# pgvector/pgvector

Measured on AMD Instinct MI355X. Metric: QPS @ recall@10 (IVFFlat, 1M x 1536d), higher is better.
Workload: dtype f32

## Files before the change

include/pgv_hip.h:

```cpp
#ifndef PGV_HIP_H
#define PGV_HIP_H

#include <stddef.h>
#include <stdint.h>

#ifdef __cplusplus
extern "C" {
#endif

#define PGV_ABI_VERSION 1

#define PGV_OK 0
#define PGV_ERR_ARG 1
#define PGV_ERR_DIMS 2
#define PGV_ERR_DEVICE 3
#define PGV_ERR_NOMEM 4
#define PGV_ERR_STATE 5
#define PGV_ERR_DATA 6

typedef enum pgv_dtype
{
	PGV_F32 = 0,
	PGV_F16 = 1
}			pgv_dtype;

typedef enum pgv_metric
{
	PGV_L2SQ = 0,
	PGV_NEG_IP = 1,
	PGV_L1 = 2
}			pgv_metric;

typedef enum pgv_ops
{
	PGV_OPS_L2 = 0,
	PGV_OPS_IP = 1,
	PGV_OPS_COSINE = 2
}			pgv_ops;

typedef struct pgv_ctx pgv_ctx;
typedef struct pgv_index pgv_index;
typedef struct pgv_hnsw pgv_hnsw;

typedef struct pgv_rng
{
	double		(*next_double) (void *state);
	uint32_t	(*next_u32) (void *state);
	void	   *state;
	uint64_t	seed;
}			pgv_rng;


const char *pgv_last_error(void);
int			pgv_abi_version(void);

int			pgv_device_count(void);
int			pgv_scan_chain_length(int dim, pgv_dtype dtype, int path);
int			pgv_device_memory(int device, uint64_t *free_bytes, uint64_t *total_bytes);
int			pgv_pinned_alloc(size_t bytes, void **out);
void		pgv_pinned_free(void *p);
int			pgv_pinned_register(void *p, size_t bytes);
void		pgv_pinned_unregister(void *p);

#define PGV_DEFAULT_STREAM ((void *) (intptr_t) -1)
int			pgv_ctx_create(int device, void *stream, pgv_ctx * *out);
void		pgv_ctx_destroy(pgv_ctx * ctx);
int			pgv_ctx_sync(pgv_ctx * ctx);
void	   *pgv_ctx_stream(pgv_ctx * ctx);
int			pgv_timer_start(pgv_ctx * ctx);
int			pgv_timer_stop(pgv_ctx * ctx, float *out_ms);

typedef struct pgv_stats
{
	double		scan_ms;
	int64_t		scan_launches;
	double		scan_pairs;
	double		scan_rows;
	double		aux_ms;
	int64_t		aux_launches;
	double		aux_pairs;
	double		assign_redo_rows;
	double		assign_rows;
	double		assign_recheck_rows;
	double		scan_unique_rows;
	double		scan_redo_queries;
	double		scan_widened_queries;
	double		scan_shadow_queries;
}			pgv_stats;
int			pgv_ctx_set_profiling(pgv_ctx * ctx, int on);
int			pgv_ctx_set_exact_scan(pgv_ctx * ctx, int on);
#define PGV_BOUND_STATISTICAL 0
#define PGV_BOUND_WORST_CASE 1
int			pgv_ctx_set_bound(pgv_ctx * ctx, int mode);
int			pgv_ctx_reset_stats(pgv_ctx * ctx);
int			pgv_ctx_get_stats(pgv_ctx * ctx, pgv_stats * out);


int			pgv_index_upload(pgv_ctx * ctx, pgv_metric metric, pgv_dtype dtype, int dim, int nlists,
							 const void *centers, const int64_t *list_offsets,
							 const void *vectors, const uint64_t *tids, pgv_index * *out);
void		pgv_index_free(pgv_index * index);
int			pgv_index_share(pgv_index * index, pgv_ctx * ctx, pgv_index * *out);
int			pgv_index_set_overlap(pgv_index * index, int lanes);
#define PGV_INDEX_HANDLE_BYTES 256
typedef struct pgv_index_handle
{
	unsigned char bytes[PGV_INDEX_HANDLE_BYTES];
}			pgv_index_handle;
int			pgv_index_export(pgv_index * index, pgv_index_handle * out);
int			pgv_index_import(pgv_ctx * ctx, const pgv_index_handle * handle, pgv_index * *out);
int			pgv_index_tids(pgv_index * index, const int64_t *slots, int64_t n, uint64_t *out);
int64_t		pgv_index_rows(const pgv_index * index);
int			pgv_index_lists(const pgv_index * index);

int			pgv_rank_lists(pgv_index * index, const void *queries, int nq, int maxprobes,
						   int32_t *out_lists, float *out_dist);

int			pgv_scan_lists(pgv_index * index, const void *query, const int32_t *lists, int nlists,
						   float *out_dist, int64_t *out_slot, int64_t capacity, int64_t *out_count);

int			pgv_search_batch(pgv_index * index, const void *queries, int nq, int probes, int k,
							 float *out_dist, int64_t *out_slot, uint64_t *out_tid);

int			pgv_scan_batch(pgv_index * index, const void *queries, int nq, const int32_t *probe_lists,
						   int probes, int k, float *out_dist, int64_t *out_slot, uint64_t *out_tid);

typedef struct pgv_query pgv_query;
int			pgv_query_begin(pgv_index * index, pgv_query * *out);
void		pgv_query_end(pgv_query * q);
int			pgv_query_rank(pgv_query * q, const void *query, int max_probes);
int			pgv_query_scan(pgv_query * q, int first, int nprobes, int head, float *out_dist, int64_t *out_slot,
						   uint64_t *out_tid, int *out_count, int64_t *out_total);
int			pgv_query_more(pgv_query * q, int skip, int count, float *out_dist, int64_t *out_slot,
						   uint64_t *out_tid, int *out_count);
int			pgv_query_lists(pgv_query * q, int32_t *out_lists, int n);


int			pgv_assign(pgv_ctx * ctx, pgv_metric metric, pgv_dtype dtype, int dim,
					   const void *centers, int k, const void *rows, int64_t n,
					   int32_t *out_list, float *out_dist);

int			pgv_kmeans(pgv_ctx * ctx, pgv_ops ops, pgv_dtype dtype, int dim,
					   const void *samples, int n, int k, int max_iterations, const pgv_rng * rng,
					   void *out_centers, int32_t *out_closest, int *out_iters);

int			pgv_lloyd_partial(pgv_ctx * ctx, pgv_ops ops, pgv_dtype dtype, int dim,
							  const void *samples, int n, const void *centers, int k,
							  int32_t *io_closest, float *out_sums, int32_t *out_counts,
							  int64_t *out_changes);
int			pgv_lloyd_finish(pgv_ctx * ctx, pgv_ops ops, pgv_dtype dtype, int dim, int k,
							 const float *sums, const int32_t *counts, const pgv_rng * rng,
							 void *out_centers);

int			pgv_kmeanspp_init(pgv_ctx * ctx, pgv_ops ops, pgv_dtype dtype, int dim,
							  const void *samples, int n, int k, const pgv_rng * rng,
							  void *out_centers);


typedef struct pgv_comm pgv_comm;

#define PGV_COMM_ID_BYTES 128
int			pgv_comm_unique_id(void *out_id);
int			pgv_comm_create(pgv_ctx * ctx, int nranks, int rank, const void *unique_id, pgv_comm * *out);

typedef struct pgv_collectives
{
	int			(*all_reduce_sum_f32) (void *state, float *buf, size_t count, void *stream);
	int			(*all_gather) (void *state, const void *send, void *recv, size_t bytes_per_rank, void *stream);
	void	   *state;
}			pgv_collectives;
int			pgv_comm_create_custom(pgv_ctx * ctx, int nranks, int rank, const pgv_collectives * coll, pgv_comm * *out);
void		pgv_comm_destroy(pgv_comm * comm);
int			pgv_comm_size(const pgv_comm * comm);
int			pgv_comm_rank(const pgv_comm * comm);

int			pgv_kmeans_sharded(pgv_comm * comm, pgv_ops ops, pgv_dtype dtype, int dim,
							   const void *samples_local, int n_local, int k, int max_iterations,
							   const pgv_rng * rng, void *out_centers, int32_t *out_closest_local, int *out_iters);

int			pgv_search_batch_sharded(pgv_comm * comm, pgv_index * local_index, const void *queries, int nq,
									 int probes, int k, float *out_dist, uint64_t *out_tid);

typedef struct pgv_builder pgv_builder;
int			pgv_builder_begin(pgv_ctx * ctx, pgv_metric metric, pgv_dtype dtype, int dim, int nlists, const void *centers,
							  int64_t expected_rows, pgv_builder * *out);
int			pgv_builder_add(pgv_builder * b, const void *rows, const uint64_t *tids, int64_t n);
int			pgv_builder_set_centers(pgv_builder * b, const void *centers);
int64_t		pgv_builder_rows(const pgv_builder * b);
int			pgv_builder_finish(pgv_builder * b, pgv_index * *out_index, int64_t *out_offsets, int32_t *out_lists);
void		pgv_builder_free(pgv_builder * b);
typedef int (*pgv_rows_sink) (void *arg, int64_t first_slot, int64_t count, const void *vectors, const uint64_t *tids);
int			pgv_index_drain(pgv_index * index, int64_t chunk_rows, pgv_rows_sink sink, void *arg);


int			pgv_distance_batch(pgv_ctx * ctx, pgv_metric metric, pgv_dtype dtype, int dim,
							   const void *query, const void *rows, int64_t n, float *out);

int			pgv_exact_topk(pgv_ctx * ctx, pgv_metric metric, pgv_dtype dtype, int dim, const void *queries, int nq,
						   const void *rows, int64_t n, int k, float *out_dist, int64_t *out_idx);

int			pgv_cosine_distance_batch(pgv_ctx * ctx, pgv_dtype dtype, int dim,
									  const void *query, const void *rows, int64_t n, double *out);

typedef enum pgv_bit_metric
{
	PGV_BIT_HAMMING = 0,
	PGV_BIT_JACCARD = 1
}			pgv_bit_metric;

int			pgv_bit_distance_batch(pgv_ctx * ctx, pgv_bit_metric metric, int nbits,
								   const void *query, const void *rows, int64_t n, double *out);


int			pgv_hnsw_upload(pgv_ctx * ctx, pgv_metric metric, pgv_dtype dtype, int dim,
							const void *elements, int64_t n, pgv_hnsw * *out);
void		pgv_hnsw_free(pgv_hnsw * h);
int			pgv_hnsw_upload_payload(pgv_ctx * ctx, pgv_metric metric, pgv_dtype dtype, int dim, const void *elements,
									int64_t n, const void *payload, int payload_bytes, pgv_hnsw * *out);
int			pgv_hnsw_get_payload(pgv_hnsw * h, const int64_t *elements, int n, void *out);

int			pgv_hnsw_export(pgv_hnsw * h, pgv_index_handle * out);
int			pgv_hnsw_share(pgv_hnsw * h, pgv_ctx * ctx, pgv_hnsw * *out);
int			pgv_hnsw_device(const pgv_hnsw * h);
int			pgv_hnsw_import(pgv_ctx * ctx, const pgv_index_handle * handle, pgv_hnsw * *out);

int			pgv_hnsw_score(pgv_hnsw * h, const void *queries, int nq,
						   const int32_t *slot, const int32_t *query_of, int64_t npairs, float *out);

int			pgv_hnsw_set_graph(pgv_hnsw * h, int m, int32_t entry, const int32_t *levels,
							   const int64_t *nbr_start, const int32_t *nbr);

int			pgv_hnsw_search(pgv_hnsw * h, const void *queries, int nq, int ef_search, int k,
							int64_t *out_elem, float *out_dist, int64_t *out_scored);


int			pgv_hnsw_build_search(pgv_hnsw * h, const int32_t *elements, const int32_t *insert_levels, int nq,
								  int ef_construction, int layer_cap,
								  int32_t *out_ids, float *out_dist, int32_t *out_count);

int			pgv_hnsw_build_neighbors(pgv_hnsw * h, const int32_t *elements, const int32_t *insert_levels, int nq,
									 int ef_construction, int layer_cap,
									 int32_t *out_ids, float *out_dist, uint8_t *out_closer, int32_t *out_count,
									 int64_t *out_pairs);

int			pgv_hnsw_build_search_keep(pgv_hnsw * h, const int32_t *elements, const int32_t *insert_levels, int nq,
									   int ef_construction, int layer_cap, int slot);
int			pgv_hnsw_build_select_kept(pgv_hnsw * h, int slot, int32_t *out_ids, float *out_dist, uint8_t *out_closer,
									   int32_t *out_count, int64_t *out_pairs);

int			pgv_hnsw_link_begin(pgv_hnsw * h);
int			pgv_hnsw_link_prepare(pgv_hnsw * h, const int32_t *elements, const uint8_t *linked, int nq, int layer_cap,
								  const int32_t *sel_ids, const float *sel_dist, const uint8_t *sel_closer,
								  const int32_t *sel_count, int64_t *out_pairs);
int			pgv_hnsw_link_apply(pgv_hnsw * h, int32_t entry);
int			pgv_hnsw_link_end(pgv_hnsw * h, int32_t *out_nbr, int64_t *out_pairs, int64_t *out_deferred);

int			pgv_hnsw_score_pairs(pgv_hnsw * h, const int32_t *a, const int32_t *b, int64_t npairs, float *out);
int			pgv_hnsw_score_groups(pgv_hnsw * h, const int32_t *ids, const int64_t *ids_start, const int32_t *from,
								  const int64_t *pair_start, int ngroups, int64_t nids, int64_t npairs, float *out);


int			pgv_hnsw_update_graph(pgv_hnsw * h, int32_t entry, const int32_t *elements, int nupd,
								  const int64_t *tuple_offsets, const int32_t *tuples);

#ifdef __cplusplus
}
#endif
#endif
```

pgvector_amd/_lib.py:

```python
import ctypes as C
import os

try:
    import torch
except ImportError:
    torch = None

_HERE = os.path.dirname(os.path.abspath(__file__))
LIB_PATH = os.environ.get("PGV_HIP_LIB") or os.path.join(_HERE, "lib", "libpgv_hip.so")

PGV_OK, PGV_ERR_ARG, PGV_ERR_DIMS, PGV_ERR_DEVICE, PGV_ERR_NOMEM, PGV_ERR_STATE, PGV_ERR_DATA = range(7)
PGV_F32, PGV_F16 = 0, 1
PGV_L2SQ, PGV_NEG_IP, PGV_L1 = 0, 1, 2
PGV_OPS_L2, PGV_OPS_IP, PGV_OPS_COSINE = 0, 1, 2
PGV_BOUND_STATISTICAL, PGV_BOUND_WORST_CASE = 0, 1

SYMBOLS = [
    "pgv_last_error", "pgv_abi_version", "pgv_device_count", "pgv_scan_chain_length", "pgv_ctx_create", "pgv_ctx_destroy",
    "pgv_ctx_sync", "pgv_ctx_stream", "pgv_timer_start", "pgv_timer_stop", "pgv_ctx_set_profiling", "pgv_ctx_set_exact_scan", "pgv_index_share", "pgv_pinned_alloc", "pgv_pinned_free",
    "pgv_ctx_reset_stats", "pgv_ctx_get_stats", "pgv_index_upload", "pgv_index_free",
    "pgv_index_rows", "pgv_index_lists", "pgv_rank_lists", "pgv_scan_lists", "pgv_search_batch", "pgv_scan_batch",
    "pgv_assign", "pgv_kmeans", "pgv_lloyd_partial", "pgv_lloyd_finish", "pgv_kmeanspp_init",
    "pgv_distance_batch", "pgv_cosine_distance_batch", "pgv_bit_distance_batch", "pgv_hnsw_upload", "pgv_hnsw_free", "pgv_hnsw_score", "pgv_hnsw_set_graph", "pgv_hnsw_search",
    "pgv_hnsw_build_search", "pgv_hnsw_build_neighbors", "pgv_hnsw_link_begin", "pgv_hnsw_link_prepare",
    "pgv_hnsw_link_apply", "pgv_hnsw_link_end", "pgv_hnsw_build_search_keep", "pgv_hnsw_build_select_kept", "pgv_hnsw_score_pairs", "pgv_hnsw_score_groups", "pgv_hnsw_update_graph",
    "pgv_query_begin", "pgv_query_end", "pgv_query_rank", "pgv_query_scan", "pgv_query_more", "pgv_query_lists",
    "pgv_comm_unique_id", "pgv_comm_create", "pgv_comm_create_custom", "pgv_comm_destroy", "pgv_comm_size",
    "pgv_comm_rank", "pgv_kmeans_sharded", "pgv_search_batch_sharded",
    "pgv_device_memory", "pgv_pinned_register", "pgv_pinned_unregister", "pgv_index_export", "pgv_index_import",
    "pgv_index_tids", "pgv_hnsw_export", "pgv_hnsw_import", "pgv_hnsw_share", "pgv_hnsw_device", "pgv_exact_topk", "pgv_ctx_set_bound",
    "pgv_hnsw_upload_payload", "pgv_hnsw_get_payload", "pgv_builder_begin", "pgv_builder_add", "pgv_builder_set_centers", "pgv_builder_rows", "pgv_builder_finish", "pgv_builder_free", "pgv_index_drain",
    "pgv_index_set_overlap",
]


class PgvError(RuntimeError):
    def __init__(self, code, message):
        super().__init__("libpgv_hip error %d: %s" % (code, message))
        self.code = code
        self.message = message


class PgvStats(C.Structure):
    _fields_ = [("scan_ms", C.c_double), ("scan_launches", C.c_int64),
                ("scan_pairs", C.c_double), ("scan_rows", C.c_double),
                ("aux_ms", C.c_double), ("aux_launches", C.c_int64), ("aux_pairs", C.c_double),
                ("assign_redo_rows", C.c_double), ("assign_rows", C.c_double), ("assign_recheck_rows", C.c_double), ("scan_unique_rows", C.c_double), ("scan_redo_queries", C.c_double), ("scan_widened_queries", C.c_double),
                ("scan_shadow_queries", C.c_double)]


ALL_REDUCE_F32 = C.CFUNCTYPE(C.c_int, C.c_void_p, C.c_void_p, C.c_size_t, C.c_void_p)
ALL_GATHER = C.CFUNCTYPE(C.c_int, C.c_void_p, C.c_void_p, C.c_void_p, C.c_size_t, C.c_void_p)


class PgvCollectives(C.Structure):
    _fields_ = [("all_reduce_sum_f32", ALL_REDUCE_F32), ("all_gather", ALL_GATHER), ("state", C.c_void_p)]


NEXT_DOUBLE = C.CFUNCTYPE(C.c_double, C.c_void_p)
NEXT_U32 = C.CFUNCTYPE(C.c_uint32, C.c_void_p)


class PgvRng(C.Structure):
    _fields_ = [("next_double", C.c_void_p), ("next_u32", C.c_void_p),
                ("state", C.c_void_p), ("seed", C.c_uint64)]


def _load():
    if not os.path.exists(LIB_PATH):
        raise ImportError(
            "libpgv_hip.so not built (%s): run `python -c 'import __graft_entry__ as g; g.build()'` "
            "or `make -C pgvector_amd/csrc` -- there is no CPU fallback" % LIB_PATH)
    lib = C.CDLL(LIB_PATH)
    P, I, I64 = C.c_void_p, C.c_int, C.c_int64
    lib.pgv_last_error.restype = C.c_char_p
    lib.pgv_last_error.argtypes = []
    lib.pgv_abi_version.restype = I
    lib.pgv_device_count.restype = I
    lib.pgv_scan_chain_length.argtypes = [I, I, I]
    lib.pgv_scan_chain_length.restype = I
    lib.pgv_ctx_create.argtypes = [I, P, C.POINTER(P)]
    lib.pgv_ctx_destroy.argtypes = [P]
    lib.pgv_ctx_destroy.restype = None
    lib.pgv_ctx_sync.argtypes = [P]
    lib.pgv_ctx_stream.argtypes = [P]
    lib.pgv_ctx_stream.restype = P
    lib.pgv_timer_start.argtypes = [P]
    lib.pgv_timer_stop.argtypes = [P, C.POINTER(C.c_float)]
    lib.pgv_ctx_set_profiling.argtypes = [P, I]
    lib.pgv_ctx_set_exact_scan.argtypes = [P, I]
    lib.pgv_ctx_reset_stats.argtypes = [P]
    lib.pgv_ctx_get_stats.argtypes = [P, C.POINTER(PgvStats)]
    lib.pgv_index_upload.argtypes = [P, I, I, I, I, P, P, P, P, C.POINTER(P)]
    lib.pgv_index_free.argtypes = [P]
    lib.pgv_index_share.argtypes = [P, P, C.POINTER(P)]
    lib.pgv_index_set_overlap.argtypes = [P, I]
    lib.pgv_index_free.restype = None
    lib.pgv_index_export.argtypes = [P, P]
    lib.pgv_index_import.argtypes = [P, P, C.POINTER(P)]
    lib.pgv_index_tids.argtypes = [P, P, I64, P]
    lib.pgv_hnsw_export.argtypes = [P, P]
    lib.pgv_hnsw_share.argtypes = [P, P, C.POINTER(P)]
    lib.pgv_hnsw_device.argtypes = [P]
    lib.pgv_hnsw_upload_payload.argtypes = [P, I, I, I, P, I64, P, I, C.POINTER(P)]
    lib.pgv_hnsw_get_payload.argtypes = [P, P, I, P]
    lib.pgv_exact_topk.argtypes = [P, I, I, I, P, I, P, I64, I, P, P]
    lib.pgv_ctx_set_bound.argtypes = [P, I]
    lib.pgv_builder_begin.argtypes = [P, I, I, I, I, P, I64, C.POINTER(P)]
    lib.pgv_builder_add.argtypes = [P, P, P, I64]
    lib.pgv_builder_set_centers.argtypes = [P, P]
    lib.pgv_builder_rows.argtypes = [P]
    lib.pgv_builder_rows.restype = I64
    lib.pgv_builder_finish.argtypes = [P, C.POINTER(P), P, P]
    lib.pgv_builder_free.argtypes = [P]
    lib.pgv_builder_free.restype = None
    lib.pgv_index_drain.argtypes = [P, I64, P, P]
    lib.pgv_hnsw_import.argtypes = [P, P, C.POINTER(P)]
    lib.pgv_device_memory.argtypes = [I, C.POINTER(C.c_uint64), C.POINTER(C.c_uint64)]
    lib.pgv_pinned_register.argtypes = [P, C.c_size_t]
    lib.pgv_pinned_unregister.argtypes = [P]
    lib.pgv_pinned_unregister.restype = None
    lib.pgv_index_rows.argtypes = [P]
    lib.pgv_index_rows.restype = I64
    lib.pgv_index_lists.argtypes = [P]
    lib.pgv_rank_lists.argtypes = [P, P, I, I, P, P]
    lib.pgv_scan_lists.argtypes = [P, P, P, I, P, P, I64, C.POINTER(I64)]
    lib.pgv_search_batch.argtypes = [P, P, I, I, I, P, P, P]
    lib.pgv_scan_batch.argtypes = [P, P, I, P, I, I, P, P, P]
    lib.pgv_query_begin.argtypes = [P, C.POINTER(P)]
    lib.pgv_query_end.argtypes = [P]
    lib.pgv_query_end.restype = None
    lib.pgv_query_rank.argtypes = [P, P, I]
    lib.pgv_query_scan.argtypes = [P, I, I, I, P, P, P, C.POINTER(I), C.POINTER(I64)]
    lib.pgv_query_more.argtypes = [P, I, I, P, P, P, C.POINTER(I)]
    lib.pgv_query_lists.argtypes = [P, P, I]
    lib.pgv_comm_unique_id.argtypes = [P]
    lib.pgv_comm_create.argtypes = [P, I, I, P, C.POINTER(P)]
    lib.pgv_comm_create_custom.argtypes = [P, I, I, C.POINTER(PgvCollectives), C.POINTER(P)]
    lib.pgv_comm_destroy.argtypes = [P]
    lib.pgv_comm_destroy.restype = None
    lib.pgv_comm_size.argtypes = [P]
    lib.pgv_comm_rank.argtypes = [P]
    lib.pgv_kmeans_sharded.argtypes = [P, I, I, I, P, I, I, I, C.POINTER(PgvRng), P, P, C.POINTER(I)]
    lib.pgv_search_batch_sharded.argtypes = [P, P, P, I, I, I, P, P]
    lib.pgv_assign.argtypes = [P, I, I, I, P, I, P, I64, P, P]
    lib.pgv_kmeans.argtypes = [P, I, I, I, P, I, I, I, C.POINTER(PgvRng), P, P, C.POINTER(I)]
    lib.pgv_lloyd_partial.argtypes = [P, I, I, I, P, I, P, I, P, P, P, P]
    lib.pgv_lloyd_finish.argtypes = [P, I, I, I, I, P, P, C.POINTER(PgvRng), P]
    lib.pgv_kmeanspp_init.argtypes = [P, I, I, I, P, I, I, C.POINTER(PgvRng), P]
    lib.pgv_distance_batch.argtypes = [P, I, I, I, P, P, I64, P]
    lib.pgv_hnsw_upload.argtypes = [P, I, I, I, P, I64, C.POINTER(P)]
    lib.pgv_hnsw_free.argtypes = [P]
    lib.pgv_hnsw_free.restype = None
    lib.pgv_hnsw_score.argtypes = [P, P, I, P, P, I64, P]
    lib.pgv_cosine_distance_batch.argtypes = [P, I, I, P, P, I64, P]
    lib.pgv_bit_distance_batch.argtypes = [P, I, I, P, P, I64, P]
    lib.pgv_hnsw_set_graph.argtypes = [P, I, C.c_int32, P, P, P]
    lib.pgv_hnsw_search.argtypes = [P, P, I, I, I, P, P, P]
    lib.pgv_hnsw_build_search.argtypes = [P, P, P, I, I, I, P, P, P]
    lib.pgv_hnsw_build_neighbors.argtypes = [P, P, P, I, I, I, P, P, P, P, P]
    lib.pgv_hnsw_score_pairs.argtypes = [P, P, P, I64, P]
    lib.pgv_hnsw_update_graph.argtypes = [P, C.c_int32, P, I, P, P]
    return lib


lib = _load()


def check(rc):
    if rc != PGV_OK:
        raise PgvError(rc, lib.pgv_last_error().decode("utf-8", "replace"))
```

pgvector_amd/csrc/kernels_query.hip:

```cpp
#include "pgv_device.h"
#include "pgv_select.h"

#include <type_traits>

namespace pgv {

namespace {

constexpr int kQThreads = kSelThreads;
constexpr int kQWaves = kQThreads / kWave;
constexpr int kMaxBatchLists = 256;
constexpr int kHeadCap = 1024;

template <typename T, int METRIC, int NCH> struct WholeRows {
    Raw16 q[NCH];
    __device__ __forceinline__ void load_query(const char *qp, int lane) {
#pragma unroll
        for (int c = 0; c < NCH; c++) q[c] = load16(qp + ((size_t)c * kWave + lane) * sizeof(Raw16));
    }
    __device__ __forceinline__ float pair(const char *a, const char *b, int lane) const {
        Raw16 ra[NCH], rb[NCH];
#pragma unroll
        for (int c = 0; c < NCH; c++) ra[c] = load16(a + ((size_t)c * kWave + lane) * sizeof(Raw16));
#pragma unroll
// ... 162 lines not shown
        return lbeg[lo] + (j - offs[lo]);
    }
};

template <typename T, int METRIC, int NCH>
__global__ __launch_bounds__(kQThreads) void query_scan_kernel(
    const char *__restrict__ vectors, const int64_t *__restrict__ list_off, const int32_t *__restrict__ probe_lists,
    int nprobes, int nvec, int lg, const char *__restrict__ qp, float *__restrict__ seg, int per) {
    __shared__ BatchMap map;
    const size_t row_bytes = (size_t)nvec * sizeof(Raw16);
    map.build(probe_lists, nprobes, list_off);
    const int64_t m = map.offs[nprobes];
    for (int64_t first = (int64_t)blockIdx.x * per; first < m; first += (int64_t)gridDim.x * per) {
        const int64_t end = first + per < m ? first + per : m;
        if (qp) {
            score_rows<T, METRIC, NCH>([&](int64_t j) { return vectors + (size_t)map.slot_of(j, nprobes) * row_bytes; },
                                       first, end, qp, nvec, lg, seg);
        } else {
            for (int64_t j = first + threadIdx.x; j < end; j += kQThreads) seg[j] = 0.f;
        }
    }
}

__global__ __launch_bounds__(kQThreads) void query_head_kernel(
    const float *__restrict__ seg, const int64_t *__restrict__ list_off, const uint64_t *__restrict__ tids,
    const int32_t *__restrict__ probe_lists, int nprobes, int skip, int count, int kp, QueryHead *__restrict__ hdr,
    float *__restrict__ head_dist, int64_t *__restrict__ head_slot, uint64_t *__restrict__ head_tid, unsigned seq) {
    extern __shared__ __attribute__((aligned(16))) char smem[];
    __shared__ BatchMap map;
    map.build(probe_lists, nprobes, list_off);
    const int64_t m = map.offs[nprobes];
    unsigned long long *ent = reinterpret_cast<unsigned long long *>(smem);
    SelShared *s = reinterpret_cast<SelShared *>(smem + (size_t)kHeadCap * 8);
    const int k = skip + count;
    block_topk_auto(seg, m, k, kp, kHeadCap, ent, s);
    const int have = (int)(m < k ? m : k) - skip;
    for (int i = threadIdx.x; i < have; i += kQThreads) {
        const unsigned long long e = ent[skip + i];
        const int64_t slot = map.slot_of((int64_t)(unsigned)(e & 0xffffffffu), nprobes);
        head_dist[i] = key_to_float((unsigned)(e >> 32));
        head_slot[i] = slot;
        head_tid[i] = tids ? tids[slot] : ~0ull;
    }
    asm volatile("s_waitcnt vmcnt(0)" ::: "memory");
    __syncthreads();
    if (threadIdx.x == 0) {
        hdr->total = m;
        hdr->count = have > 0 ? have : 0;
        __hip_atomic_store(&hdr->seq, seq, __ATOMIC_RELEASE, __HIP_MEMORY_SCOPE_SYSTEM);
    }
}

__global__ __launch_bounds__(1024) void query_stage_kernel(const Raw16 *__restrict__ src, Raw16 *__restrict__ dst, int nvec) {
    for (int i = threadIdx.x; i < nvec; i += 1024) dst[i] = src[i];
}

__global__ void query_iota_kernel(int32_t *__restrict__ out, int n) {
    const int i = blockIdx.x * blockDim.x + threadIdx.x;
    if (i < n) out[i] = i;
}

template <typename T, int METRIC, int NCH>
__global__ __launch_bounds__(kQThreads) void mq_rank_kernel(const char *__restrict__ centers, int nlists, int nvec, int lg,
                                                            const char *__restrict__ queries, float *__restrict__ cdist,
                                                            int64_t cd_stride, int per) {
    const size_t row_bytes = (size_t)nvec * sizeof(Raw16);
    const char *qp = queries + (size_t)blockIdx.y * row_bytes;
    float *cd = cdist + (size_t)blockIdx.y * cd_stride;
    for (int64_t first = (int64_t)blockIdx.x * per; first < nlists; first += (int64_t)gridDim.x * per) {
        const int64_t end = first + per < nlists ? first + per : nlists;
        score_rows<T, METRIC, NCH>([&](int64_t j) { return centers + (size_t)j * row_bytes; }, first, end, qp, nvec, lg, cd);
    }
}

__global__ __launch_bounds__(kQThreads) void mq_lists_kernel(const float *__restrict__ cdist, int64_t cd_stride, int nlists,
                                                             int max_probes, int kp, int32_t *__restrict__ out_lists,
                                                             float *__restrict__ out_dist) {
    extern __shared__ __attribute__((aligned(16))) char smem[];
    unsigned long long *ent = reinterpret_cast<unsigned long long *>(smem);
    SelShared *s = reinterpret_cast<SelShared *>(smem + (size_t)kHeadCap * 8);
    const int q = blockIdx.x;
    block_topk_auto(cdist + (size_t)q * cd_stride, nlists, max_probes, kp, kHeadCap, ent, s);
    for (int i = threadIdx.x; i < max_probes; i += kQThreads) {
        out_lists[(size_t)q * max_probes + i] = (int32_t)(unsigned)(ent[i] & 0xffffffffu);
        if (out_dist) out_dist[(size_t)q * max_probes + i] = key_to_float((unsigned)(ent[i] >> 32));
    }
}

template <typename T, int METRIC, int NCH>
__global__ __launch_bounds__(kQThreads) void mq_scan_kernel(
    const char *__restrict__ vectors, const int64_t *__restrict__ list_off, const int32_t *__restrict__ probe_lists,
    int nprobes, int nvec, int lg, const char *__restrict__ queries, float *__restrict__ seg, int64_t seg_stride, int per) {
    __shared__ BatchMap map;
    const size_t row_bytes = (size_t)nvec * sizeof(Raw16);
    const int q = blockIdx.y;
    map.build(probe_lists + (size_t)q * nprobes, nprobes, list_off);
    const int64_t m = map.offs[nprobes];
    const char *qp = queries + (size_t)q * row_bytes;
    float *sg = seg + (size_t)q * seg_stride;
    for (int64_t first = (int64_t)blockIdx.x * per; first < m; first += (int64_t)gridDim.x * per) {
        const int64_t end = first + per < m ? first + per : m;
        score_rows<T, METRIC, NCH>([&](int64_t j) { return vectors + (size_t)map.slot_of(j, nprobes) * row_bytes; },
                                   first, end, qp, nvec, lg, sg);
    }
}

__global__ __launch_bounds__(kQThreads) void mq_head_kernel(
    const float *__restrict__ seg, int64_t seg_stride, const int64_t *__restrict__ list_off,
    const uint64_t *__restrict__ tids, const int32_t *__restrict__ probe_lists, int nprobes, int k, int kp,
    float *__restrict__ out_dist, int64_t *__restrict__ out_slot, uint64_t *__restrict__ out_tid,
    double *__restrict__ stats) {
    extern __shared__ __attribute__((aligned(16))) char smem[];
    __shared__ BatchMap map;
    const int q = blockIdx.x;
    map.build(probe_lists + (size_t)q * nprobes, nprobes, list_off);
    const int64_t m = map.offs[nprobes];
    unsigned long long *ent = reinterpret_cast<unsigned long long *>(smem);
    SelShared *s = reinterpret_cast<SelShared *>(smem + (size_t)kHeadCap * 8);
    block_topk_auto(seg + (size_t)q * seg_stride, m, k, kp, kHeadCap, ent, s);
    const int have = (int)(m < k ? m : k);
    for (int i = threadIdx.x; i < k; i += kQThreads) {
        const size_t o = (size_t)q * k + i;
        if (i < have) {
            const unsigned long long e = ent[i];
            const int64_t slot = map.slot_of((int64_t)(unsigned)(e & 0xffffffffu), nprobes);
            out_dist[o] = key_to_float((unsigned)(e >> 32));
            if (out_slot) out_slot[o] = slot;
            if (out_tid) out_tid[o] = tids ? tids[slot] : ~0ull;
        } else {
            out_dist[o] = INFINITY;
            if (out_slot) out_slot[o] = -1;
            if (out_tid) out_tid[o] = ~0ull;
        }
    }
    if (stats && threadIdx.x == 0) {
        atomicAdd(&stats[0], (double)m);
        atomicAdd(&stats[1], (double)m);
        atomicAdd(&stats[5], (double)m);
    }
}

constexpr int kRecheckCap = 256;

template <typename T, bool DOT = false>
__global__ __launch_bounds__(kQThreads) void batch_recheck_kernel(
    const char *__restrict__ vectors, const uint64_t *__restrict__ tids, int nvec, int lg,
    const char *__restrict__ queries, int kprime, int k, const float *__restrict__ approx_val,
    const int64_t *__restrict__ cand_pos, const int64_t *__restrict__ cand_slot,
    const int64_t *__restrict__ list_off, const int32_t *__restrict__ probe_lists,
    const int64_t *__restrict__ probe_off, int probes,
    const int64_t *__restrict__ seg_start, int64_t fixed_len,
    const unsigned *__restrict__ row_norm_max, ScanBound bound, const float *__restrict__ eps_add, int nq,
    float *__restrict__ out_dist, int64_t *__restrict__ out_slot, uint64_t *__restrict__ out_tid,
    int32_t *__restrict__ out_i32, int32_t *__restrict__ flags, float *__restrict__ pair_t) {
    static_assert(!DOT || std::is_same<T, float>::value, "pair terms: fp32 rows");
    __shared__ float exact[kRecheckCap];
    __shared__ float dots[DOT ? kRecheckCap : 1];
    __shared__ __attribute__((aligned(16))) unsigned long long ent[kRecheckCap];
    const int q = blockIdx.x;
    const size_t row_bytes = (size_t)nvec * sizeof(Raw16);
    const int64_t m = seg_start ? seg_start[q + 1] - seg_start[q] : fixed_len;
    const int ncand = (int)(m < kprime ? m : (int64_t)kprime);
    const int kk = ncand < k ? ncand : k;
    const float *av = approx_val + (size_t)q * kprime;
    __shared__ float qn_part[kQWaves];
    {
        const char *qrow = queries + (size_t)q * row_bytes;
        float a = 0.f;
        for (int v = threadIdx.x; v < nvec; v += kQThreads) {
            const Raw16 x = load16(qrow + (size_t)v * sizeof(Raw16));
            a = accum_slice<T, 1>(a, x, x);
        }
        for (int m2 = 32; m2 > 0; m2 >>= 1) a += __shfl_xor(a, m2);
        if ((threadIdx.x & (kWave - 1)) == 0) qn_part[threadIdx.x >> 6] = a;
    }
    __syncthreads();
    float qn = 0.f;
    for (int w = 0; w < kQWaves; w++) qn += qn_part[w];
    const float rn = __uint_as_float(*row_norm_max);
    const float cross = 2.f * sqrtf(qn * rn);
    const float eps = 1.001f * (bound.g_sq * (qn + rn + cross) + bound.g_dot * cross + bound.g_norm * rn +
                                (eps_add ? eps_add[q] : 0.f));
    unsigned band = 0u;
    if (kk > 0) {
        const float edge = av[kk - 1] + 2.f * eps;
        band = float_to_key(edge + bound.g_ref * fabsf(edge + qn));
    }
    const int cnt = __syncthreads_count((int)threadIdx.x < ncand && float_to_key(av[threadIdx.x]) <= band);
    __shared__ int64_t slots[kRecheckCap];
    if ((int)threadIdx.x < cnt) {
        const int64_t p = cand_pos[(size_t)q * kprime + threadIdx.x];
        int64_t slot = p;
        if (cand_slot) {
            slot = cand_slot[(size_t)q * kprime + threadIdx.x];
        } else {
            const int64_t *off = probe_off + (size_t)q * probes;
            int lo = 0, hi = probes - 1;
            while (lo < hi) {
                const int mid = (lo + hi + 1) >> 1;
                if (off[mid] <= p)
                    lo = mid;
                else
                    hi = mid - 1;
            }
            slot = list_off[probe_lists[(size_t)q * probes + lo]] + (p - off[lo]);
        }
        slots[threadIdx.x] = slot;
    }
    __syncthreads();
    if constexpr (DOT)
        score_rows_dot([&](int64_t j) { return vectors + (size_t)slots[j] * row_bytes; }, 0, cnt,
                       queries + (size_t)q * row_bytes, nvec, lg, exact, dots);
    else
        score_rows<T, 0, 0>([&](int64_t j) { return vectors + (size_t)slots[j] * row_bytes; }, 0, cnt,
                            queries + (size_t)q * row_bytes, nvec, lg, exact);
    __syncthreads();
    if ((int)threadIdx.x < kRecheckCap)
        ent[threadIdx.x] = (int)threadIdx.x < cnt
                               ? ((unsigned long long)float_to_key(exact[threadIdx.x]) << 32) |
                                     (unsigned)cand_pos[(size_t)q * kprime + threadIdx.x]
                               : ~0ull;
    __syncthreads();
    const unsigned long long mine = ent[threadIdx.x];
    const int64_t my_slot = (int)threadIdx.x < cnt ? slots[threadIdx.x] : -1;
    int rank = 0;
    {
        const ulonglong2 *e2 = reinterpret_cast<const ulonglong2 *>(ent);
        const int n2 = (cnt + 1) / 2;
#pragma unroll 8
        for (int j = 0; j < n2; j++) {
            const ulonglong2 o = e2[j];
            rank += o.x < mine ? 1 : 0;
            rank += o.y < mine ? 1 : 0;
        }
    }
    if ((int)threadIdx.x < cnt && rank < k) {
        const size_t o = (size_t)q * k + rank;
        out_dist[o] = key_to_float((unsigned)(mine >> 32));
        if (out_slot) out_slot[o] = my_slot;
        if (out_i32) out_i32[o] = (int32_t)my_slot;
        if (out_tid) out_tid[o] = tids ? tids[my_slot] : ~0ull;
        if constexpr (DOT) pair_t[o] = -2.f * dots[threadIdx.x];
    }
    if ((int)threadIdx.x >= kk && (int)threadIdx.x < k) {
        const size_t o = (size_t)q * k + threadIdx.x;
        out_dist[o] = INFINITY;
        if (out_slot) out_slot[o] = -1;
        if (out_i32) out_i32[o] = -1;
        if (out_tid) out_tid[o] = ~0ull;
        if constexpr (DOT) pair_t[o] = 0.f;
    }
    if (threadIdx.x == 0) {
        const int32_t flag = (m > ncand && cnt == ncand) ? 1 : 0;
        flags[q] = flag;
        if (flag) flags[nq + 1 + atomicAdd(&flags[nq], 1)] = q;
    }
}

constexpr int kWide = kRecheckCap;

template <typename T>
__global__ __launch_bounds__(kQThreads) void batch_fix_kernel(
    const char *__restrict__ vectors, const int64_t *__restrict__ list_off, const uint64_t *__restrict__ tids, int nvec,
    int lg, const char *__restrict__ queries, const int32_t *__restrict__ probe_lists,
    const int64_t *__restrict__ probe_off, int probes, const int64_t *__restrict__ seg_start, int64_t fixed_len,
    const int32_t *__restrict__ flags, int nq, float *__restrict__ seg_vals, int k, int kp, int cap,
    const unsigned *__restrict__ row_norm_max, ScanBound bound, const float *__restrict__ eps_add, int widen,
    float *__restrict__ out_dist, int64_t *__restrict__ out_slot, uint64_t *__restrict__ out_tid,
    int32_t *__restrict__ out_i32, double *__restrict__ stats, float *__restrict__ pair_t) {
    extern __shared__ __attribute__((aligned(16))) char smem[];
    unsigned long long *ent = reinterpret_cast<unsigned long long *>(smem);
    SelShared *sel = reinterpret_cast<SelShared *>(smem + (size_t)cap * 8);
    __shared__ float exact[kWide];
    __shared__ int64_t slots[kWide];
    __shared__ float qn_part[kQWaves];
    const int nflag = flags[nq];
    const size_t row_bytes = (size_t)nvec * sizeof(Raw16);
    for (int f = blockIdx.x; f < nflag; f += gridDim.x) {
        const int q = flags[nq + 1 + f];
        const int64_t base = probe_lists ? seg_start[q] : (int64_t)q * fixed_len;
        const int64_t m = probe_lists ? seg_start[q + 1] - base : fixed_len;
        const int64_t *off = probe_off + (size_t)q * probes;
        const int32_t *pl = probe_lists + (size_t)q * probes;
        auto slot_of = [&](int64_t j) -> int64_t {
            if (!probe_lists) return j;
            int lo = 0, hi = probes - 1;
            while (lo < hi) {
                const int mid = (lo + hi + 1) >> 1;
                if (off[mid] <= j)
                    lo = mid;
                else
                    hi = mid - 1;
            }
            return list_off[pl[lo]] + (j - off[lo]);
        };
        float *v = seg_vals + base;
        const char *qrow = queries + (size_t)q * row_bytes;
        auto pair_terms = [&]() {
            if constexpr (std::is_same<T, float>::value) {
                if (pair_t) {
                    __threadfence();
                    __syncthreads();
                    fill_pair_terms(vectors, row_bytes, qrow, nvec * 4, out_i32 ? out_i32 + (size_t)q * k : nullptr,
                                    out_slot ? out_slot + (size_t)q * k : nullptr, k, pair_t + (size_t)q * k);
                }
            }
        };
        bool settled = false;
        if (widen && k <= kWide / 2) {
            const int nw = (int)(m < kWide ? m : (int64_t)kWide);
            block_topk([v](int64_t i) { return v[i]; }, m, nw, kWide, cap, ent, sel);
            {
                float a = 0.f;
                for (int x = threadIdx.x; x < nvec; x += kQThreads) {
                    const Raw16 e = load16(qrow + (size_t)x * sizeof(Raw16));
                    a = accum_slice<T, 1>(a, e, e);
                }
                for (int m2 = 32; m2 > 0; m2 >>= 1) a += __shfl_xor(a, m2);
                if ((threadIdx.x & (kWave - 1)) == 0) qn_part[threadIdx.x >> 6] = a;
            }
            __syncthreads();
            float qn = 0.f;
            for (int w = 0; w < kQWaves; w++) qn += qn_part[w];
            const float rn = __uint_as_float(*row_norm_max);
            const float cross = 2.f * sqrtf(qn * rn);
            const float eps = 1.001f * (bound.g_sq * (qn + rn + cross) + bound.g_dot * cross + bound.g_norm * rn +
                                        (eps_add ? eps_add[q] : 0.f));
            const int kk = nw < k ? nw : k;
            unsigned band = 0u;
            if (kk > 0) {
                const float edge = key_to_float((unsigned)(ent[kk - 1] >> 32)) + 2.f * eps;
                band = float_to_key(edge + bound.g_ref * fabsf(edge + qn));
            }
            const int cnt = __syncthreads_count((int)threadIdx.x < nw && (unsigned)(ent[threadIdx.x] >> 32) <= band);
            settled = !(m > nw && cnt == nw);
            if (settled) {
                const unsigned my_pos = (int)threadIdx.x < cnt ? (unsigned)(ent[threadIdx.x] & 0xffffffffu) : 0u;
                if ((int)threadIdx.x < cnt) slots[threadIdx.x] = slot_of((int64_t)my_pos);
                __syncthreads();
                score_rows<T, 0, 0>([&](int64_t j) { return vectors + (size_t)slots[j] * row_bytes; }, 0, cnt, qrow, nvec, lg,
                                    exact);
                __syncthreads();
                if ((int)threadIdx.x < kWide)
                    ent[threadIdx.x] = (int)threadIdx.x < cnt
                                           ? ((unsigned long long)float_to_key(exact[threadIdx.x]) << 32) | my_pos
                                           : ~0ull;
                __syncthreads();
                const unsigned long long mine = ent[threadIdx.x];
                int rank = 0;
                for (int j = 0; j < cnt; j++) rank += ent[j] < mine ? 1 : 0;
                const int have = (int)(m < k ? m : (int64_t)k);
                if ((int)threadIdx.x < cnt && rank < k) {
                    const size_t o = (size_t)q * k + rank;
                    const int64_t slot = slots[threadIdx.x];
                    out_dist[o] = key_to_float((unsigned)(mine >> 32));
                    if (out_slot) out_slot[o] = slot;
                    if (out_i32) out_i32[o] = (int32_t)slot;
                    if (out_tid) out_tid[o] = tids ? tids[slot] : ~0ull;
                }
                if ((int)threadIdx.x >= have && (int)threadIdx.x < k) {
                    const size_t o = (size_t)q * k + threadIdx.x;
                    out_dist[o] = INFINITY;
                    if (out_slot) out_slot[o] = -1;
                    if (out_i32) out_i32[o] = -1;
                    if (out_tid) out_tid[o] = ~0ull;
                }
                if (stats && threadIdx.x == 0) atomicAdd(&stats[7], 1.0);
                pair_terms();
            }
            __syncthreads();
        }
        if (settled) continue;
        if (stats && threadIdx.x == 0) atomicAdd(&stats[6], 1.0);
        score_rows<T, 0, 0>([&](int64_t j) { return vectors + (size_t)slot_of(j) * row_bytes; }, 0, m, qrow, nvec, lg, v);
        __threadfence();
        __syncthreads();
        block_topk([v](int64_t i) { return __hip_atomic_load(v + i, __ATOMIC_RELAXED, __HIP_MEMORY_SCOPE_AGENT); }, m, k, kp,
                   cap, ent, sel);
        for (int i = threadIdx.x; i < k; i += kQThreads) {
            const unsigned long long e = ent[i];
            const bool have = e != ~0ull && (int64_t)i < (m < k ? m : (int64_t)k);
            const int64_t slot = have ? slot_of((int64_t)(unsigned)(e & 0xffffffffu)) : -1;
            out_dist[(size_t)q * k + i] = have ? key_to_float((unsigned)(e >> 32)) : INFINITY;
            if (out_slot) out_slot[(size_t)q * k + i] = slot;
            if (out_i32) out_i32[(size_t)q * k + i] = (int32_t)slot;
            if (out_tid) out_tid[(size_t)q * k + i] = (have && tids) ? tids[slot] : ~0ull;
        }
        pair_terms();
        __syncthreads();
    }
}

constexpr size_t kQueryLds = (size_t)kHeadCap * 8 + sizeof(SelShared);

void run_geometry(pgv_ctx *ctx, const RowGeom &g, int64_t nrows, int *per, int *grid) {
    const bool whole = g.lpr_log2 == 6 && g.nvec % kWave == 0;
    const int step = kQWaves * (whole ? 2 : (kWave >> g.lpr_log2));
    int64_t runs = (nrows + step - 1) / step;
    const int64_t cap = (int64_t)ctx->num_cus * 8;
    *per = step;
    *grid = (int)(runs < 1 ? 1 : (runs > cap ? cap : runs));
}

int pow2_at_least(int k) {
    int kp = 2;
    while (kp < k) kp <<= 1;
    return kp;
}

template <typename T, int METRIC, typename F> int dispatch_nch(const RowGeom &g, F f) {
    if (g.lpr_log2 == 6 && g.nvec % kWave == 0) {
        switch (g.nvec / kWave) {
            case 1: return f(std::integral_constant<int, 1>());
            case 2: return f(std::integral_constant<int, 2>());
            case 3: return f(std::integral_constant<int, 3>());
            case 4: return f(std::integral_constant<int, 4>());
            case 6: return f(std::integral_constant<int, 6>());
        }
    }
    return f(std::integral_constant<int, 0>());
}

template <typename F> int dispatch_metric(pgv_metric metric, pgv_dtype dtype, F f) {
#define PGV_QM(T)                                                                     \
    switch (metric) {                                                                 \
        case PGV_L2SQ: return f((T *)nullptr, std::integral_constant<int, 0>());      \
        case PGV_NEG_IP: return f((T *)nullptr, std::integral_constant<int, 1>());    \
        case PGV_L1: return f((T *)nullptr, std::integral_constant<int, 2>());        \
    }
    if (dtype == PGV_F32) {
        PGV_QM(float)
    } else {
        PGV_QM(__half)
    }
#undef PGV_QM
    PGV_FAIL(PGV_ERR_ARG, "query: unknown metric %d", (int)metric);
}

}

int query_max_batch_lists() { return kMaxBatchLists; }
int query_head_cap() { return kHeadCap; }
size_t query_head_bytes(int head) { return sizeof(QueryHead) + (size_t)head * (4 + 8 + 8) + 64; }

int launch_query_stage(pgv_ctx *ctx, const void *src_pinned, void *dst_dev, int nvec) {
    hipLaunchKernelGGL(query_stage_kernel, dim3(1), dim3(1024), 0, ctx->stream, static_cast<const Raw16 *>(src_pinned),
                       static_cast<Raw16 *>(dst_dev), nvec);
    PGV_HIP(hipGetLastError());
    return PGV_OK;
}

int launch_query_iota(pgv_ctx *ctx, int32_t *out, int n) {
    hipLaunchKernelGGL(query_iota_kernel, dim3((n + 255) / 256), dim3(256), 0, ctx->stream, out, n);
    PGV_HIP(hipGetLastError());
    return PGV_OK;
}

int launch_one_query_rows(pgv_ctx *ctx, pgv_metric metric, pgv_dtype dtype, const RowGeom &g, const void *rows, int n,
                          const void *q_dev, float *out) {
    if (n <= 0) return PGV_OK;
    int per, grid;
    run_geometry(ctx, g, n, &per, &grid);
    return dispatch_metric(metric, dtype, [&](auto *tp, auto mc) {
        using T = std::remove_pointer_t<decltype(tp)>;
        constexpr int M = decltype(mc)::value;
        return dispatch_nch<T, M>(g, [&](auto nc) {
            constexpr int NCH = decltype(nc)::value;
            hipLaunchKernelGGL((query_rank_kernel<T, M, NCH>), dim3(grid), dim3(kQThreads), 0, ctx->stream,
                               static_cast<const char *>(rows), n, g.nvec, g.lpr_log2, static_cast<const char *>(q_dev),
                               out, per);
            PGV_HIP(hipGetLastError());
            return PGV_OK;
        });
    });
}

int launch_query_rank(pgv_ctx *ctx, const pgv_index *ix, const void *q_dev, float *cdist, int max_probes,
                      int32_t *out_lists) {
    const RowGeom &g = ix->geom;
    int per, grid;
    run_geometry(ctx, g, ix->nlists, &per, &grid);
    const int kp = pow2_at_least(max_probes);
    PGV_TRY(dispatch_metric(ix->metric, ix->dtype, [&](auto *tp, auto mc) {
        using T = std::remove_pointer_t<decltype(tp)>;
        constexpr int M = decltype(mc)::value;
        return dispatch_nch<T, M>(g, [&](auto nc) {
            constexpr int NCH = decltype(nc)::value;
            hipLaunchKernelGGL((query_rank_kernel<T, M, NCH>), dim3(grid), dim3(kQThreads), 0, ctx->stream,
                               static_cast<const char *>(ix->centers), ix->nlists, g.nvec, g.lpr_log2,
                               static_cast<const char *>(q_dev), cdist, per);
            PGV_HIP(hipGetLastError());
            return PGV_OK;
        });
    }));
    hipLaunchKernelGGL(query_lists_kernel, dim3(1), dim3(kQThreads), kQueryLds, ctx->stream, cdist, ix->nlists,
                       max_probes, kp, out_lists);
    PGV_HIP(hipGetLastError());
    return PGV_OK;
}

int launch_query_scan(pgv_ctx *ctx, const pgv_index *ix, const void *q_dev, const int32_t *probe_lists, int nprobes,
                      int64_t rows_bound, float *seg) {
    const RowGeom &g = ix->geom;
    int per, grid;
    run_geometry(ctx, g, rows_bound, &per, &grid);
    return dispatch_metric(ix->metric, ix->dtype, [&](auto *tp, auto mc) {
        using T = std::remove_pointer_t<decltype(tp)>;
        constexpr int M = decltype(mc)::value;
        return dispatch_nch<T, M>(g, [&](auto nc) {
            constexpr int NCH = decltype(nc)::value;
            hipLaunchKernelGGL((query_scan_kernel<T, M, NCH>), dim3(grid), dim3(kQThreads), 0, ctx->stream,
                               static_cast<const char *>(ix->vectors), ix->list_offsets, probe_lists, nprobes, g.nvec,
                               g.lpr_log2, static_cast<const char *>(q_dev), seg, per);
            PGV_HIP(hipGetLastError());
            return PGV_OK;
        });
    });
}

int launch_query_head(pgv_ctx *ctx, const pgv_index *ix, const float *seg, const int32_t *probe_lists, int nprobes,
                      int skip, int count, void *head_rec, unsigned seq) {
    const int kp = pow2_at_least(skip + count);
    QueryHead *hdr = static_cast<QueryHead *>(head_rec);
    char *base = static_cast<char *>(head_rec) + 64;
    int64_t *h_slot = reinterpret_cast<int64_t *>(base);
    uint64_t *h_tid = reinterpret_cast<uint64_t *>(base + (size_t)count * 8);
    float *h_dist = reinterpret_cast<float *>(base + (size_t)count * 16);
    hipLaunchKernelGGL(query_head_kernel, dim3(1), dim3(kQThreads), kQueryLds, ctx->stream, seg, ix->list_offsets,
                       ix->tids, probe_lists, nprobes, skip, count, kp, hdr, h_dist, h_slot, h_tid, seq);
    PGV_HIP(hipGetLastError());
    return PGV_OK;
}

int launch_multi_rank(pgv_ctx *ctx, const pgv_index *ix, const void *q_dev, int nq, float *cdist, int64_t cd_stride,
                      int max_probes, int32_t *out_lists, float *out_dist) {
    const RowGeom &g = ix->geom;
    int per, grid;
    run_geometry(ctx, g, ix->nlists, &per, &grid);
    const int kp = pow2_at_least(max_probes);
    PGV_TRY(dispatch_metric(ix->metric, ix->dtype, [&](auto *tp, auto mc) {
        using T = std::remove_pointer_t<decltype(tp)>;
        constexpr int M = decltype(mc)::value;
        return dispatch_nch<T, M>(g, [&](auto nc) {
            constexpr int NCH = decltype(nc)::value;
            hipLaunchKernelGGL((mq_rank_kernel<T, M, NCH>), dim3(grid, nq), dim3(kQThreads), 0, ctx->stream,
                               static_cast<const char *>(ix->centers), ix->nlists, g.nvec, g.lpr_log2,
                               static_cast<const char *>(q_dev), cdist, cd_stride, per);
            PGV_HIP(hipGetLastError());
            return PGV_OK;
        });
    }));
    hipLaunchKernelGGL(mq_lists_kernel, dim3(nq), dim3(kQThreads), kQueryLds, ctx->stream, cdist, cd_stride, ix->nlists,
                       max_probes, kp, out_lists, out_dist);
    PGV_HIP(hipGetLastError());
    return PGV_OK;
}

int launch_multi_scan(pgv_ctx *ctx, const pgv_index *ix, const void *q_dev, int nq, const int32_t *probe_lists, int nprobes,
                      int64_t rows_bound, float *seg, int64_t seg_stride, int k, float *out_dist, int64_t *out_slot,
                      uint64_t *out_tid) {
    const RowGeom &g = ix->geom;
    int per, grid;
    run_geometry(ctx, g, rows_bound, &per, &grid);
    const int cap = (ctx->num_cus * 8 + nq - 1) / nq;
    if (grid > cap) grid = cap < 1 ? 1 : cap;
    PGV_TRY(dispatch_metric(ix->metric, ix->dtype, [&](auto *tp, auto mc) {
        using T = std::remove_pointer_t<decltype(tp)>;
        constexpr int M = decltype(mc)::value;
        return dispatch_nch<T, M>(g, [&](auto nc) {
            constexpr int NCH = decltype(nc)::value;
            hipLaunchKernelGGL((mq_scan_kernel<T, M, NCH>), dim3(grid, nq), dim3(kQThreads), 0, ctx->stream,
                               static_cast<const char *>(ix->vectors), ix->list_offsets, probe_lists, nprobes, g.nvec,
                               g.lpr_log2, static_cast<const char *>(q_dev), seg, seg_stride, per);
            PGV_HIP(hipGetLastError());
            return PGV_OK;
        });
    }));
    double *stats = (ctx->profiling && ctx->stats_dev.p) ? ctx->stats_dev.as<double>() : nullptr;
    hipLaunchKernelGGL(mq_head_kernel, dim3(nq), dim3(kQThreads), kQueryLds, ctx->stream, seg, seg_stride, ix->list_offsets,
                       ix->tids, probe_lists, nprobes, k, pow2_at_least(k), out_dist, out_slot, out_tid, stats);
    PGV_HIP(hipGetLastError());
    return PGV_OK;
}

int launch_batch_recheck(pgv_ctx *ctx, const ExactRows &xr, const void *q_dev, int nq, int kprime, int k,
                         const float *approx_val, const int64_t *cand_pos, const int64_t *cand_slot,
                         const int64_t *seg_start, int64_t fixed_len, const ScanBound &bound,
                         float *out_dist, int64_t *out_slot, uint64_t *out_tid, int32_t *flags, int32_t *out_i32,
                         const int32_t *probe_lists, const int64_t *probe_off, int probes, const float *eps_add,
                         float *pair_t) {
    if (nq <= 0) return PGV_OK;
    if (kprime > kRecheckCap || k > kprime) PGV_FAIL(PGV_ERR_ARG, "recheck: k' = %d outside k..%d", kprime, kRecheckCap);
    if (pair_t && xr.dtype != PGV_F32) PGV_FAIL(PGV_ERR_ARG, "recheck: pair terms are for fp32 rows");
#define PGV_RECHECK(T, DOT)                                                                                         \
    hipLaunchKernelGGL((batch_recheck_kernel<T, DOT>), dim3(nq), dim3(kQThreads), 0, ctx->stream,                    \
                       static_cast<const char *>(xr.vectors), xr.tids, xr.geom.nvec, xr.geom.lpr_log2,               \
                       static_cast<const char *>(q_dev), kprime, k, approx_val, cand_pos, cand_slot, xr.list_offsets, \
                       probe_lists, probe_off, probes, seg_start, fixed_len, xr.norm_max, bound, eps_add, nq, out_dist, out_slot,  \
                       out_tid, out_i32, flags, pair_t)
    if (pair_t)
        PGV_RECHECK(float, true);
    else if (xr.dtype == PGV_F32)
        PGV_RECHECK(float, false);
    else
        PGV_RECHECK(__half, false);
#undef PGV_RECHECK
    PGV_HIP(hipGetLastError());
    return PGV_OK;
}

int launch_batch_fix(pgv_ctx *ctx, const ExactRows &xr, const void *q_dev, int nq, const int32_t *probe_lists,
                     const int64_t *probe_off, int probes, const int64_t *seg_start, int64_t fixed_len,
                     const int32_t *flags, float *seg_vals, int k, const ScanBound &bound, float *out_dist, int64_t *out_slot,
                     uint64_t *out_tid, int32_t *out_i32, const float *eps_add, float *pair_t) {
    if (nq <= 0) return PGV_OK;
    if (pair_t && xr.dtype != PGV_F32) PGV_FAIL(PGV_ERR_ARG, "fix: pair terms are for fp32 rows");
    double *stats = (ctx->profiling && ctx->stats_dev.p) ? ctx->stats_dev.as<double>() : nullptr;
    if (k > 4096) PGV_FAIL(PGV_ERR_ARG, "top-k: k = %d exceeds the supported 4096", k);
    int kp = 2;
    while (kp < k) kp <<= 1;
    const int cap = kp > kFastCap ? kp : kFastCap;
    const int widen = ctx->no_widen ? 0 : 1;
    const size_t lds = (size_t)cap * 8 + sizeof(SelShared);
    const int grid = nq < ctx->num_cus ? nq : ctx->num_cus;
#define PGV_FIX(T)                                                                                                   \
    hipLaunchKernelGGL(batch_fix_kernel<T>, dim3(grid), dim3(kQThreads), lds, ctx->stream,                           \
                       static_cast<const char *>(xr.vectors), xr.list_offsets, xr.tids, xr.geom.nvec,                \
                       xr.geom.lpr_log2, static_cast<const char *>(q_dev), probe_lists, probe_off, probes, seg_start, \
                       fixed_len, flags, nq, seg_vals, k, kp, cap, xr.norm_max, bound, eps_add, widen, out_dist,      \
                       out_slot, out_tid, out_i32, stats, pair_t)
    if (xr.dtype == PGV_F32)
        PGV_FIX(float);
    else
        PGV_FIX(__half);
#undef PGV_FIX
    PGV_HIP(hipGetLastError());
    return PGV_OK;
}

}
```

pgvector_amd/csrc/kernels_select.hip:

```cpp
#include "pgv_device.h"
#include "pgv_select.h"

namespace pgv {

namespace {


__global__ void plan_count_kernel(const int32_t *__restrict__ probe_lists,
                                  const int64_t *__restrict__ list_off, int nq, int probes,
                                  int *__restrict__ cnt, int64_t *__restrict__ probe_off,
                                  int64_t *__restrict__ seg_len) {
    const int q = blockIdx.x * blockDim.x + threadIdx.x;
    if (q >= nq) return;
    int64_t run = 0;
    for (int p = 0; p < probes; p++) {
        const int l = probe_lists[(size_t)q * probes + p];
        probe_off[(size_t)q * probes + p] = run;
        run += list_off[l + 1] - list_off[l];
        atomicAdd(&cnt[l], 1);
    }
    seg_len[q] = run;
}

template <typename F>
__device__ void block_exclusive_scan(int n, F value, int64_t *out, int64_t *scratch ) {
    const int lane = threadIdx.x & 63, wave = threadIdx.x >> 6, nwaves = blockDim.x >> 6;
    int64_t carry = 0;
    for (int base = 0; base < n; base += blockDim.x) {
        const int i = base + threadIdx.x;
        const int64_t v = i < n ? value(i) : 0;
        int64_t incl = v;
#pragma unroll
        for (int d = 1; d < 64; d <<= 1) {
            const int64_t t = __shfl_up(incl, d);
            if (lane >= d) incl += t;
        }
        if (lane == 63) scratch[wave] = incl;
        __syncthreads();
        int64_t before = 0, total = 0;
        for (int w = 0; w < nwaves; w++) {
            const int64_t t = scratch[w];
            if (w < wave) before += t;
            total += t;
        }
        if (i < n) out[i] = carry + before + incl - v;
        carry += total;
        __syncthreads();
    }
    if (threadIdx.x == 0) out[n] = carry;
    __syncthreads();
}

__global__ __launch_bounds__(1024) void plan_scan_kernel(
    const int *__restrict__ cnt, const int64_t *__restrict__ list_off,
    const int64_t *__restrict__ seg_len, int nq, int nlists, int qt, int rows_per_task,
    int64_t *__restrict__ seg_start, int64_t *__restrict__ pair_start,
    int64_t *__restrict__ task_start, int64_t *__restrict__ totals ) {
    __shared__ int64_t scratch[1024 / 64 + 1];
    block_exclusive_scan(nq, [&](int i) { return seg_len[i]; }, seg_start, scratch);
    block_exclusive_scan(nlists, [&](int i) { return (int64_t)cnt[i]; }, pair_start, scratch);
    block_exclusive_scan(
        nlists,
        [&](int i) {
            const int64_t len = list_off[i + 1] - list_off[i];
            const int64_t ng = (cnt[i] + qt - 1) / qt;
            const int64_t nc = (len + rows_per_task - 1) / rows_per_task;
            return ng * nc;
        },
        task_start, scratch);
    if (threadIdx.x == 0) {
        totals[0] = seg_start[nq];
        totals[1] = task_start[nlists];
        *reinterpret_cast<int *>(totals + 2) = (int)task_start[nlists];
    }
}

__global__ void plan_pairs_kernel(const int32_t *__restrict__ probe_lists,
                                  const int64_t *__restrict__ list_off,
                                  const int64_t *__restrict__ probe_off,
                                  const int64_t *__restrict__ seg_start,
                                  const int64_t *__restrict__ pair_start, int *__restrict__ fill,
                                  int nq, int probes, const float *__restrict__ pair_t,
                                  ScanPair *__restrict__ pairs) {
    const int64_t i = (int64_t)blockIdx.x * blockDim.x + threadIdx.x;
    if (i >= (int64_t)nq * probes) return;
    const int q = (int)(i / probes);
    const int l = probe_lists[i];
    const int64_t pos = pair_start[l] + atomicAdd(&fill[l], 1);
    ScanPair pr;
    pr.out_rel = seg_start[q] + probe_off[i] - list_off[l];
    pr.query = q;
    pr.pad = pair_t ? (int32_t)__float_as_uint(pair_t[i]) : 0;
    pairs[pos] = pr;
}

__global__ void plan_tasks_kernel(const int *__restrict__ cnt, const int64_t *__restrict__ list_off,
                                  const int64_t *__restrict__ pair_start,
                                  const int64_t *__restrict__ task_start, int nlists, int qt,
                                  int rows_per_task, ScanTask *__restrict__ tasks) {
    const int64_t ntasks = task_start[nlists];
    for (int64_t t = (int64_t)blockIdx.x * blockDim.x + threadIdx.x; t < ntasks; t += (int64_t)gridDim.x * blockDim.x) {
        int lo = 0, hi = nlists - 1;
        while (lo < hi) {
            const int mid = (lo + hi + 1) >> 1;
            if (task_start[mid] <= t)
                lo = mid;
            else
                hi = mid - 1;
        }
        const int l = lo;
        const int64_t len = list_off[l + 1] - list_off[l];
        const int ng = (cnt[l] + qt - 1) / qt;
        const int64_t rel = t - task_start[l];
        const int c = (int)(rel / ng), g = (int)(rel % ng);
        ScanTask task;
        task.row0 = list_off[l] + (int64_t)c * rows_per_task;
        const int64_t left = len - (int64_t)c * rows_per_task;
        task.nrows = (int)(left < rows_per_task ? left : rows_per_task);
        task.pair0 = (int)(pair_start[l] + (int64_t)g * qt);
        const int pl = cnt[l] - g * qt;
        task.npairs = pl < qt ? pl : qt;
        task.pad = ng > 1 ? 1 : 0;
        tasks[t] = task;
    }
}

__device__ __forceinline__ bool dist_before(float a, float b) { return float_to_key(a) < float_to_key(b); }


__global__ __launch_bounds__(kSelThreads) void topk_kernel(
    const float *__restrict__ vals, const int64_t *__restrict__ seg_start, int64_t fixed_len,
    int k, int kp, int cap, float *__restrict__ out_val, int64_t *__restrict__ out_pos,
    int32_t *__restrict__ zero_word) {
    extern __shared__ __attribute__((aligned(16))) char smem[];
    unsigned long long *ent = reinterpret_cast<unsigned long long *>(smem);
    SelShared *s = reinterpret_cast<SelShared *>(smem + (size_t)cap * 8);

    const int seg = blockIdx.x;
    if (zero_word && seg == 0 && threadIdx.x == 0) *zero_word = 0;
    const int64_t base = seg_start ? seg_start[seg] : (int64_t)seg * fixed_len;
    const int64_t m = seg_start ? seg_start[seg + 1] - base : fixed_len;
    const float *v = vals + base;
    block_topk_auto(v, m, k, kp, cap, ent, s);

    for (int i = threadIdx.x; i < k; i += kSelThreads) {
        const unsigned long long e = ent[i];
        const bool have = e != ~0ull && (int64_t)i < (m < k ? m : (int64_t)k);
        out_val[(size_t)seg * k + i] = have ? key_to_float((unsigned)(e >> 32)) : INFINITY;
        out_pos[(size_t)seg * k + i] = have ? (int64_t)(unsigned)(e & 0xffffffffu) : -1;
    }
}

__global__ void positions_to_slots_kernel(const int32_t *__restrict__ probe_lists,
                                          const int64_t *__restrict__ probe_off,
                                          const int64_t *__restrict__ list_off,
                                          const uint64_t *__restrict__ tids, int nq, int probes,
                                          int k, const int64_t *__restrict__ pos,
                                          int64_t *__restrict__ out_slot,
                                          uint64_t *__restrict__ out_tid) {
    const int64_t i = (int64_t)blockIdx.x * blockDim.x + threadIdx.x;
    if (i >= (int64_t)nq * k) return;
    const int q = (int)(i / k);
    const int64_t p = pos[i];
    int64_t slot = -1;
    if (p >= 0) {
        const int64_t *off = probe_off + (size_t)q * probes;
        int lo = 0, hi = probes - 1;
        while (lo < hi) {
            const int mid = (lo + hi + 1) >> 1;
            if (off[mid] <= p)
                lo = mid;
            else
                hi = mid - 1;
        }
        const int l = probe_lists[(size_t)q * probes + lo];
        slot = list_off[l] + (p - off[lo]);
    }
    if (out_slot) out_slot[i] = slot;
    if (out_tid) out_tid[i] = (slot >= 0 && tids) ? tids[slot] : ~0ull;
}

__global__ void iota_slots_kernel(const int32_t *__restrict__ lists,
                                  const int64_t *__restrict__ probe_off,
                                  const int64_t *__restrict__ list_off,
                                  int64_t *__restrict__ out_slot) {
    const int p = blockIdx.x;
    const int l = lists[p];
    const int64_t beg = list_off[l], len = list_off[l + 1] - beg;
    for (int64_t i = threadIdx.x; i < len; i += blockDim.x) out_slot[probe_off[p] + i] = beg + i;
}

__global__ __launch_bounds__(256) void plan_stats_kernel(const int *__restrict__ cnt,
                                                         const int64_t *__restrict__ list_off,
                                                         const int64_t *__restrict__ totals, int nlists,
                                                         int qt, double *__restrict__ acc) {
    __shared__ double red[256], red_u[256];
    double rows = 0.0, uniq = 0.0;
    for (int l = threadIdx.x; l < nlists; l += 256) {
        const double len = (double)(list_off[l + 1] - list_off[l]);
        rows += (double)((cnt[l] + qt - 1) / qt) * len;
        uniq += cnt[l] > 0 ? len : 0.0;
    }
    red[threadIdx.x] = rows;
    red_u[threadIdx.x] = uniq;
    __syncthreads();
    for (int s = 128; s > 0; s >>= 1) {
        if (threadIdx.x < s) {
            red[threadIdx.x] += red[threadIdx.x + s];
            red_u[threadIdx.x] += red_u[threadIdx.x + s];
        }
        __syncthreads();
    }
    if (threadIdx.x == 0) {
        acc[0] += (double)totals[0];
        acc[1] += red[0];
        acc[5] += red_u[0];
    }
}

__global__ void merge_heads_kernel(const float *__restrict__ dist_all, const uint64_t *__restrict__ tid_all, int nranks,
                                   int nq, int k, float *__restrict__ out_dist, uint64_t *__restrict__ out_tid) {
    const int q = blockIdx.x * blockDim.x + threadIdx.x;
    if (q >= nq) return;
    int at[16];
    for (int r = 0; r < nranks; r++) at[r] = 0;
    for (int i = 0; i < k; i++) {
        int best = -1;
        float bd = INFINITY;
        for (int r = 0; r < nranks; r++) {
            if (at[r] >= k) continue;
            const float d = dist_all[((size_t)r * nq + q) * k + at[r]];
            if (best < 0 || dist_before(d, bd)) {
                best = r;
                bd = d;
            }
        }
        out_dist[(size_t)q * k + i] = bd;
        out_tid[(size_t)q * k + i] = tid_all[((size_t)best * nq + q) * k + at[best]];
        at[best]++;
    }
}

__global__ void cast_pos_kernel(const int64_t *__restrict__ pos, int64_t n,
                                int32_t *__restrict__ out) {
    const int64_t i = (int64_t)blockIdx.x * blockDim.x + threadIdx.x;
    if (i < n) out[i] = (int32_t)pos[i];
}

}

int launch_merge_heads(pgv_ctx *ctx, const float *dist_all, const uint64_t *tid_all, int nranks, int nq, int k,
                       float *out_dist, uint64_t *out_tid) {
    if (nq <= 0) return PGV_OK;
    if (nranks > 16) PGV_FAIL(PGV_ERR_ARG, "merge: more than 16 ranks");
    hipLaunchKernelGGL(merge_heads_kernel, dim3((nq + 127) / 128), dim3(128), 0, ctx->stream, dist_all, tid_all, nranks,
                       nq, k, out_dist, out_tid);
    PGV_HIP(hipGetLastError());
    return PGV_OK;
}

int launch_cast_pos_to_i32(pgv_ctx *ctx, const int64_t *pos, int64_t n, int32_t *out) {
    if (n <= 0) return PGV_OK;
    hipLaunchKernelGGL(cast_pos_kernel, dim3((unsigned)((n + 255) / 256)), dim3(256), 0,
                       ctx->stream, pos, n, out);
    PGV_HIP(hipGetLastError());
    return PGV_OK;
}

int launch_plan_batch(pgv_ctx *ctx, const pgv_index *ix, const int32_t *probe_lists, int nq,
                      int probes, int qt, int rows_per_task, bool read_totals, PlanResult *res, const float *pair_t) {
    const int nlists = ix->nlists;
    const size_t npairs = (size_t)nq * probes;

    int64_t max_chunks = 0, sum_chunks = 0;
    for (int l = 0; l < nlists; l++) {
        const int64_t nc = (ix->h_offsets[l + 1] - ix->h_offsets[l] + rows_per_task - 1) / rows_per_task;
        sum_chunks += nc;
        if (nc > max_chunks) max_chunks = nc;
    }
    res->ntasks_bound = max_chunks * (int64_t)(npairs / qt) + sum_chunks;
    res->out_bound = (int64_t)nq * ix->len_prefix[probes];
    if (res->ntasks_bound > 0x7fffffff) PGV_FAIL(PGV_ERR_ARG, "plan: too many tasks");

    PGV_TRY(ctx->plan_a.ensure(sizeof(int) * 2 * (size_t)nlists));
    const size_t nb = npairs + (size_t)nq + (size_t)nq + 1 + 2 * ((size_t)nlists + 1) + 3;
    PGV_TRY(ctx->plan_b.ensure(sizeof(int64_t) * nb));
    PGV_TRY(ctx->pairs.ensure(sizeof(ScanPair) * npairs));
    PGV_TRY(ctx->tasks.ensure(sizeof(ScanTask) * (size_t)(res->ntasks_bound > 0 ? res->ntasks_bound : 1) + 16));
    int *cnt = ctx->plan_a.as<int>();
    int *fill = cnt + nlists;
    int64_t *probe_off = ctx->plan_b.as<int64_t>();
    int64_t *seg_len = probe_off + npairs;
    int64_t *seg_start = seg_len + nq;
    int64_t *pair_start = seg_start + nq + 1;
    int64_t *task_start = pair_start + nlists + 1;
    int64_t *totals = task_start + nlists + 1;
    ScanTask *tasks = ctx->tasks.as<ScanTask>();

    PGV_HIP(hipMemsetAsync(cnt, 0, sizeof(int) * 2 * (size_t)nlists, ctx->stream));
    hipLaunchKernelGGL(plan_count_kernel, dim3((nq + 255) / 256), dim3(256), 0, ctx->stream,
                       probe_lists, ix->list_offsets, nq, probes, cnt, probe_off, seg_len);
    hipLaunchKernelGGL(plan_scan_kernel, dim3(1), dim3(1024), 0, ctx->stream, cnt,
                       ix->list_offsets, seg_len, nq, nlists, qt, rows_per_task, seg_start,
                       pair_start, task_start, totals);
    hipLaunchKernelGGL(plan_pairs_kernel, dim3((unsigned)((npairs + 255) / 256)), dim3(256), 0,
                       ctx->stream, probe_lists, ix->list_offsets, probe_off, seg_start,
                       pair_start, fill, nq, probes, pair_t, ctx->pairs.as<ScanPair>());
    {
        const int64_t want = (res->ntasks_bound + 255) / 256;
        const int64_t cap = (int64_t)ctx->num_cus * 8;
        hipLaunchKernelGGL(plan_tasks_kernel, dim3((unsigned)(want < 1 ? 1 : (want > cap ? cap : want))), dim3(256), 0,
                           ctx->stream, cnt, ix->list_offsets, pair_start, task_start, nlists, qt, rows_per_task, tasks);
    }
    PGV_HIP(hipGetLastError());

    res->ntasks = res->ntasks_bound;
    res->total_out = res->out_bound;
    if (read_totals) {
        PGV_TRY(ctx->stats_dev.ensure(8 * sizeof(double)));
        hipLaunchKernelGGL(plan_stats_kernel, dim3(1), dim3(256), 0, ctx->stream, cnt,
                           ix->list_offsets, totals, nlists, qt, ctx->stats_dev.as<double>());
        PGV_HIP(hipGetLastError());
    }
    res->tasks = tasks;
    res->pairs = ctx->pairs.as<ScanPair>();
    res->ntasks_dev = reinterpret_cast<int *>(totals + 2);
    res->seg_start = seg_start;
    res->probe_off = probe_off;
    res->pair_start = pair_start;
    return PGV_OK;
}

int launch_topk_segments(pgv_ctx *ctx, const float *vals, const int64_t *seg_start, int nseg,
                         int64_t fixed_len, int k, float *out_val, int64_t *out_pos, int32_t *zero_word) {
    if (nseg <= 0 || k <= 0) return PGV_OK;
    if (k > 4096) PGV_FAIL(PGV_ERR_ARG, "top-k: k = %d exceeds the supported 4096", k);
    int kp = 1;
    while (kp < k) kp <<= 1;
    if (kp < 2) kp = 2;
    const int cap = kp > kFastCap ? kp : kFastCap;
    const size_t lds = (size_t)cap * 8 + sizeof(SelShared);
    hipLaunchKernelGGL(topk_kernel, dim3(nseg), dim3(kSelThreads), lds, ctx->stream, vals,
                       seg_start, fixed_len, k, kp, cap, out_val, out_pos, zero_word);
    PGV_HIP(hipGetLastError());
    return PGV_OK;
}

int launch_positions_to_slots(pgv_ctx *ctx, const pgv_index *ix, const int32_t *probe_lists,
                              const int64_t *probe_off, int nq, int probes, int k,
                              const int64_t *pos, int64_t *out_slot, uint64_t *out_tid) {
    const int64_t total = (int64_t)nq * k;
    if (total <= 0) return PGV_OK;
    hipLaunchKernelGGL(positions_to_slots_kernel, dim3((unsigned)((total + 255) / 256)), dim3(256),
                       0, ctx->stream, probe_lists, probe_off, ix->list_offsets, ix->tids, nq,
                       probes, k, pos, out_slot, out_tid);
    PGV_HIP(hipGetLastError());
    return PGV_OK;
}

int launch_iota_slots(pgv_ctx *ctx, const pgv_index *ix, const int32_t *lists_dev, int nlists,
                      const int64_t *probe_off, int64_t *out_slot) {
    if (nlists <= 0) return PGV_OK;
    hipLaunchKernelGGL(iota_slots_kernel, dim3(nlists), dim3(256), 0, ctx->stream, lists_dev,
                       probe_off, ix->list_offsets, out_slot);
    PGV_HIP(hipGetLastError());
    return PGV_OK;
}

}
```

pgvector_amd/csrc/kernels_shadow.hip:

```cpp
#include "pgv_device.h"

#include <cfloat>

namespace pgv {

namespace {

__device__ __forceinline__ int list_of_row(const int64_t *__restrict__ list_off, int nlists, int64_t r) {
    int lo = 0, hi = nlists - 1;
    while (lo < hi) {
        const int mid = (lo + hi + 1) >> 1;
        if (list_off[mid] <= r)
            lo = mid;
        else
            hi = mid - 1;
    }
    return lo;
}

__device__ __forceinline__ int scale_for(float m) {
    if (!(m > 0.f) || !isfinite(m)) return 0;
    int e;
    (void)frexpf(m, &e);
    return e - 14;
}

__global__ __launch_bounds__(256) void shadow_absmax_kernel(const float *__restrict__ rows, const float *__restrict__ centers,
                                                            const int64_t *__restrict__ list_off, int nlists, int64_t n,
                                                            int ld, unsigned *__restrict__ max_bits) {
    const int64_t r = (int64_t)blockIdx.x * 4 + (threadIdx.x >> 6);
    if (r >= n) return;
    const int lane = threadIdx.x & (kWave - 1);
    const float *x = rows + (size_t)r * ld;
    const float *c = centers ? centers + (size_t)list_of_row(list_off, nlists, r) * ld : nullptr;
    float m = 0.f;
    for (int i = lane; i < ld; i += kWave) {
        const float d = fabsf(c ? x[i] - c[i] : x[i]);
        m = (d > m || d != d) ? d : m;
    }
    for (int o = 32; o > 0; o >>= 1) {
        const float v = __shfl_xor(m, o);
        m = (v > m || v != v) ? v : m;
    }
    if (lane == 0 && __float_as_uint(m) > __hip_atomic_load(max_bits, __ATOMIC_RELAXED, __HIP_MEMORY_SCOPE_AGENT))
        atomicMax(max_bits, __float_as_uint(m));
}

__global__ __launch_bounds__(256) void shadow_build_kernel(const float *__restrict__ rows, const float *__restrict__ centers,
                                                           const int64_t *__restrict__ list_off, int nlists, int64_t n,
                                                           int ld, int ld16, const unsigned *__restrict__ max_bits,
                                                           __half *__restrict__ shadow,
                                                           unsigned long long *__restrict__ ep_bits) {
    const int64_t r = (int64_t)blockIdx.x * 4 + (threadIdx.x >> 6);
    if (r >= n) return;
    const int lane = threadIdx.x & (kWave - 1);
    const int s = scale_for(__uint_as_float(*max_bits));
    const float *x = rows + (size_t)r * ld;
    const float *c = centers ? centers + (size_t)list_of_row(list_off, nlists, r) * ld : nullptr;
    __half *h = shadow + (size_t)r * ld16;
    const double up = ldexp(1.0, s);
    double e2 = 0.0, p2 = 0.0;
    for (int i = lane; i < ld16; i += kWave) {
        __half v = __float2half(0.f);
        if (i < ld) {
            const float ci = c ? c[i] : 0.f;
            v = __float2half(ldexpf(x[i] - ci, -s));
            const double back = (double)__half2float(v) * up;
            const double d = ((double)x[i] - (double)ci) - back;
            e2 = fma(d, d, e2);
            p2 = fma(back, back, p2);
        }
        h[i] = v;
    }
    for (int o = 32; o > 0; o >>= 1) {
        e2 += __shfl_xor(e2, o);
        p2 += __shfl_xor(p2, o);
    }
    if (lane == 0) {
        const unsigned long long eb = (unsigned long long)__double_as_longlong(e2 != e2 ? INFINITY : e2),
                                 pb = (unsigned long long)__double_as_longlong(p2 != p2 ? INFINITY : p2);
        if (eb > __hip_atomic_load(&ep_bits[0], __ATOMIC_RELAXED, __HIP_MEMORY_SCOPE_AGENT)) atomicMax(&ep_bits[0], eb);
        if (pb > __hip_atomic_load(&ep_bits[1], __ATOMIC_RELAXED, __HIP_MEMORY_SCOPE_AGENT)) atomicMax(&ep_bits[1], pb);
    }
}

__global__ __launch_bounds__(256) void shadow_query_kernel(const float *__restrict__ queries, int nq, int ld, int ld16,
                                                           ShadowTerms st, RankShadowTerms rt,
                                                           const float *__restrict__ center_norm_max,
                                                           const float *__restrict__ row_norm_max,
                                                           __half *__restrict__ qcast, float *__restrict__ qscale,
                                                           float *__restrict__ qeps, float *__restrict__ cscale,
                                                           float *__restrict__ ceps) {
    const int q = (int)(blockIdx.x * 4 + (threadIdx.x >> 6));
    if (q >= nq) return;
    const int lane = threadIdx.x & (kWave - 1);
    const float *x = queries + (size_t)q * ld;
    float m = 0.f;
    for (int i = lane; i < ld; i += kWave) {
        const float a = fabsf(x[i]);
        m = (a > m || a != a) ? a : m;
    }
    for (int o = 32; o > 0; o >>= 1) {
        const float v = __shfl_xor(m, o);
        m = (v > m || v != v) ? v : m;
    }
    const int sq = scale_for(m);
    const double up = ldexp(1.0, sq);
    double qq = 0.0, dd = 0.0, hh = 0.0;
    __half *h = qcast + (size_t)q * ld16;
    for (int i = lane; i < ld16; i += kWave) {
        __half v = __float2half(0.f);
        if (i < ld) {
            v = __float2half(ldexpf(x[i], -sq));
            const double back = (double)__half2float(v) * up, xi = (double)x[i];
            qq = fma(xi, xi, qq);
            dd = fma(xi - back, xi - back, dd);
            hh = fma(back, back, hh);
        }
        h[i] = v;
    }
    for (int o = 32; o > 0; o >>= 1) {
        qq += __shfl_xor(qq, o);
        dd += __shfl_xor(dd, o);
        hh += __shfl_xor(hh, o);
    }
    const double u = 5.9604644775390625e-8;
    if (lane == 0 && ceps) {
        const int e = 1 + rt.s + sq;
        const double qn = sqrt(qq), dq = sqrt(dd), qh = sqrt(hh);
        const double cn = (double)*center_norm_max * (1.0 + rt.g_cn);
        double eps = 2.0 * (qn * rt.E + dq * rt.P)
                     + rt.g_dot * 2.0 * qh * rt.P
                     + 4.0 * u * (cn + 2.0 * qh * rt.P * (1.0 + rt.g_dot));
        eps = eps * (1.0 + 1.0 / 1048576.0) + 4.0 * (double)FLT_MIN;
        if (e < -125 || e > 125 || !(eps < 1e30)) eps = INFINITY;
        cscale[q] = ldexpf(1.f, e < -125 ? 0 : (e > 125 ? 0 : e));
        ceps[q] = (float)eps;
    }
    if (lane == 0 && qeps) {
        const int e = 1 + st.s + sq;
        const double qn = sqrt(qq), dq = sqrt(dd), qh = sqrt(hh);
        const double cmax = sqrt((double)*center_norm_max * (1.0 + st.g_cn)), rn = (double)*row_norm_max * (1.0 + st.g_cn);
        const double tmax = 2.0 * qn * cmax;
        double eps = 2.0 * (qn * st.E + dq * st.P)
                     + st.g_dot * 2.0 * qh * st.P
                     + st.g_pair * tmax
                     + 4.0 * u * (rn + tmax * (1.0 + st.g_pair) + 2.0 * qh * st.P * (1.0 + st.g_dot));
        eps = eps * (1.0 + 1.0 / 1048576.0) + 4.0 * (double)FLT_MIN;
        if (e < -125 || e > 125 || !(eps < 1e30)) eps = INFINITY;
        qscale[q] = ldexpf(1.f, e < -125 ? 0 : (e > 125 ? 0 : e));
        qeps[q] = (float)eps;
    }
}

__global__ __launch_bounds__(256) void shadow_pair_kernel(const float *__restrict__ queries, const float *__restrict__ centers,
                                                          const int64_t *__restrict__ pair_start, int nlists, int64_t npairs,
                                                          int ld, ScanPair *__restrict__ pairs) {
    const int64_t pos = (int64_t)blockIdx.x * 4 + (threadIdx.x >> 6);
    if (pos >= npairs) return;
    const int lane = threadIdx.x & (kWave - 1);
    int lo = 0, hi = nlists - 1;
    while (lo < hi) {
        const int mid = (lo + hi + 1) >> 1;
        if (pair_start[mid] <= pos)
            lo = mid;
        else
            hi = mid - 1;
    }
    const int q = pairs[pos].query;
    const float *x = queries + (size_t)q * ld;
    const float *c = centers + (size_t)lo * ld;
    float a = 0.f;
    for (int i = lane; i < ld; i += kWave) a = fmaf(x[i], c[i], a);
    for (int o = 32; o > 0; o >>= 1) a += __shfl_xor(a, o);
    if (lane == 0) pairs[pos].pad = (int32_t)__float_as_uint(-2.f * a);
}

}

int launch_shadow_build(pgv_ctx *ctx, const RowGeom &g32, const RowGeom &g16, const void *rows, const void *centers,
                        const int64_t *list_off, int nlists, int64_t n, void *shadow, void *words) {
    if (n <= 0) return PGV_OK;
    PGV_HIP(hipMemsetAsync(words, 0, 24, ctx->stream));
    unsigned *max_bits = static_cast<unsigned *>(words);
    unsigned long long *ep = reinterpret_cast<unsigned long long *>(static_cast<char *>(words) + 8);
    const dim3 grid((unsigned)((n + 3) / 4));
    hipLaunchKernelGGL(shadow_absmax_kernel, grid, dim3(256), 0, ctx->stream, static_cast<const float *>(rows),
                       static_cast<const float *>(centers), list_off, nlists, n, g32.ld, max_bits);
    hipLaunchKernelGGL(shadow_build_kernel, grid, dim3(256), 0, ctx->stream, static_cast<const float *>(rows),
                       static_cast<const float *>(centers), list_off, nlists, n, g32.ld, g16.ld, max_bits, static_cast<__half *>(shadow), ep);
    PGV_HIP(hipGetLastError());
    return PGV_OK;
}

int shadow_scale_of(float max_abs) {
    if (!(max_abs > 0.f) || !std::isfinite(max_abs)) return 0;
    int e;
    (void)std::frexp(max_abs, &e);
    return e - 14;
}

int launch_shadow_query(pgv_ctx *ctx, const RowGeom &g32, const RowGeom &g16, const void *queries, int nq,
                        const ShadowTerms &st, const RankShadowTerms &rt, const float *center_norm_max,
                        const float *row_norm_max, void *qcast, float *qscale, float *qeps, float *cscale, float *ceps) {
    if (nq <= 0) return PGV_OK;
    hipLaunchKernelGGL(shadow_query_kernel, dim3((unsigned)((nq + 3) / 4)), dim3(256), 0, ctx->stream,
                       static_cast<const float *>(queries), nq, g32.ld, g16.ld, st, rt, center_norm_max, row_norm_max,
                       static_cast<__half *>(qcast), qscale, qeps, cscale, ceps);
    PGV_HIP(hipGetLastError());
    return PGV_OK;
}

int launch_shadow_pairs(pgv_ctx *ctx, const RowGeom &g32, const void *queries, const void *centers,
                        const int64_t *pair_start, int nlists, int64_t npairs, ScanPair *pairs) {
    if (npairs <= 0) return PGV_OK;
    hipLaunchKernelGGL(shadow_pair_kernel, dim3((unsigned)((npairs + 3) / 4)), dim3(256), 0, ctx->stream,
                       static_cast<const float *>(queries), static_cast<const float *>(centers), pair_start, nlists, npairs,
                       g32.ld, pairs);
    PGV_HIP(hipGetLastError());
    return PGV_OK;
}

}
```

pgvector_amd/csrc/pgv_abi_ivf.hip:

```cpp
#include "pgv_abi_common.h"

extern "C" {


namespace {
struct IndexLayout {
    size_t centers, vectors, offsets, tids, row_norms, center_norms, bytes;
    bool has_tids, has_norms;
};
IndexLayout index_layout(int nlists, int64_t n, size_t row_bytes, bool has_tids, bool l2) {
    auto up = [](size_t v) { return (v + 255) & ~(size_t)255; };
    IndexLayout L{};
    size_t at = 0;
    L.centers = at; at = up(at + (size_t)nlists * row_bytes);
    L.vectors = at; at = up(at + (size_t)(n > 0 ? n : 1) * row_bytes);
    L.offsets = at; at = up(at + sizeof(int64_t) * ((size_t)nlists + 1));
    L.has_tids = has_tids;
    L.tids = at; if (has_tids) at = up(at + sizeof(uint64_t) * (size_t)n);
    L.has_norms = l2;
    L.row_norms = at; if (l2 && n > 0) at = up(at + sizeof(float) * ((size_t)n + 1));
    L.center_norms = at; if (l2) at = up(at + sizeof(float) * ((size_t)nlists + 1));
    L.bytes = at;
    return L;
}
void index_carve(pgv_index *ix, const IndexLayout &L) {
    char *b = static_cast<char *>(ix->arena);
    ix->centers = b + L.centers;
    ix->vectors = b + L.vectors;
    ix->list_offsets = reinterpret_cast<int64_t *>(b + L.offsets);
    ix->tids = L.has_tids ? reinterpret_cast<uint64_t *>(b + L.tids) : nullptr;
    ix->row_norms = L.has_norms && ix->nrows > 0 ? reinterpret_cast<float *>(b + L.row_norms) : nullptr;
    ix->center_norms = L.has_norms ? reinterpret_cast<float *>(b + L.center_norms) : nullptr;
}
void index_host_tables(pgv_index *ix) {
    const int nlists = ix->nlists;
    std::vector<int64_t> lens((size_t)nlists);
    int64_t maxlen = 0;
    for (int l = 0; l < nlists; l++) {
        lens[l] = ix->h_offsets[l + 1] - ix->h_offsets[l];
        if (lens[l] > maxlen) maxlen = lens[l];
    }
    ix->max_list_len = maxlen;
    std::sort(lens.begin(), lens.end(), [](int64_t a, int64_t b) { return a > b; });
    ix->len_prefix.assign((size_t)nlists + 1, 0);
    for (int l = 0; l < nlists; l++) ix->len_prefix[l + 1] = ix->len_prefix[l] + lens[l];
}
}

extern "C++" {
namespace {

int shadow_env() {
    const char *e = getenv("PGV_SCAN_SHADOW");
    return e ? atoi(e) : -1;
}

int rank_shadow_env() {
    const char *e = getenv("PGV_RANK_SHADOW");
    return e ? atoi(e) : 1;
}

int shadow_create(pgv_ctx *ctx, pgv_index *ix) {
    const int env = shadow_env();
    if (env == 0 || ix->metric != PGV_L2SQ || ix->dtype != PGV_F32 || ix->nrows <= 0 || !ix->row_norms || !ix->center_norms)
        return PGV_OK;
    if (env < 0 && !rows_stream_past_caches(ix->geom, ix->dtype, ix->nrows)) return PGV_OK;
    const RowGeom g16 = row_geom(ix->dim, PGV_F16);
    const size_t bytes = ((size_t)ix->nrows * g16.ld * sizeof(uint16_t) + 255) & ~(size_t)255;
    const size_t cbytes = ((size_t)ix->nlists * g16.ld * sizeof(uint16_t) + 255) & ~(size_t)255;
    void *sh = nullptr;
    if (hipMalloc(&sh, bytes + 256 + cbytes) != hipSuccess) {
        (void)hipGetLastError();
        return PGV_OK;
    }
    void *words = static_cast<char *>(sh) + bytes;
    void *csh = static_cast<char *>(sh) + bytes + 256;
    int rc = launch_shadow_build(ctx, ix->geom, g16, ix->vectors, ix->centers, ix->list_offsets, ix->nlists, ix->nrows, sh,
                                 words);
    if (rc == PGV_OK)
        rc = launch_shadow_build(ctx, ix->geom, g16, ix->centers, nullptr, nullptr, 0, ix->nlists, csh,
                                 static_cast<char *>(words) + 32);
    unsigned char h[56];
    if (rc == PGV_OK && (hipStreamSynchronize(ctx->stream) != hipSuccess ||
                         hipMemcpy(h, words, sizeof(h), hipMemcpyDeviceToHost) != hipSuccess)) {
        set_error("shadow build failed: %s", hipGetErrorString(hipGetLastError()));
        rc = PGV_ERR_DEVICE;
    }
    if (rc != PGV_OK) {
        (void)hipFree(sh);
        return rc;
    }
    float max_abs;
    double e2, p2;
    memcpy(&max_abs, h, 4);
    memcpy(&e2, h + 8, 8);
    memcpy(&p2, h + 16, 8);
    const double P = std::sqrt(p2), E = std::sqrt(e2);
    if (!std::isfinite(E) || !std::isfinite(P) || !std::isfinite(max_abs)) {
        (void)hipFree(sh);
        return PGV_OK;
    }
    ix->shadow = sh;
    ix->shadow_geom = g16;
    ix->shadow_s = shadow_scale_of(max_abs);
    ix->shadow_E = (E + 1e-12 * (P + E)) * (1.0 + 1e-9);
    ix->shadow_P = P * (1.0 + 1e-9);
    float cmax_abs;
    double ce2, cp2;
    memcpy(&cmax_abs, h + 32, 4);
    memcpy(&ce2, h + 40, 8);
    memcpy(&cp2, h + 48, 8);
    const double Pc = std::sqrt(cp2), Ec = std::sqrt(ce2);
    if (std::isfinite(Ec) && std::isfinite(Pc) && std::isfinite(cmax_abs)) {
        ix->cshadow = csh;
        ix->cshadow_s = shadow_scale_of(cmax_abs);
        ix->cshadow_E = (Ec + 1e-12 * (Pc + Ec)) * (1.0 + 1e-9);
        ix->cshadow_P = Pc * (1.0 + 1e-9);
    }
    return PGV_OK;
}

struct ShadowBatch {
    void *qcast = nullptr;
    float *qscale = nullptr, *qeps = nullptr;
    float *cscale = nullptr, *ceps = nullptr;
    float *pair_t = nullptr;
    bool scan_follows = false;
    bool cast_for_scan = false, cast_for_rank = false, pairs_done = false;
};

int shadow_batch_cast(pgv_index *ix, const void *q_dev, int nq, int probes, bool for_rank, bool for_scan, ShadowBatch *sb) {
    pgv_ctx *ctx = ix->ctx;
    const RowGeom &g16 = ix->shadow_geom;
    const size_t qb = ((size_t)nq * g16.ld * sizeof(uint16_t) + 255) & ~(size_t)255;
    PGV_TRY(ctx->sh_q.ensure(qb + sizeof(float) * (size_t)nq * (4 + (size_t)probes)));
    sb->qcast = ctx->sh_q.p;
    sb->qscale = reinterpret_cast<float *>(ctx->sh_q.as<char>() + qb);
    sb->qeps = sb->qscale + nq;
    sb->cscale = sb->qeps + nq;
    sb->ceps = sb->cscale + nq;
    sb->pair_t = sb->ceps + nq;
    constexpr double u = 5.9604644775390625e-8;
    ShadowTerms st{};
    st.s = ix->shadow_s;
    st.E = ix->shadow_E;
    st.P = ix->shadow_P;
    st.g_dot = gamma_n(shadow_chain_length(g16) + 4.0, u);
    st.g_pair = gamma_n((double)pair_chain_length(ix->geom), u);
    st.g_cn = gamma_n(ix->geom.ld / 64.0 + 10.0, u);
    RankShadowTerms rt{};
    rt.s = ix->cshadow_s;
    rt.E = ix->cshadow_E;
    rt.P = ix->cshadow_P;
    rt.g_dot = st.g_dot;
    rt.g_cn = st.g_cn;
    PGV_TRY(launch_shadow_query(ctx, ix->geom, g16, q_dev, nq, st, rt, ix->center_norms + ix->nlists,
                                ix->row_norms + ix->nrows, sb->qcast, for_scan ? sb->qscale : nullptr,
                                for_scan ? sb->qeps : nullptr, for_rank ? sb->cscale : nullptr,
                                for_rank ? sb->ceps : nullptr));
    sb->cast_for_scan = for_scan;
    sb->cast_for_rank = for_rank;
    return PGV_OK;
}

bool shadow_scan_expected(const pgv_index *ix, int nq, int probes, int k) {
    const double share = (double)nq * probes / (double)ix->nlists;
    const bool small = (share <= 0.4 || nq <= 4) && nq <= 1024 && probes <= query_max_batch_lists() && k <= query_head_cap();
    return !small && share > 3.0 && k <= 192 && !ix->ctx->no_mfma_scan && ix->metric == PGV_L2SQ && ix->row_norms &&
           ix->shadow && shadow_env() != 0;
}

template <typename Fill>
int index_create(pgv_ctx *ctx, pgv_metric metric, pgv_dtype dtype, int dim, int nlists, const std::vector<int64_t> &off,
                 bool has_tids, Fill fill, pgv_index **out) {
    const int64_t n = off[nlists];
    pgv_index *ix = new (std::nothrow) pgv_index();
    if (!ix) PGV_FAIL(PGV_ERR_NOMEM, "out of host memory");
    ix->ctx = ctx;
    ix->refs = new (std::nothrow) int(1);
    if (!ix->refs) {
        delete ix;
        PGV_FAIL(PGV_ERR_NOMEM, "out of host memory");
    }
    ix->metric = metric;
    ix->dtype = dtype;
    ix->dim = dim;
    ix->nlists = nlists;
    ix->nrows = n;
    ix->geom = row_geom(dim, dtype);
    ix->h_offsets = off;
    index_host_tables(ix);
    const size_t row_bytes = (size_t)ix->geom.ld * elem_size(dtype);

    auto fail = [&](int rc) {
        pgv_index_free(ix);
        return rc;
    };
    IndexLayout lay = index_layout(nlists, n, row_bytes, has_tids && n > 0, metric == PGV_L2SQ);
    if (malloc_exportable(&ix->arena, lay.bytes) != hipSuccess) {
        (void)hipGetLastError();
        set_error("hipMalloc(%zu) for the index mirror failed", lay.bytes);
        return fail(PGV_ERR_NOMEM);
    }
    ix->arena_bytes = lay.bytes;
    index_carve(ix, lay);
    int rc;
    if ((rc = fill(ix)) != PGV_OK) return fail(rc);
    if (hipMemcpyAsync(ix->list_offsets, ix->h_offsets.data(), sizeof(int64_t) * off.size(),
                       hipMemcpyHostToDevice, ctx->stream) != hipSuccess)
        return fail((set_error("copy of list_offsets failed"), PGV_ERR_DEVICE));
    if (ix->row_norms) {
        if (hipMemsetAsync(ix->row_norms + n, 0, sizeof(float), ctx->stream) != hipSuccess)
            return fail((set_error("memset of row_norms failed"), PGV_ERR_DEVICE));
        if ((rc = launch_row_norms(ctx, dtype, ix->geom, ix->vectors, n, ix->row_norms,
                                   reinterpret_cast<unsigned *>(ix->row_norms + n))) != PGV_OK)
            return fail(rc);
    }
    if (ix->center_norms) {
        if (hipMemsetAsync(ix->center_norms + nlists, 0, sizeof(float), ctx->stream) != hipSuccess)
            return fail((set_error("memset of center_norms failed"), PGV_ERR_DEVICE));
        if ((rc = launch_row_norms(ctx, dtype, ix->geom, ix->centers, nlists, ix->center_norms,
                                   reinterpret_cast<unsigned *>(ix->center_norms + nlists))) != PGV_OK)
            return fail(rc);
    }
    if ((rc = shadow_create(ctx, ix)) != PGV_OK) return fail(rc);
    if (hipStreamSynchronize(ctx->stream) != hipSuccess)
        return fail((set_error("index upload failed: %s", hipGetErrorString(hipGetLastError())), PGV_ERR_DEVICE));
    *out = ix;
    return PGV_OK;
}

int put_rows_on(hipStream_t stream, const RowGeom &g, pgv_dtype dtype, int dim, void *dst, const void *src, int64_t rows) {
    if (rows == 0) return PGV_OK;
    const size_t es = elem_size(dtype), row_bytes = (size_t)g.ld * es;
    const bool dev = is_device_ptr(src);
    if (g.ld == dim) {
        PGV_HIP(hipMemcpyAsync(dst, src, (size_t)rows * row_bytes, dev ? hipMemcpyDeviceToDevice : hipMemcpyHostToDevice,
                               stream));
    } else {
        PGV_HIP(hipMemsetAsync(dst, 0, (size_t)rows * row_bytes, stream));
        PGV_HIP(hipMemcpy2DAsync(dst, row_bytes, src, (size_t)dim * es, (size_t)dim * es, (size_t)rows,
                                 dev ? hipMemcpyDeviceToDevice : hipMemcpyHostToDevice, stream));
    }
    return PGV_OK;
}

int put_rows(pgv_ctx *ctx, const RowGeom &g, pgv_dtype dtype, int dim, void *dst, const void *src, int64_t rows) {
    return put_rows_on(ctx->stream, g, dtype, dim, dst, src, rows);
}

}
}

int pgv_index_upload(pgv_ctx *ctx, pgv_metric metric, pgv_dtype dtype, int dim, int nlists,
                     const void *centers, const int64_t *list_offsets, const void *vectors,
                     const uint64_t *tids, pgv_index **out) {
    if (!ctx || !out) PGV_FAIL(PGV_ERR_ARG, "pgv_index_upload: ctx/out is NULL");
    *out = nullptr;
    PGV_TRY(check_common(dtype, dim));
    PGV_TRY(check_metric(metric));
    if (nlists < 1 || nlists > 32768) PGV_FAIL(PGV_ERR_ARG, "lists %d outside 1..32768", nlists);
    if (!centers || !list_offsets) PGV_FAIL(PGV_ERR_ARG, "centers/list_offsets is NULL");
    PGV_HIP(hipSetDevice(ctx->device));

    std::vector<int64_t> off((size_t)nlists + 1);
    if (is_device_ptr(list_offsets)) {
        PGV_HIP(hipMemcpy(off.data(), list_offsets, sizeof(int64_t) * off.size(), hipMemcpyDeviceToHost));
    } else {
        memcpy(off.data(), list_offsets, sizeof(int64_t) * off.size());
    }
    if (off[0] != 0) PGV_FAIL(PGV_ERR_ARG, "list_offsets[0] must be 0");
    for (int l = 0; l < nlists; l++)
        if (off[l + 1] < off[l]) PGV_FAIL(PGV_ERR_ARG, "list_offsets not ascending at list %d", l);
    const int64_t n = off[nlists];
    if (n > 0 && !vectors) PGV_FAIL(PGV_ERR_ARG, "vectors is NULL");
    return index_create(ctx, metric, dtype, dim, nlists, off, tids != nullptr, [&](pgv_index *ix) -> int {
        PGV_TRY(put_rows(ctx, ix->geom, dtype, dim, ix->centers, centers, nlists));
        PGV_TRY(put_rows(ctx, ix->geom, dtype, dim, ix->vectors, vectors, n));
        if (ix->tids)
            PGV_HIP(hipMemcpyAsync(ix->tids, tids, sizeof(uint64_t) * (size_t)n,
                                   is_device_ptr(tids) ? hipMemcpyDeviceToDevice : hipMemcpyHostToDevice, ctx->stream));
// ... 374 lines not shown
        PGV_FAIL(PGV_ERR_STATE, "pgv_index_import: the handle was exported by this process (use pgv_index_share)");
    if (w.device != ctx->device)
        PGV_FAIL(PGV_ERR_ARG, "pgv_index_import: the index lives on device %d, the context on %d", w.device, ctx->device);
    PGV_TRY(check_common((pgv_dtype)w.dtype, w.dim));
    PGV_TRY(check_metric((pgv_metric)w.metric));
    if (w.nlists < 1 || w.nlists > 32768 || w.nrows < 0) PGV_FAIL(PGV_ERR_ARG, "pgv_index_import: corrupt handle");
    PGV_HIP(hipSetDevice(ctx->device));
    pgv_index *ix = new (std::nothrow) pgv_index();
    if (!ix) PGV_FAIL(PGV_ERR_NOMEM, "out of host memory");
    ix->refs = new (std::nothrow) int(1);
    if (!ix->refs) {
        delete ix;
        PGV_FAIL(PGV_ERR_NOMEM, "out of host memory");
    }
    ix->ctx = ctx;
    ix->metric = (pgv_metric)w.metric;
    ix->dtype = (pgv_dtype)w.dtype;
    ix->dim = w.dim;
    ix->nlists = w.nlists;
    ix->nrows = w.nrows;
    ix->geom = row_geom(w.dim, ix->dtype);
    ix->imported = true;
    const size_t row_bytes = (size_t)ix->geom.ld * elem_size(ix->dtype);
    IndexLayout lay = index_layout(w.nlists, w.nrows, row_bytes, w.has_tids != 0, ix->metric == PGV_L2SQ);
    if (lay.bytes != w.arena_bytes) {
        pgv_index_free(ix);
        PGV_FAIL(PGV_ERR_ARG, "pgv_index_import: handle describes %llu bytes, this library lays the mirror out in %zu",
                 (unsigned long long)w.arena_bytes, lay.bytes);
    }
    hipError_t e = hipIpcOpenMemHandle(&ix->arena, w.mem, hipIpcMemLazyEnablePeerAccess);
    if (e != hipSuccess) {
        (void)hipGetLastError();
        ix->arena = nullptr;
        pgv_index_free(ix);
        PGV_FAIL(PGV_ERR_DEVICE, "hipIpcOpenMemHandle failed: %s (is the exporting process alive, and "
                 "HSA_ENABLE_IPC_MODE_LEGACY=0 set in both?)", hipGetErrorString(e));
    }
    ix->arena_bytes = lay.bytes;
    index_carve(ix, lay);
    ix->h_offsets.assign((size_t)w.nlists + 1, 0);
    if (hipMemcpy(ix->h_offsets.data(), ix->list_offsets, sizeof(int64_t) * ix->h_offsets.size(),
                  hipMemcpyDeviceToHost) != hipSuccess) {
        set_error("pgv_index_import: reading list_offsets failed: %s", hipGetErrorString(hipGetLastError()));
        pgv_index_free(ix);
        return PGV_ERR_DEVICE;
    }
    if (ix->h_offsets[0] != 0 || ix->h_offsets[w.nlists] != w.nrows) {
        pgv_index_free(ix);
        PGV_FAIL(PGV_ERR_DATA, "pgv_index_import: the shared mirror does not match its handle");
    }
    index_host_tables(ix);
    *out = ix;
    return PGV_OK;
}

static void index_drop_lanes(pgv_index *ix) {
    for (pgv_index *v : ix->lanes) {
        pgv_ctx *lc = v->ctx;
        if (ix->ctx) {
            auto &ch = ix->ctx->children;
            ch.erase(std::remove(ch.begin(), ch.end(), lc), ch.end());
        }
        pgv_index_free(v);
        pgv_ctx_destroy(lc);
    }
    ix->lanes.clear();
    if (ix->lane_event) (void)hipEventDestroy(ix->lane_event);
    ix->lane_event = nullptr;
    if (ix->lane_scan_done) (void)hipEventDestroy(ix->lane_scan_done);
    ix->lane_scan_done = nullptr;
}

void pgv_index_free(pgv_index *ix) {
    if (!ix) return;
    if (!ix->lanes.empty()) index_drop_lanes(ix);
    if (ix->ctx) (void)hipStreamSynchronize(ix->ctx->stream);
    if (ix->refs && __atomic_sub_fetch(ix->refs, 1, __ATOMIC_ACQ_REL) > 0) {
        delete ix;
        return;
    }
    if (ix->arena) {
        if (ix->imported)
            (void)hipIpcCloseMemHandle(ix->arena);
        else
            (void)hipFree(ix->arena);
    }
    if (ix->shadow) (void)hipFree(ix->shadow);
    delete ix->refs;
    delete ix;
}

int pgv_index_tids(pgv_index *ix, const int64_t *slots, int64_t n, uint64_t *out) {
    if (!ix || !out || (n > 0 && !slots)) PGV_FAIL(PGV_ERR_ARG, "pgv_index_tids: index/slots/out is NULL");
    if (!ix->tids) PGV_FAIL(PGV_ERR_STATE, "pgv_index_tids: the index was uploaded without tids");
    if (is_device_ptr(slots) || is_device_ptr(out)) PGV_FAIL(PGV_ERR_ARG, "pgv_index_tids: host arrays only");
    PGV_HIP(hipSetDevice(ix->ctx->device));
    int64_t i = 0;
    while (i < n) {
        if (slots[i] < 0 || slots[i] >= ix->nrows) PGV_FAIL(PGV_ERR_ARG, "pgv_index_tids: slot %lld out of range", (long long)slots[i]);
        int64_t j = i + 1;
        while (j < n && slots[j] == slots[j - 1] + 1) j++;
        if (slots[j - 1] >= ix->nrows) PGV_FAIL(PGV_ERR_ARG, "pgv_index_tids: slot %lld out of range", (long long)slots[j - 1]);
        PGV_HIP(hipMemcpyAsync(out + i, ix->tids + slots[i], sizeof(uint64_t) * (size_t)(j - i), hipMemcpyDeviceToHost,
                               ix->ctx->stream));
        i = j;
    }
    PGV_HIP(hipStreamSynchronize(ix->ctx->stream));
    return PGV_OK;
}

int64_t pgv_index_rows(const pgv_index *ix) { return ix ? ix->nrows : -1; }
int pgv_index_lists(const pgv_index *ix) { return ix ? ix->nlists : -1; }



static int rank_lists_impl(pgv_index *ix, const void *q_dev, int nq, int maxprobes,
                           int32_t *out_lists_dev, float *out_dist_dev, ShadowBatch *sb) {
    pgv_ctx *ctx = ix->ctx;
    PGV_TRY(ctx->dist_mat.ensure(sizeof(float) * (size_t)nq * ix->nlists));
    float *mat = ctx->dist_mat.as<float>();
    PGV_TRY(ctx->sel_a.ensure(sizeof(int64_t) * (size_t)nq * maxprobes));
    float *dist = out_dist_dev;
    if (!dist) {
        PGV_TRY(ctx->sel_b.ensure(sizeof(float) * (size_t)nq * maxprobes));
        dist = ctx->sel_b.as<float>();
    }
    int64_t *pos = ctx->sel_a.as<int64_t>();
    if (nq <= 24 && maxprobes <= query_head_cap()) {
        const int64_t cd_stride = ((int64_t)ix->nlists + 7) / 4 * 4;
        PGV_TRY(ctx->dist_mat.ensure(sizeof(float) * (size_t)nq * cd_stride));
        return launch_multi_rank(ctx, ix, q_dev, nq, ctx->dist_mat.as<float>(), cd_stride, maxprobes, out_lists_dev,
                                 out_dist_dev);
    }
    int cand = maxprobes + 16 < ix->nlists ? maxprobes + 16 : ix->nlists;
    const int rank_env = rank_shadow_env();
    const bool rank_sh = ix->metric == PGV_L2SQ && ix->cshadow && ix->dtype == PGV_F32 && rank_env != 0 && shadow_env() != 0;
    if (rank_sh && maxprobes + 54 <= 256) cand = maxprobes + 54 < ix->nlists ? maxprobes + 54 : ix->nlists;
    const bool mfma = nq >= 128 && ix->nlists >= 64 && !ctx->no_mfma_scan &&
                      (ix->metric == PGV_NEG_IP || (ix->metric == PGV_L2SQ && ix->center_norms && cand <= 256));
    if (mfma && ix->metric == PGV_L2SQ) {
        ApproxScratch sc;
        PGV_TRY(sc.carve(ctx, ctx->ms_b, nq, cand));
        ShadowBatch own;
        if (!sb) sb = &own;
        const bool scan_follows = sb->scan_follows;
        if (rank_sh) {
            PGV_TRY(shadow_batch_cast(ix, q_dev, nq, maxprobes, true, scan_follows, sb));
            PGV_TRY(dense_scan(ctx, ix->metric, PGV_F16, ix->shadow_geom, ix->cshadow, ix->nlists, sb->qcast, nq, ix->nlists,
                               mat, true, ix->center_norms, nullptr, sb->cscale));
        } else {
            PGV_TRY(dense_scan(ctx, ix->metric, ix->dtype, ix->geom, ix->centers, ix->nlists, q_dev, nq, ix->nlists, mat,
                               true, ix->center_norms, nullptr));
        }
        PGV_TRY(launch_topk_segments(ctx, mat, nullptr, nq, ix->nlists, cand, sc.cand_val, sc.cand_pos, sc.flags + nq));
        const ExactRows xr{ix->centers, nullptr, nullptr, ix->geom, ix->dtype,
                           reinterpret_cast<const unsigned *>(ix->center_norms + ix->nlists)};
        ScanBound bound = scan_bound_chain(ctx, ix->geom.ld, scan_chain_length(ix->geom, ix->dtype, false));
        if (rank_sh)
            bound = {0.f, 0.f, gamma_n(ix->geom.ld / 64.0 + 10.0, 5.9604645e-8), bound.g_ref};
        float *pair_t = (rank_sh && rank_env == 1 && scan_follows) ? sb->pair_t : nullptr;
        PGV_TRY(launch_batch_recheck(ctx, xr, q_dev, nq, cand, maxprobes, sc.cand_val, sc.cand_pos, sc.cand_pos, nullptr,
                                     ix->nlists, bound, dist, nullptr, nullptr, sc.flags,
                                     out_lists_dev, nullptr, nullptr, 0, rank_sh ? sb->ceps : nullptr, pair_t));
        PGV_TRY(launch_batch_fix(ctx, xr, q_dev, nq, nullptr, nullptr, 0, nullptr, ix->nlists, sc.flags, mat, maxprobes,
                                 bound, dist, nullptr, nullptr, out_lists_dev, rank_sh ? sb->ceps : nullptr, pair_t));
        sb->pairs_done = pair_t != nullptr;
        return PGV_OK;
    } else {
        PGV_TRY(dense_scan(ctx, ix->metric, ix->dtype, ix->geom, ix->centers, ix->nlists, q_dev, nq, ix->nlists, mat,
                           mfma, nullptr, nullptr));
        PGV_TRY(launch_topk_segments(ctx, mat, nullptr, nq, ix->nlists, maxprobes, dist, pos));
    }
    PGV_TRY(launch_cast_pos_to_i32(ctx, pos, (int64_t)nq * maxprobes, out_lists_dev));
    return PGV_OK;
}

int rank_lists_dev(pgv_index *ix, const void *q_dev, int nq, int maxprobes, int32_t *out_lists_dev, float *out_dist_dev) {
    return rank_lists_impl(ix, q_dev, nq, maxprobes, out_lists_dev, out_dist_dev, nullptr);
}

int pgv_rank_lists(pgv_index *ix, const void *queries, int nq, int maxprobes, int32_t *out_lists,
                   float *out_dist) {
    if (!ix || !out_lists) PGV_FAIL(PGV_ERR_ARG, "pgv_rank_lists: index/out_lists is NULL");
    if (nq < 0) PGV_FAIL(PGV_ERR_ARG, "nq < 0");
    if (maxprobes < 1 || maxprobes > ix->nlists)
        PGV_FAIL(PGV_ERR_ARG, "maxprobes %d outside 1..lists (%d)", maxprobes, ix->nlists);
    if (nq == 0) return PGV_OK;
    if (!queries) PGV_FAIL(PGV_ERR_ARG, "queries is NULL");
    pgv_ctx *ctx = ix->ctx;
    PGV_HIP(hipSetDevice(ctx->device));
    const void *q_dev;
    PGV_TRY(stage_rows(ctx, queries, nq, ix->dim, ix->dtype, ix->geom, ctx->q_stage, &q_dev));
    OutArg ol, od;
    PGV_TRY(ol.init(out_lists, sizeof(int32_t) * (size_t)nq * maxprobes, ctx->out_stage));
    PGV_TRY(od.init(out_dist, sizeof(float) * (size_t)nq * maxprobes, ctx->out_stage2));
    PGV_TRY(rank_lists_dev(ix, q_dev, nq, maxprobes, ol.as<int32_t>(), od.as<float>()));
    bool need = false;
    PGV_TRY(ol.finish(ctx, &need));
    PGV_TRY(od.finish(ctx, &need));
    return sync_if(ctx, need);
}

int pgv_scan_lists(pgv_index *ix, const void *query, const int32_t *lists, int nlists,
                   float *out_dist, int64_t *out_slot, int64_t capacity, int64_t *out_count) {
    if (!ix || !out_count) PGV_FAIL(PGV_ERR_ARG, "pgv_scan_lists: index/out_count is NULL");
    if (nlists < 0 || (nlists > 0 && !lists)) PGV_FAIL(PGV_ERR_ARG, "bad list array");
    pgv_ctx *ctx = ix->ctx;
    PGV_HIP(hipSetDevice(ctx->device));

    std::vector<int32_t> hl((size_t)nlists);
    if (nlists) {
        if (is_device_ptr(lists))
            PGV_HIP(hipMemcpy(hl.data(), lists, sizeof(int32_t) * (size_t)nlists, hipMemcpyDeviceToHost));
        else
            memcpy(hl.data(), lists, sizeof(int32_t) * (size_t)nlists);
    }
    int64_t m = 0;
    for (int p = 0; p < nlists; p++) {
        if (hl[p] < 0 || hl[p] >= ix->nlists) PGV_FAIL(PGV_ERR_ARG, "list id %d out of range", hl[p]);
        m += ix->h_offsets[hl[p] + 1] - ix->h_offsets[hl[p]];
    }
    *out_count = m;
    if (m > capacity) PGV_FAIL(PGV_ERR_ARG, "output capacity %lld < %lld tuples", (long long)capacity, (long long)m);
    if (m == 0) return PGV_OK;
    if (!out_dist || !out_slot) PGV_FAIL(PGV_ERR_ARG, "out_dist/out_slot is NULL");

    OutArg od, os;
    PGV_TRY(od.init(out_dist, sizeof(float) * (size_t)m, ctx->out_stage));
    PGV_TRY(os.init(out_slot, sizeof(int64_t) * (size_t)m, ctx->out_stage2));

    const int ch = rows_per_task_for(ctx, m, 1);
    int64_t ntasks = 0;
    for (int p = 0; p < nlists; p++) {
        int64_t len = ix->h_offsets[hl[p] + 1] - ix->h_offsets[hl[p]];
        ntasks += (len + ch - 1) / ch;
    }
    const size_t tb = sizeof(ScanTask) * (size_t)ntasks, pb = sizeof(ScanPair) * (size_t)nlists,
                 ob = sizeof(int64_t) * (size_t)nlists, lb = sizeof(int32_t) * (size_t)nlists;
    PGV_TRY(staging_acquire(ctx));
    PGV_TRY(ctx->h_a.ensure(tb + pb + ob + lb + 16));
    char *hb = ctx->h_a.as<char>();
    ScanTask *ht = reinterpret_cast<ScanTask *>(hb);
    ScanPair *hp = reinterpret_cast<ScanPair *>(hb + tb);
    int64_t *hoff = reinterpret_cast<int64_t *>(hb + tb + pb);
    int32_t *hlist = reinterpret_cast<int32_t *>(hb + tb + pb + ob);
    int *hn = reinterpret_cast<int *>(hb + tb + pb + ob + lb);
    int64_t t = 0, run = 0;
    for (int p = 0; p < nlists; p++) {
        const int64_t beg = ix->h_offsets[hl[p]], len = ix->h_offsets[hl[p] + 1] - beg;
        hp[p].out_rel = run - beg;
        hp[p].query = 0;
        hp[p].pad = 0;
        hoff[p] = run;
        hlist[p] = hl[p];
        for (int64_t c = 0; c * ch < len; c++) {
            ht[t].row0 = beg + c * ch;
            int64_t left = len - c * ch;
            ht[t].nrows = (int)(left < ch ? left : ch);
            ht[t].pair0 = p;
            ht[t].npairs = 1;
            ht[t].pad = 0;
            t++;
        }
        run += len;
    }
    *hn = (int)ntasks;
    const size_t total = tb + pb + ob + lb + 16;
    PGV_TRY(ctx->tasks.ensure(total));
    PGV_HIP(hipMemcpyAsync(ctx->tasks.p, hb, total, hipMemcpyHostToDevice, ctx->stream));
    char *db = ctx->tasks.as<char>();

    PGV_TRY(launch_iota_slots(ctx, ix, reinterpret_cast<int32_t *>(db + tb + pb + ob), nlists,
                              reinterpret_cast<int64_t *>(db + tb + pb), os.as<int64_t>()));
    if (query == nullptr) {
        PGV_HIP(hipMemsetAsync(od.dev, 0, sizeof(float) * (size_t)m, ctx->stream));
    } else {
        const void *q_dev;
        PGV_TRY(stage_rows(ctx, query, 1, ix->dim, ix->dtype, ix->geom, ctx->q_stage, &q_dev));
        ScanTimer timer{ctx};
        PGV_TRY(timer.begin((double)m, (double)m));
        PGV_TRY(launch_scan(ctx, ix->metric, ix->dtype, ix->geom, ix->vectors, q_dev,
                            reinterpret_cast<ScanTask *>(db), reinterpret_cast<int *>(db + tb + pb + ob + lb),
                            (int)ntasks, reinterpret_cast<ScanPair *>(db + tb), 1, od.as<float>()));
        PGV_TRY(timer.end());
    }
    bool need = true;
    PGV_TRY(od.finish(ctx, &need));
    PGV_TRY(os.finish(ctx, &need));
    return sync_if(ctx, need);
}


static int scan_turn_begin(pgv_ctx *ctx) {
    if (ctx->scan_gate) PGV_HIP(hipStreamWaitEvent(ctx->stream, ctx->scan_gate, 0));
    return PGV_OK;
}
static int scan_turn_end(pgv_ctx *ctx) {
    if (ctx->scan_gate) PGV_HIP(hipEventRecord(ctx->scan_gate, ctx->stream));
    return PGV_OK;
}

static int scan_batch_impl(pgv_index *ix, const void *q_dev, int nq, const int32_t *probe_lists, int probes,
                           int k, float *out_dist, int64_t *out_slot, uint64_t *out_tid, ShadowBatch *sb) {
    pgv_ctx *ctx = ix->ctx;
    const double share = (double)nq * probes / (double)ix->nlists;
    if ((share <= 0.4 || nq <= 4) && nq <= 1024 && probes <= query_max_batch_lists() && k <= query_head_cap()) {
        const int64_t bound = ix->len_prefix[probes];
        const int64_t seg_stride = (bound + 7) / 4 * 4;
        PGV_TRY(ctx->plan_d.ensure(sizeof(float) * (size_t)nq * seg_stride));
        OutArg od, os, ot;
        PGV_TRY(od.init(out_dist, sizeof(float) * (size_t)nq * k, ctx->out_stage));
        PGV_TRY(os.init(out_slot, sizeof(int64_t) * (size_t)nq * k, ctx->out_stage2));
        PGV_TRY(ot.init(out_tid, sizeof(uint64_t) * (size_t)nq * k, ctx->sel_b));
        PGV_TRY(scan_turn_begin(ctx));
        ScanTimer timer{ctx};
        PGV_TRY(timer.begin(0.0, 0.0));
        PGV_TRY(launch_multi_scan(ctx, ix, q_dev, nq, probe_lists, probes, bound, ctx->plan_d.as<float>(), seg_stride, k,
                                  od.as<float>(), os.as<int64_t>(), ot.as<uint64_t>()));
        PGV_TRY(timer.end());
        PGV_TRY(scan_turn_end(ctx));
        bool need = false;
        PGV_TRY(od.finish(ctx, &need));
        PGV_TRY(os.finish(ctx, &need));
        PGV_TRY(ot.finish(ctx, &need));
        return sync_if(ctx, need);
    }
    const bool use_mfma = share > 3.0 && k <= 192 && !ctx->no_mfma_scan &&
                          (ix->metric == PGV_NEG_IP || (ix->metric == PGV_L2SQ && ix->row_norms));
    const bool use_tile = !use_mfma && tile_scan_supported(ix->geom) && share > 8.0;
    static const int wide_env = [] {
        const char *e = getenv("PGV_SCAN_WIDE");
        return e ? atoi(e) : -1;
    }();
    const bool wide = use_mfma && (wide_env < 0 ? share > 12.0 : wide_env != 0);
    const int qt = use_mfma ? (wide ? mfma_scan_queries_per_task_wide() : mfma_scan_queries_per_task())
                            : (use_tile ? tile_scan_queries_per_task()
                                        : scan_group_size(ix->geom, ix->dtype, (int)std::ceil(share)));
    constexpr int rpt_tiles = 20;
    const int rows_per_task = use_mfma ? mfma_scan_rows_per_task()
                                       : (use_tile ? rpt_tiles * tile_scan_tile_rows(ix->geom)
                                                   : (qt >= 16 ? 256 : (qt >= 4 ? 128 : 64)));
    const bool approx = use_mfma && ix->metric == PGV_L2SQ;
    const bool shadow = approx && ix->shadow && shadow_env() != 0;
    ShadowBatch own;
    if (!sb) sb = &own;
    if (shadow && !sb->cast_for_scan) PGV_TRY(shadow_batch_cast(ix, q_dev, nq, probes, false, true, sb));
    const float *pair_t = (shadow && sb->pairs_done) ? sb->pair_t : nullptr;
    PlanResult plan;
    PGV_TRY(launch_plan_batch(ctx, ix, probe_lists, nq, probes, qt, rows_per_task, ctx->profiling, &plan, pair_t));

    int kprime = k;
    ApproxScratch sc;
    if (approx) {
        kprime = approx_candidates(k);
        PGV_TRY(sc.carve(ctx, ctx->ms_a, nq, kprime));
    }
    float *cand_val = sc.cand_val;
    int64_t *cand_pos = sc.cand_pos;
    int32_t *flags = sc.flags;
    void *qcast = nullptr;
    float *qscale = nullptr, *qeps = nullptr;
    if (shadow) {
        qcast = sb->qcast;
        qscale = sb->qscale;
        qeps = sb->qeps;
        if (!pair_t)
            PGV_TRY(launch_shadow_pairs(ctx, ix->geom, q_dev, ix->centers, plan.pair_start, ix->nlists, (int64_t)nq * probes,
                                        plan.pairs));
        ctx->scan_shadow_queries += nq;
    }

    PGV_TRY(ctx->plan_d.ensure(sizeof(float) * (size_t)(plan.out_bound > 0 ? plan.out_bound : 1)));
    float *seg_vals = ctx->plan_d.as<float>();
    if (plan.ntasks_bound > 0) {
        PGV_TRY(scan_turn_begin(ctx));
        ScanTimer timer{ctx};
        PGV_TRY(timer.begin(0.0, 0.0));
        if (shadow)
            PGV_TRY(launch_mfma_scan(ctx, ix->metric, PGV_F16, ix->shadow_geom, ix->shadow, qcast, plan.tasks,
                                     plan.ntasks_dev, (int)plan.ntasks_bound, plan.pairs, ix->row_norms, nullptr,
                                     seg_vals, rows_stream_past_caches(ix->shadow_geom, PGV_F16, ix->nrows), qt, qscale));
        else if (use_mfma)
            PGV_TRY(launch_mfma_scan(ctx, ix->metric, ix->dtype, ix->geom, ix->vectors, q_dev, plan.tasks,
                                     plan.ntasks_dev, (int)plan.ntasks_bound, plan.pairs, ix->row_norms, nullptr,
                                     seg_vals, rows_stream_past_caches(ix->geom, ix->dtype, ix->nrows), qt));
        else if (use_tile)
            PGV_TRY(launch_tile_scan(ctx, ix->metric, ix->dtype, ix->geom, ix->vectors, q_dev, plan.tasks,
                                     plan.ntasks_dev, (int)plan.ntasks_bound, plan.pairs, seg_vals));
        else
            PGV_TRY(launch_scan(ctx, ix->metric, ix->dtype, ix->geom, ix->vectors, q_dev, plan.tasks,
                                plan.ntasks_dev, (int)plan.ntasks_bound, plan.pairs, qt, seg_vals));
        PGV_TRY(timer.end());
        PGV_TRY(scan_turn_end(ctx));
    }

    OutArg od, os, ot;
    PGV_TRY(od.init(out_dist, sizeof(float) * (size_t)nq * k, ctx->out_stage));
    PGV_TRY(os.init(out_slot, sizeof(int64_t) * (size_t)nq * k, ctx->out_stage2));
    PGV_TRY(ot.init(out_tid, sizeof(uint64_t) * (size_t)nq * k, ctx->sel_b));
    PGV_TRY(ctx->sel_a.ensure(sizeof(int64_t) * (size_t)nq * k));
    int64_t *pos = ctx->sel_a.as<int64_t>();
    if (approx) {
        ScanBound gamma = scan_bound_chain(ctx, ix->geom.ld, scan_chain_length(ix->geom, ix->dtype, wide));
        if (shadow)
            gamma = {0.f, 0.f, gamma_n(ix->geom.ld / 64.0 + 10.0, 5.9604645e-8), gamma.g_ref};
        PGV_TRY(launch_topk_segments(ctx, seg_vals, plan.seg_start, nq, 0, kprime, cand_val, cand_pos, flags + nq));
        const ExactRows xr{ix->vectors, ix->tids, ix->list_offsets, ix->geom, ix->dtype,
                           reinterpret_cast<const unsigned *>(ix->row_norms + ix->nrows)};
        PGV_TRY(launch_batch_recheck(ctx, xr, q_dev, nq, kprime, k, cand_val, cand_pos, nullptr, plan.seg_start, 0,
                                     gamma, od.as<float>(), os.as<int64_t>(), ot.as<uint64_t>(), flags, nullptr,
                                     probe_lists, plan.probe_off, probes, qeps));
        PGV_TRY(launch_batch_fix(ctx, xr, q_dev, nq, probe_lists, plan.probe_off, probes, plan.seg_start, 0, flags,
                                 seg_vals, k, gamma, od.as<float>(), os.as<int64_t>(), ot.as<uint64_t>(), nullptr, qeps));
    } else {
        PGV_TRY(launch_topk_segments(ctx, seg_vals, plan.seg_start, nq, 0, k, od.as<float>(), pos));
        PGV_TRY(launch_positions_to_slots(ctx, ix, probe_lists, plan.probe_off, nq, probes, k, pos,
                                          os.as<int64_t>(), ot.as<uint64_t>()));
    }
    bool need = false;
    PGV_TRY(od.finish(ctx, &need));
    PGV_TRY(os.finish(ctx, &need));
    PGV_TRY(ot.finish(ctx, &need));
    return sync_if(ctx, need);
}

int scan_batch_dev(pgv_index *ix, const void *q_dev, int nq, const int32_t *probe_lists, int probes, int k, float *out_dist,
                   int64_t *out_slot, uint64_t *out_tid) {
    return scan_batch_impl(ix, q_dev, nq, probe_lists, probes, k, out_dist, out_slot, out_tid, nullptr);
}

int check_batch_args(pgv_index *ix, const void *queries, int nq, int probes, int k, float *out_dist,
                            uint64_t *out_tid, const char *who) {
    if (!ix) PGV_FAIL(PGV_ERR_ARG, "%s: index is NULL", who);
    if (nq < 0 || k < 1) PGV_FAIL(PGV_ERR_ARG, "bad nq/k");
    if (probes < 1 || probes > ix->nlists)
        PGV_FAIL(PGV_ERR_ARG, "probes %d outside 1..lists (%d)", probes, ix->nlists);
    if (out_tid && !ix->tids) PGV_FAIL(PGV_ERR_STATE, "index was uploaded without tids");
    if (nq > 0 && (!queries || !out_dist)) PGV_FAIL(PGV_ERR_ARG, "queries/out_dist is NULL");
    return PGV_OK;
}

int pgv_search_batch(pgv_index *ix, const void *queries, int nq, int probes, int k, float *out_dist,
                     int64_t *out_slot, uint64_t *out_tid) {
    PGV_TRY(check_batch_args(ix, queries, nq, probes, k, out_dist, out_tid, "pgv_search_batch"));
    if (nq == 0) return PGV_OK;
    if (!ix->lanes.empty()) {
        pgv_index *lane = ix->lanes[ix->lane_next++ % ix->lanes.size()];
        PGV_HIP(hipSetDevice(ix->ctx->device));
        PGV_HIP(hipEventRecord(ix->lane_event, ix->ctx->stream));
        PGV_HIP(hipStreamWaitEvent(lane->ctx->stream, ix->lane_event, 0));
        return pgv_search_batch(lane, queries, nq, probes, k, out_dist, out_slot, out_tid);
    }
    pgv_ctx *ctx = ix->ctx;
    PGV_HIP(hipSetDevice(ctx->device));
    const void *q_dev;
    PGV_TRY(stage_rows(ctx, queries, nq, ix->dim, ix->dtype, ix->geom, ctx->q_stage, &q_dev));
    PGV_TRY(ctx->idx_stage.ensure(sizeof(int32_t) * (size_t)nq * probes));
    int32_t *probe_lists = ctx->idx_stage.as<int32_t>();
    ShadowBatch sb;
    sb.scan_follows = shadow_scan_expected(ix, nq, probes, k);
    PGV_TRY(rank_lists_impl(ix, q_dev, nq, probes, probe_lists, nullptr, &sb));
    return scan_batch_impl(ix, q_dev, nq, probe_lists, probes, k, out_dist, out_slot, out_tid, &sb);
}

int pgv_scan_batch(pgv_index *ix, const void *queries, int nq, const int32_t *probe_lists, int probes, int k,
                   float *out_dist, int64_t *out_slot, uint64_t *out_tid) {
    PGV_TRY(check_batch_args(ix, queries, nq, probes, k, out_dist, out_tid, "pgv_scan_batch"));
    if (nq == 0) return PGV_OK;
    if (!probe_lists) PGV_FAIL(PGV_ERR_ARG, "probe_lists is NULL");
    pgv_ctx *ctx = ix->ctx;
    PGV_HIP(hipSetDevice(ctx->device));
    if (!is_device_ptr(probe_lists)) {
        for (size_t i = 0; i < (size_t)nq * probes; i++)
            if (probe_lists[i] < 0 || probe_lists[i] >= ix->nlists)
                PGV_FAIL(PGV_ERR_ARG, "probe list id %d out of range 0..%d", probe_lists[i], ix->nlists - 1);
    }
    const void *q_dev, *pl_dev;
    PGV_TRY(stage_rows(ctx, queries, nq, ix->dim, ix->dtype, ix->geom, ctx->q_stage, &q_dev));
    PGV_TRY(stage_flat(ctx, probe_lists, sizeof(int32_t) * (size_t)nq * probes, ctx->idx_stage, &pl_dev));
    return scan_batch_dev(ix, q_dev, nq, static_cast<const int32_t *>(pl_dev), probes, k, out_dist, out_slot,
                          out_tid);
}

namespace {

struct QueryHeadHost {
    long long total;
    int count;
    unsigned seq;
};

static int g_scan_gate_width = -1;
static PgvGate g_scan_gate;
static void scan_gate_enter() {
    if (g_scan_gate_width < 0) {
        const char *e = getenv("PGV_MAX_INFLIGHT_SCANS");
        __atomic_store_n(&g_scan_gate_width, e ? atoi(e) : 16, __ATOMIC_RELAXED);
    }
    g_scan_gate.enter(g_scan_gate_width);
}
static void scan_gate_leave() { g_scan_gate.leave(g_scan_gate_width); }
struct ScanGate {
    ScanGate() { scan_gate_enter(); }
    ~ScanGate() { scan_gate_leave(); }
};

int wait_head(pgv_ctx *ctx, pgv_query *q, unsigned seq) {
    volatile QueryHeadHost *h = static_cast<volatile QueryHeadHost *>(q->head_pinned);
    for (int spin = 0; spin < 200000; spin++) {
        if (__atomic_load_n(&h->seq, __ATOMIC_ACQUIRE) == seq) return PGV_OK;
        __builtin_ia32_pause();
    }
    PGV_HIP(hipStreamSynchronize(ctx->stream));
    if (__atomic_load_n(&h->seq, __ATOMIC_ACQUIRE) != seq) PGV_FAIL(PGV_ERR_DEVICE, "query kernel did not report");
    return PGV_OK;
}

void copy_head(pgv_query *q, int stride, int n, float *out_dist, int64_t *out_slot, uint64_t *out_tid) {
    const char *base = static_cast<const char *>(q->head_pinned) + 64;
    if (out_slot) memcpy(out_slot, base, sizeof(int64_t) * (size_t)n);
    if (out_tid) memcpy(out_tid, base + (size_t)stride * 8, sizeof(uint64_t) * (size_t)n);
    if (out_dist) memcpy(out_dist, base + (size_t)stride * 16, sizeof(float) * (size_t)n);
}

}

static bool query_direct_enabled() {
    static const bool on = [] {
        const char *e = getenv("PGV_QUERY_DIRECT");
        return !(e && e[0] == '0');
    }();
    return on;
}

int pgv_query_begin(pgv_index *ix, pgv_query **out) {
    if (!ix || !out) PGV_FAIL(PGV_ERR_ARG, "pgv_query_begin: index/out is NULL");
    *out = nullptr;
    pgv_ctx *ctx = ix->ctx;
    PGV_HIP(hipSetDevice(ctx->device));
    pgv_query *q = new (std::nothrow) pgv_query();
    if (!q) PGV_FAIL(PGV_ERR_NOMEM, "out of host memory");
    q->ix = ix;
    const int cap = query_head_cap();
    const size_t state_bytes = sizeof(int32_t) * (size_t)cap + sizeof(float) * ((size_t)ix->nlists + 4);
    const size_t row_bytes = (size_t)ix->geom.ld * elem_size(ix->dtype);
    q->head_bytes = query_head_bytes(cap);
    int rc = q->state.ensure(state_bytes);
    if (rc == PGV_OK) rc = q->q_dev.ensure(row_bytes);
    if (rc == PGV_OK && hipHostMalloc(&q->q_pinned, row_bytes, hipHostMallocDefault) != hipSuccess) rc = PGV_ERR_NOMEM;
    if (rc == PGV_OK && hipHostMalloc(&q->head_pinned, q->head_bytes, hipHostMallocDefault) != hipSuccess)
        rc = PGV_ERR_NOMEM;
    if (rc == PGV_OK && hipMemsetAsync(q->state.p, 0, state_bytes, ctx->stream) != hipSuccess) rc = PGV_ERR_DEVICE;
    int large_bar = 0;
    if (rc == PGV_OK && query_direct_enabled() &&
        hipDeviceGetAttribute(&large_bar, hipDeviceAttributeIsLargeBar, ctx->device) == hipSuccess && large_bar) {
        if (hipExtMallocWithFlags(&q->q_direct, row_bytes, hipDeviceMallocFinegrained) != hipSuccess) {
            (void)hipGetLastError();
            q->q_direct = nullptr;
        }
    }
    if (rc != PGV_OK) {
        set_error("pgv_query_begin: allocation failed");
        pgv_query_end(q);
        return rc;
    }
    memset(q->head_pinned, 0, q->head_bytes);
    q->lists = q->state.as<int32_t>();
    q->cdist = reinterpret_cast<float *>(q->lists + cap);
    *out = q;
    return PGV_OK;
}

void pgv_query_end(pgv_query *q) {
    if (!q) return;
    if (q->ix && q->ix->ctx) (void)hipStreamSynchronize(q->ix->ctx->stream);
    q->state.release();
    q->seg.release();
    q->q_dev.release();
    if (q->q_pinned) (void)hipHostFree(q->q_pinned);
    if (q->q_direct) (void)hipFree(q->q_direct);
    if (q->head_pinned) (void)hipHostFree(q->head_pinned);
    delete q;
}

int pgv_query_rank(pgv_query *q, const void *query, int max_probes) {
    if (!q) PGV_FAIL(PGV_ERR_ARG, "pgv_query_rank: q is NULL");
    pgv_index *ix = q->ix;
    pgv_ctx *ctx = ix->ctx;
    if (max_probes < 1 || max_probes > ix->nlists)
        PGV_FAIL(PGV_ERR_ARG, "maxprobes %d outside 1..lists (%d)", max_probes, ix->nlists);
    if (max_probes > query_head_cap())
        PGV_FAIL(PGV_ERR_ARG, "pgv_query_rank handles up to %d probes; use pgv_rank_lists", query_head_cap());
    PGV_HIP(hipSetDevice(ctx->device));
    q->max_probes = max_probes;
    q->is_null = query == nullptr;
    q->cur_n = 0;
    if (q->is_null) return launch_query_iota(ctx, q->lists, max_probes);
    const size_t es = elem_size(ix->dtype);
    const size_t row_bytes = (size_t)ix->geom.ld * es;
    if (is_device_ptr(query)) {
        PGV_HIP(hipMemsetAsync(q->q_dev.p, 0, row_bytes, ctx->stream));
        PGV_HIP(hipMemcpyAsync(q->q_dev.p, query, (size_t)ix->dim * es, hipMemcpyDeviceToDevice, ctx->stream));
        q->q_row = q->q_dev.p;
    } else {
        if (q->rank_pending) PGV_HIP(hipStreamSynchronize(ctx->stream));
        void *dst = q->q_direct ? q->q_direct : q->q_pinned;
        memcpy(dst, query, (size_t)ix->dim * es);
        if (row_bytes > (size_t)ix->dim * es) memset(static_cast<char *>(dst) + (size_t)ix->dim * es, 0, row_bytes - (size_t)ix->dim * es);
        if (q->q_direct) {
            __builtin_ia32_sfence();
            q->q_row = q->q_direct;
        } else {
            PGV_TRY(launch_query_stage(ctx, q->q_pinned, q->q_dev.p, ix->geom.nvec));
            q->q_row = q->q_dev.p;
        }
    }
    q->rank_pending = true;
    return launch_query_rank(ctx, ix, q->q_row, q->cdist, max_probes, q->lists);
}

int pgv_query_scan(pgv_query *q, int first, int nprobes, int head, float *out_dist, int64_t *out_slot,
                   uint64_t *out_tid, int *out_count, int64_t *out_total) {
    if (!q || !out_count) PGV_FAIL(PGV_ERR_ARG, "pgv_query_scan: q/out_count is NULL");
    pgv_index *ix = q->ix;
    pgv_ctx *ctx = ix->ctx;
    if (q->max_probes <= 0) PGV_FAIL(PGV_ERR_STATE, "pgv_query_scan before pgv_query_rank");
    if (first < 0 || nprobes < 1 || first + nprobes > q->max_probes)
        PGV_FAIL(PGV_ERR_ARG, "lists [%d, %d) outside the %d ranked", first, first + nprobes, q->max_probes);
    if (nprobes > query_max_batch_lists())
        PGV_FAIL(PGV_ERR_ARG, "pgv_query_scan handles up to %d lists per batch; use pgv_scan_lists", query_max_batch_lists());
    if (head < 1 || head > query_head_cap()) PGV_FAIL(PGV_ERR_ARG, "head %d outside 1..%d", head, query_head_cap());
    if (out_tid && !ix->tids) PGV_FAIL(PGV_ERR_STATE, "index was uploaded without tids");
    PGV_HIP(hipSetDevice(ctx->device));
    const int64_t bound = ix->len_prefix[nprobes];
    PGV_TRY(q->seg.ensure(sizeof(float) * (size_t)(bound + 4)));
    const unsigned seq = ++q->seq ? q->seq : ++q->seq;
// ... 50 lines not shown
```

pgvector_amd/csrc/pgv_internal.h:

```cpp
#pragma once

#include <hip/hip_runtime.h>

#include <cstdint>
#include <cstdio>
#include <cstdlib>
#include <cstring>
#include <cmath>
#include <vector>

#include "../../include/pgv_hip.h"

namespace pgv {

void set_error(const char *fmt, ...) __attribute__((format(printf, 1, 2)));

#define PGV_FAIL(code, ...)            \
    do {                               \
        ::pgv::set_error(__VA_ARGS__); \
        return (code);                 \
    } while (0)

#define PGV_HIP(call)                                                                  \
    do {                                                                               \
// ... 239 lines not shown
    constexpr double v = 5.9604645e-8;
    return {0.f, gamma_n(dim / 4.0 + 4.0, v), gamma_n(dim / 64.0 + 10.0, v), 2.f * gamma_n(dim + 2.0, v)};
}
inline ScanBound scan_bound_chain(const pgv_ctx *ctx, int dim, int chain) {
    ScanBound b = scan_bound(ctx, dim);
    if (ctx->bound_mode != 0) b.g_dot = gamma_n(chain + 4.0, 5.9604645e-8);
    return b;
}
struct ExpansionBound {
    float gamma;
    float gamma_exact;
};
inline ExpansionBound argmin_bound(const pgv_ctx *ctx, int dim) {
    constexpr float u = 5.9604645e-8f;
    if (ctx->assign_bound_mode == 0) return {8.f * std::sqrt((float)dim + 4.f) * u, 0.f};
    const float n1 = (float)(dim + 1) * u, n2 = (float)(dim + 2) * u;
    return {n1 / (1.f - n1), n2 / (1.f - n2)};
}

int launch_scan(pgv_ctx *ctx, pgv_metric metric, pgv_dtype dtype, const RowGeom &g,
                const void *rows, const void *queries, const ScanTask *tasks,
                const int *ntasks_dev, int ntasks_bound, const ScanPair *pairs, int qt,
                float *out);
int scan_group_size(const RowGeom &g, pgv_dtype dtype, int wanted);
int launch_expand_groups(pgv_ctx *ctx, const int32_t *ids, const int64_t *ids_start, const int32_t *from,
                         const int64_t *pair_start, int ngroups, int32_t *a, int32_t *b);
int launch_score_gather(pgv_ctx *ctx, pgv_metric metric, pgv_dtype dtype, const RowGeom &g,
                        const void *rows, const void *queries, const int32_t *slot,
                        const int32_t *query_of, int64_t npairs, float *out);
int launch_score_groups(pgv_ctx *ctx, pgv_metric metric, pgv_dtype dtype, const RowGeom &g, const void *rows,
                        const int32_t *ids, const int64_t *ids_at, int64_t ids_stride, const int32_t *n_arr,
                        const int32_t *from_arr, const int64_t *pair_at, int ngroups, float *out);

int launch_cosine(pgv_ctx *ctx, pgv_dtype dtype, const RowGeom &g, const void *rows, const void *query, int64_t n,
                  double *out);
int launch_bit_distance(pgv_ctx *ctx, int mode, const RowGeom &g, const void *rows, const void *query, int64_t n,
                        double *out);

int hnsw_search_grid(pgv_ctx *ctx, int nq, int64_t n, int *words_out);
struct HnswSearchArgs {
    const void *queries = nullptr;
    const int32_t *qids = nullptr;
    const int32_t *qlevels = nullptr;
    int nq = 0, ef = 0, k = 0;
    int64_t *out_elem = nullptr;
    float *out_dist = nullptr;
    int64_t *out_scored = nullptr;
    int32_t *lw_ids = nullptr;
    float *lw_dist = nullptr;
    int32_t *lw_cnt = nullptr;
    int lcap = 0;
};
int launch_hnsw_search(pgv_ctx *ctx, pgv_metric metric, pgv_dtype dtype, const RowGeom &geom, const void *rows,
                       int64_t n, const int32_t *levels, const int64_t *nbr_start, const int32_t *nbr, int m,
                       int32_t entry, const HnswSearchArgs &a, uint32_t *bitmaps, int words, int grid, int *counter);
int launch_hnsw_patch(pgv_ctx *ctx, int32_t *nbr, const int64_t *nbr_start, int64_t n, const int32_t *ids,
                      const int64_t *packed_off, const int32_t *packed, int nupd);

bool tile_scan_supported(const RowGeom &g);
int tile_scan_queries_per_task();
int tile_scan_tile_rows(const RowGeom &g);
int launch_tile_scan(pgv_ctx *ctx, pgv_metric metric, pgv_dtype dtype, const RowGeom &g,
                     const void *rows, const void *queries, const ScanTask *tasks,
                     const int *ntasks_dev, int ntasks_bound, const ScanPair *pairs, float *out);

int launch_argmin(pgv_ctx *ctx, pgv_metric metric, pgv_dtype dtype, const RowGeom &g,
                  const void *rows, int64_t n, const void *centers, int k, int32_t *out_idx,
                  float *out_val);
int launch_argmin_mode(pgv_ctx *ctx, int mode, pgv_dtype dtype, const RowGeom &g,
                       const void *rows, int64_t n, const void *centers, int k,
                       int32_t *out_idx, float *out_val);

int launch_argmin_listed(pgv_ctx *ctx, int mode, pgv_dtype dtype, const RowGeom &g, const void *rows, int64_t n,
                         const void *centers, int k, const int32_t *row_list, const int *row_count,
                         unsigned long long *packed);
int launch_hnsw_select_plan(pgv_ctx *ctx, const int32_t *cnt, int ngroups, int lcap, int m, int64_t *pair_start);
int launch_hnsw_select_pairs(pgv_ctx *ctx, const int32_t *lw_ids, const int32_t *cnt, const int64_t *pair_start, int ngroups,
                             int ef, int32_t *a, int32_t *b);
int launch_hnsw_select(pgv_ctx *ctx, const int32_t *lw_ids, const float *lw_dist, const int32_t *cnt, const int32_t *qlevels,
                       const int64_t *pair_start, const float *tri, int ngroups, int lcap, int ef, int m, int stride,
                       int32_t *out_ids, float *out_dist, uint8_t *out_closer, int32_t *out_cnt);
int launch_hnsw_link_group(pgv_ctx *ctx, int step, const int32_t *elems, const uint8_t *linked, int nq, int lcap, int m,
                           const int32_t *sel_ids, const float *sel_dist, const int32_t *sel_cnt, const int32_t *levels,
                           const int64_t *nbr_start, int *list_count, int *list_rec, int *nrec, int32_t *rec_owner,
                           int32_t *rec_lc, int32_t *rec_list, const int64_t *rec_off, int *rec_fill, int32_t *link_elem,
                           float *link_dist);
int launch_hnsw_link_size(pgv_ctx *ctx, const int32_t *nbr, const uint8_t *nb_flag, const int32_t *levels,
                          const int64_t *nbr_start, int m, const int32_t *rec_owner, const int32_t *rec_lc,
                          const int32_t *rec_list, const int *list_count, int64_t *rec_off, int nrec, int pass, int64_t *rec_pos,
                          int32_t *rec_nstart, int32_t *rec_from, const int32_t *rec_wait, int64_t *size_ids,
                          int64_t *size_pairs);
int launch_hnsw_link_scan(pgv_ctx *ctx, int64_t *a, int64_t *b, int64_t *c, int n, int64_t *totals);
int launch_hnsw_link_stats(pgv_ctx *ctx, const int *blocked, const int64_t *totals, int64_t *stats);
int launch_hnsw_link_pairs(pgv_ctx *ctx, const int32_t *nbr, const int64_t *rec_pos, const int32_t *rec_nstart,
                           const int32_t *rec_from, const int64_t *rec_off, int32_t *link_elem, float *link_dist,
                           const int32_t *rec_list, int *list_count, int nrec, int pass,
                           const int64_t *ids_start, int32_t *ids, const int64_t *pair_start, int32_t *a, int32_t *b);
int launch_hnsw_link_replay(pgv_ctx *ctx, int32_t *nbr, float *nb_dist, uint8_t *nb_flag, int m, int nrec, int pass,
                            const int32_t *rec_lc, const int64_t *rec_off, const float *link_dist, const int64_t *rec_pos,
                            const int32_t *rec_nstart, const int32_t *rec_from, const int64_t *ids_start, const int32_t *ids,
                            const int64_t *pair_start, const float *tri, const int64_t *mm_start, const float *mm,
                            int32_t *rec_wait, int16_t *loc_save, int *blocked);
int launch_hnsw_link_new(pgv_ctx *ctx, int32_t *nbr, float *nb_dist, uint8_t *nb_flag, const int32_t *levels,
                         const int64_t *nbr_start, int m, const int32_t *elems, const uint8_t *linked, int nq, int lcap,
                         const int32_t *sel_ids, const float *sel_dist, const uint8_t *sel_closer, const int32_t *sel_cnt);
bool mfma_argmin_supported(int mode, int64_t n, int k);
int launch_argmin_mfma(pgv_ctx *ctx, int mode, pgv_dtype dtype, const RowGeom &g, const void *rows, int64_t n,
                       const void *centers, int k, int32_t *out_idx, float *out_val);

int mfma_scan_rows_per_task();
int mfma_scan_queries_per_task();
int launch_mfma_dense(pgv_ctx *ctx, pgv_metric metric, pgv_dtype dtype, const RowGeom &g, const void *rows, int64_t n,
                      const void *queries, int nq, const float *row_norms, float *out, int64_t out_stride);
int dense_chain_length(const RowGeom &g, pgv_dtype dtype);
int launch_row_norms(pgv_ctx *ctx, pgv_dtype dtype, const RowGeom &g, const void *rows, int64_t n, float *out,
                     unsigned *max_bits);
int launch_mfma_scan(pgv_ctx *ctx, pgv_metric metric, pgv_dtype dtype, const RowGeom &g, const void *rows,
                     const void *queries, const ScanTask *tasks, const int *ntasks_dev, int ntasks_bound,
                     const ScanPair *pairs, const float *row_norms, const float *query_norms, float *out, bool stream_rows,
                     int queries_per_task = 32, const float *shadow_scale = nullptr);
int launch_shadow_build(pgv_ctx *ctx, const RowGeom &g32, const RowGeom &g16, const void *rows, const void *centers,
                        const int64_t *list_off, int nlists, int64_t n, void *shadow, void *words);
int shadow_scale_of(float max_abs);
int shadow_chain_length(const RowGeom &g16);
int scan_chain_length(const RowGeom &g, pgv_dtype dtype, bool wide);
int launch_shadow_query(pgv_ctx *ctx, const RowGeom &g32, const RowGeom &g16, const void *queries, int nq,
                        const ShadowTerms &st, const RankShadowTerms &rt, const float *center_norm_max,
                        const float *row_norm_max, void *qcast, float *qscale, float *qeps, float *cscale, float *ceps);
int launch_shadow_pairs(pgv_ctx *ctx, const RowGeom &g32, const void *queries, const void *centers,
                        const int64_t *pair_start, int nlists, int64_t npairs, ScanPair *pairs);
int mfma_scan_queries_per_task_wide();

int launch_gather_words(pgv_ctx *ctx, const void *src, int words_per_row, int64_t nrows, const int64_t *idx, int n,
                        uint32_t *out);
size_t build_sort_scratch_bytes(int64_t n, int key_bits);
int launch_build_order(pgv_ctx *ctx, const int32_t *lists, int64_t n, int nlists, unsigned long long *keys_tmp,
                       unsigned long long *keys_sorted, unsigned long long *counts, int64_t *offsets, int *bad,
                       void *sort_scratch, size_t sort_scratch_bytes);
int launch_build_gather(pgv_ctx *ctx, const void *src_rows, const unsigned long long *keys_sorted, int64_t n, int nvec,
                        void *dst_rows, const uint64_t *src_tids, uint64_t *dst_tids);

struct PlanResult {
    ScanTask *tasks = nullptr;
    ScanPair *pairs = nullptr;
    int *ntasks_dev = nullptr;
    int64_t ntasks = 0;
    int64_t total_out = 0;
    int64_t ntasks_bound = 0;
    int64_t out_bound = 0;
    int64_t *seg_start = nullptr;
    int64_t *probe_off = nullptr;
    int64_t *pair_start = nullptr;
};
int launch_plan_batch(pgv_ctx *ctx, const pgv_index *ix, const int32_t *probe_lists, int nq,
                      int probes, int qt, int rows_per_task, bool read_totals, PlanResult *res,
                      const float *pair_t = nullptr);
int launch_topk_segments(pgv_ctx *ctx, const float *vals, const int64_t *seg_start, int nseg,
                         int64_t fixed_len, int k, float *out_val, int64_t *out_pos, int32_t *zero_word = nullptr);
int launch_positions_to_slots(pgv_ctx *ctx, const pgv_index *ix, const int32_t *probe_lists,
                              const int64_t *probe_off, int nq, int probes, int k,
                              const int64_t *pos, int64_t *out_slot, uint64_t *out_tid);
struct ExactRows {
    const void *vectors;
    const uint64_t *tids;
    const int64_t *list_offsets;
    pgv::RowGeom geom;
    pgv_dtype dtype;
    const unsigned *norm_max;
};
int launch_batch_recheck(pgv_ctx *ctx, const ExactRows &xr, const void *q_dev, int nq, int kprime, int k,
                         const float *approx_val, const int64_t *cand_pos, const int64_t *cand_slot,
                         const int64_t *seg_start, int64_t fixed_len, const ScanBound &bound,
                         float *out_dist, int64_t *out_slot, uint64_t *out_tid, int32_t *flags,
                         int32_t *out_i32 = nullptr, const int32_t *probe_lists = nullptr,
                         const int64_t *probe_off = nullptr, int probes = 0,
                         const float *eps_add = nullptr,
                         float *pair_t = nullptr);
int launch_batch_fix(pgv_ctx *ctx, const ExactRows &xr, const void *q_dev, int nq, const int32_t *probe_lists,
                     const int64_t *probe_off, int probes, const int64_t *seg_start, int64_t fixed_len,
                     const int32_t *flags, float *seg_vals, int k, const ScanBound &bound, float *out_dist, int64_t *out_slot,
                     uint64_t *out_tid, int32_t *out_i32 = nullptr, const float *eps_add = nullptr,
                     float *pair_t = nullptr);
int launch_iota_slots(pgv_ctx *ctx, const pgv_index *ix, const int32_t *lists_dev, int nlists,
                      const int64_t *probe_off, int64_t *out_slot);

int query_max_batch_lists();
int query_head_cap();
size_t query_head_bytes(int head);
int launch_query_stage(pgv_ctx *ctx, const void *src_pinned, void *dst_dev, int nvec);
int launch_multi_rank(pgv_ctx *ctx, const pgv_index *ix, const void *q_dev, int nq, float *cdist, int64_t cd_stride,
                      int max_probes, int32_t *out_lists, float *out_dist);
int launch_multi_scan(pgv_ctx *ctx, const pgv_index *ix, const void *q_dev, int nq, const int32_t *probe_lists, int nprobes,
                      int64_t rows_bound, float *seg, int64_t seg_stride, int k, float *out_dist, int64_t *out_slot,
                      uint64_t *out_tid);
int launch_query_iota(pgv_ctx *ctx, int32_t *out, int n);
int launch_one_query_rows(pgv_ctx *ctx, pgv_metric metric, pgv_dtype dtype, const RowGeom &g, const void *rows, int n,
                          const void *q_dev, float *out);
int launch_query_rank(pgv_ctx *ctx, const pgv_index *ix, const void *q_dev, float *cdist, int max_probes,
                      int32_t *out_lists);
int launch_query_scan(pgv_ctx *ctx, const pgv_index *ix, const void *q_dev, const int32_t *probe_lists, int nprobes,
                      int64_t rows_bound, float *seg);
int launch_query_head(pgv_ctx *ctx, const pgv_index *ix, const float *seg, const int32_t *probe_lists, int nprobes,
                      int skip, int count, void *head_rec, unsigned seq);

int launch_merge_heads(pgv_ctx *ctx, const float *dist_all, const uint64_t *tid_all, int nranks, int nq, int k,
                       float *out_dist, uint64_t *out_tid);

int launch_cast_pos_to_i32(pgv_ctx *ctx, const int64_t *pos, int64_t n, int32_t *out);

int kmpp_block_count(int n);
int launch_kmpp_update(pgv_ctx *ctx, const float *raw, float *weight, int n, int spherical,
                       double *block_sums);
int launch_kmpp_pick(pgv_ctx *ctx, const RowGeom &g, const void *samples, int n,
                     const float *weight, const double *block_sums, const double *draws,
                     int round, void *centers, int32_t *picked);
int launch_kmpp_total(pgv_ctx *ctx, const double *block_sums, int nblocks, double *out);
int launch_kmpp_pick_sharded(pgv_ctx *ctx, const RowGeom &g, const void *samples, int n, const float *weight,
                             const double *block_sums, const double *totals, const int64_t *counts, int nranks, int rank,
                             const double *draws, int round, void *send_row, int32_t *owner_out);
int launch_kmpp_take_row(pgv_ctx *ctx, const RowGeom &g, const void *gathered, const int32_t *owner, void *centers,
                         int round);
int launch_lloyd_pack(pgv_ctx *ctx, const int32_t *counts, const unsigned long long *changes, int k, float *tail);
int launch_lloyd_unpack(pgv_ctx *ctx, const float *tail, int k, int32_t *counts, unsigned long long *changes,
                        long long *host_rec, long long seq);
int launch_changes_hist(pgv_ctx *ctx, const int32_t *closest_new, int32_t *closest_io, int n,
                        int32_t *counts, unsigned long long *changes);
int launch_members(pgv_ctx *ctx, const int32_t *closest, int n, int k, const int32_t *counts,
                   int32_t *offsets, int32_t *members);
int launch_center_sums(pgv_ctx *ctx, pgv_dtype dtype, const RowGeom &g, const void *samples,
                       const int32_t *offsets, const int32_t *members, int k, float *sums);
int launch_finish_centers(pgv_ctx *ctx, pgv_dtype dtype, const RowGeom &g, int k, int dim,
                          const float *sums, const int32_t *counts, const float *refill,
                          const int32_t *refill_row, void *centers);
int launch_normalize_rows(pgv_ctx *ctx, pgv_dtype dtype, const RowGeom &g, void *rows, int64_t n,
                          int dim, int32_t *flag);
int launch_check_centers(pgv_ctx *ctx, pgv_dtype dtype, const RowGeom &g, const void *centers,
                         int k, int dim, int check_zero_norm, int32_t *flag);

}
```

Measured before the change: 1.332 million.

## Fuse scan-plan counting into rank recheck and merge plan pair/task kernels

The rank recheck and fix kernels now emit the scan plan's per-list counts, per-probe offsets and segment lengths while they write the pair terms. The later plan stage can then skip its counting pass when the batch shape matches. The top-k kernel zeroes the count buffers, and the pair and task planning kernels are merged into a single launch. This adds atomics and branches to the recheck kernels and a new shadow-cast export entry point, in exchange for fewer launches and passes between ranking and scanning.

```diff
diff --git a/include/pgv_hip.h b/include/pgv_hip.h
--- a/include/pgv_hip.h
+++ b/include/pgv_hip.h
@@ -122,6 +122,9 @@
 int			pgv_search_batch(pgv_index * index, const void *queries, int nq, int probes, int k,
 							 float *out_dist, int64_t *out_slot, uint64_t *out_tid);
 
+int			pgv_index_shadow_cast(pgv_index * index, const void *queries, int nq, void *out_qcast, float *out_qscale,
+								  float *out_qeps, float *out_cscale, float *out_ceps);
+
 int			pgv_scan_batch(pgv_index * index, const void *queries, int nq, const int32_t *probe_lists,
 						   int probes, int k, float *out_dist, int64_t *out_slot, uint64_t *out_tid);
 
diff --git a/pgvector_amd/_lib.py b/pgvector_amd/_lib.py
--- a/pgvector_amd/_lib.py
+++ b/pgvector_amd/_lib.py
@@ -30,7 +30,7 @@
     "pgv_device_memory", "pgv_pinned_register", "pgv_pinned_unregister", "pgv_index_export", "pgv_index_import",
     "pgv_index_tids", "pgv_hnsw_export", "pgv_hnsw_import", "pgv_hnsw_share", "pgv_hnsw_device", "pgv_exact_topk", "pgv_ctx_set_bound",
     "pgv_hnsw_upload_payload", "pgv_hnsw_get_payload", "pgv_builder_begin", "pgv_builder_add", "pgv_builder_set_centers", "pgv_builder_rows", "pgv_builder_finish", "pgv_builder_free", "pgv_index_drain",
-    "pgv_index_set_overlap",
+    "pgv_index_set_overlap", "pgv_index_shadow_cast",
 ]
 
 
@@ -95,6 +95,7 @@
     lib.pgv_index_free.argtypes = [P]
     lib.pgv_index_share.argtypes = [P, P, C.POINTER(P)]
     lib.pgv_index_set_overlap.argtypes = [P, I]
+    lib.pgv_index_shadow_cast.argtypes = [P, P, I, P, P, P, P, P]
     lib.pgv_index_free.restype = None
     lib.pgv_index_export.argtypes = [P, P]
     lib.pgv_index_import.argtypes = [P, P, C.POINTER(P)]
diff --git a/pgvector_amd/csrc/kernels_query.hip b/pgvector_amd/csrc/kernels_query.hip
--- a/pgvector_amd/csrc/kernels_query.hip
+++ b/pgvector_amd/csrc/kernels_query.hip
@@ -338,7 +338,7 @@
     const int64_t *__restrict__ seg_start, int64_t fixed_len,
     const unsigned *__restrict__ row_norm_max, ScanBound bound, const float *__restrict__ eps_add, int nq,
     float *__restrict__ out_dist, int64_t *__restrict__ out_slot, uint64_t *__restrict__ out_tid,
-    int32_t *__restrict__ out_i32, int32_t *__restrict__ flags, float *__restrict__ pair_t) {
+    int32_t *__restrict__ out_i32, int32_t *__restrict__ flags, float *__restrict__ pair_t, PlanEmit emit) {
     static_assert(!DOT || std::is_same<T, float>::value, "pair terms: fp32 rows");
     __shared__ float exact[kRecheckCap];
     __shared__ float dots[DOT ? kRecheckCap : 1];
@@ -436,6 +436,23 @@
         if (out_tid) out_tid[o] = ~0ull;
         if constexpr (DOT) pair_t[o] = 0.f;
     }
+    if constexpr (DOT) {
+        if (emit.cnt) {
+            __syncthreads();
+            if ((int)threadIdx.x < cnt && rank < k) {
+                atomicAdd(&emit.cnt[my_slot], 1);
+                slots[rank] = emit.list_off[my_slot + 1] - emit.list_off[my_slot];
+            }
+            if ((int)threadIdx.x >= kk && (int)threadIdx.x < k) slots[threadIdx.x] = 0;
+            __syncthreads();
+            if ((int)threadIdx.x < k) {
+                int64_t run = 0;
+                for (int i = 0; i < (int)threadIdx.x; i++) run += slots[i];
+                emit.probe_off[(size_t)q * k + threadIdx.x] = run;
+                if ((int)threadIdx.x == k - 1) emit.seg_len[q] = run + slots[threadIdx.x];
+            }
+        }
+    }
     if (threadIdx.x == 0) {
         const int32_t flag = (m > ncand && cnt == ncand) ? 1 : 0;
         flags[q] = flag;
@@ -453,7 +470,7 @@
     const int32_t *__restrict__ flags, int nq, float *__restrict__ seg_vals, int k, int kp, int cap,
     const unsigned *__restrict__ row_norm_max, ScanBound bound, const float *__restrict__ eps_add, int widen,
     float *__restrict__ out_dist, int64_t *__restrict__ out_slot, uint64_t *__restrict__ out_tid,
-    int32_t *__restrict__ out_i32, double *__restrict__ stats, float *__restrict__ pair_t) {
+    int32_t *__restrict__ out_i32, double *__restrict__ stats, float *__restrict__ pair_t, PlanEmit emit) {
     extern __shared__ __attribute__((aligned(16))) char smem[];
     unsigned long long *ent = reinterpret_cast<unsigned long long *>(smem);
     SelShared *sel = reinterpret_cast<SelShared *>(smem + (size_t)cap * 8);
@@ -489,9 +506,33 @@
                     __syncthreads();
                     fill_pair_terms(vectors, row_bytes, qrow, nvec * 4, out_i32 ? out_i32 + (size_t)q * k : nullptr,
                                     out_slot ? out_slot + (size_t)q * k : nullptr, k, pair_t + (size_t)q * k);
+                    if (emit.cnt) {
+                        if ((int)threadIdx.x < k) {
+                            const int l = __hip_atomic_load(out_i32 + (size_t)q * k + threadIdx.x, __ATOMIC_RELAXED,
+                                                            __HIP_MEMORY_SCOPE_AGENT);
+                            if (l >= 0) atomicAdd(&emit.cnt[l], 1);
+                            slots[threadIdx.x] = l >= 0 ? emit.list_off[l + 1] - emit.list_off[l] : 0;
+                        }
+                        __syncthreads();
+                        if ((int)threadIdx.x < k) {
+                            int64_t run = 0;
+                            for (int i = 0; i < (int)threadIdx.x; i++) run += slots[i];
+                            emit.probe_off[(size_t)q * k + threadIdx.x] = run;
+                            if ((int)threadIdx.x == k - 1) emit.seg_len[q] = run + slots[threadIdx.x];
+                        }
+                    }
                 }
             }
         };
+        if constexpr (std::is_same<T, float>::value) {
+            if (pair_t && emit.cnt) {
+                if ((int)threadIdx.x < k) {
+                    const int l = out_i32[(size_t)q * k + threadIdx.x];
+                    if (l >= 0) atomicSub(&emit.cnt[l], 1);
+                }
+                __syncthreads();
+            }
+        }
         bool settled = false;
         if (widen && k <= kWide / 2) {
             const int nw = (int)(m < kWide ? m : (int64_t)kWide);
@@ -774,8 +815,10 @@
                          const int64_t *seg_start, int64_t fixed_len, const ScanBound &bound,
                          float *out_dist, int64_t *out_slot, uint64_t *out_tid, int32_t *flags, int32_t *out_i32,
                          const int32_t *probe_lists, const int64_t *probe_off, int probes, const float *eps_add,
-                         float *pair_t) {
+                         float *pair_t, const PlanEmit &emit) {
     if (nq <= 0) return PGV_OK;
+    if (emit.cnt && !(pair_t && out_i32 && emit.probe_off && emit.seg_len && emit.list_off))
+        PGV_FAIL(PGV_ERR_ARG, "recheck: the plan is counted where the pair terms are written");
     if (kprime > kRecheckCap || k > kprime) PGV_FAIL(PGV_ERR_ARG, "recheck: k' = %d outside k..%d", kprime, kRecheckCap);
     if (pair_t && xr.dtype != PGV_F32) PGV_FAIL(PGV_ERR_ARG, "recheck: pair terms are for fp32 rows");
 #define PGV_RECHECK(T, DOT)                                                                                         \
@@ -783,7 +826,7 @@
                        static_cast<const char *>(xr.vectors), xr.tids, xr.geom.nvec, xr.geom.lpr_log2,               \
                        static_cast<const char *>(q_dev), kprime, k, approx_val, cand_pos, cand_slot, xr.list_offsets, \
                        probe_lists, probe_off, probes, seg_start, fixed_len, xr.norm_max, bound, eps_add, nq, out_dist, out_slot,  \
-                       out_tid, out_i32, flags, pair_t)
+                       out_tid, out_i32, flags, pair_t, emit)
     if (pair_t)
         PGV_RECHECK(float, true);
     else if (xr.dtype == PGV_F32)
@@ -798,8 +841,10 @@
 int launch_batch_fix(pgv_ctx *ctx, const ExactRows &xr, const void *q_dev, int nq, const int32_t *probe_lists,
                      const int64_t *probe_off, int probes, const int64_t *seg_start, int64_t fixed_len,
                      const int32_t *flags, float *seg_vals, int k, const ScanBound &bound, float *out_dist, int64_t *out_slot,
-                     uint64_t *out_tid, int32_t *out_i32, const float *eps_add, float *pair_t) {
+                     uint64_t *out_tid, int32_t *out_i32, const float *eps_add, float *pair_t, const PlanEmit &emit) {
     if (nq <= 0) return PGV_OK;
+    if (emit.cnt && !(pair_t && out_i32 && k <= kWide && emit.probe_off && emit.seg_len && emit.list_off))
+        PGV_FAIL(PGV_ERR_ARG, "fix: the plan is counted where the pair terms are written, k <= %d", kWide);
     if (pair_t && xr.dtype != PGV_F32) PGV_FAIL(PGV_ERR_ARG, "fix: pair terms are for fp32 rows");
     double *stats = (ctx->profiling && ctx->stats_dev.p) ? ctx->stats_dev.as<double>() : nullptr;
     if (k > 4096) PGV_FAIL(PGV_ERR_ARG, "top-k: k = %d exceeds the supported 4096", k);
@@ -814,7 +859,7 @@
                        static_cast<const char *>(xr.vectors), xr.list_offsets, xr.tids, xr.geom.nvec,                \
                        xr.geom.lpr_log2, static_cast<const char *>(q_dev), probe_lists, probe_off, probes, seg_start, \
                        fixed_len, flags, nq, seg_vals, k, kp, cap, xr.norm_max, bound, eps_add, widen, out_dist,      \
-                       out_slot, out_tid, out_i32, stats, pair_t)
+                       out_slot, out_tid, out_i32, stats, pair_t, emit)
     if (xr.dtype == PGV_F32)
         PGV_FIX(float);
     else
diff --git a/pgvector_amd/csrc/kernels_select.hip b/pgvector_amd/csrc/kernels_select.hip
--- a/pgvector_amd/csrc/kernels_select.hip
+++ b/pgvector_amd/csrc/kernels_select.hip
@@ -55,16 +55,21 @@
     const int *__restrict__ cnt, const int64_t *__restrict__ list_off,
     const int64_t *__restrict__ seg_len, int nq, int nlists, int qt, int rows_per_task,
     int64_t *__restrict__ seg_start, int64_t *__restrict__ pair_start,
-    int64_t *__restrict__ task_start, int64_t *__restrict__ totals ) {
+    int64_t *__restrict__ task_start, int64_t *__restrict__ totals ,
+    double *__restrict__ acc) {
     __shared__ int64_t scratch[1024 / 64 + 1];
+    __shared__ double red[2][1024 / 64];
     block_exclusive_scan(nq, [&](int i) { return seg_len[i]; }, seg_start, scratch);
     block_exclusive_scan(nlists, [&](int i) { return (int64_t)cnt[i]; }, pair_start, scratch);
+    double rows = 0.0, uniq = 0.0;
     block_exclusive_scan(
         nlists,
         [&](int i) {
             const int64_t len = list_off[i + 1] - list_off[i];
             const int64_t ng = (cnt[i] + qt - 1) / qt;
             const int64_t nc = (len + rows_per_task - 1) / rows_per_task;
+            rows += (double)ng * (double)len;
+            uniq += ng > 0 ? (double)len : 0.0;
             return ng * nc;
         },
         task_start, scratch);
@@ -73,16 +78,36 @@
         totals[1] = task_start[nlists];
         *reinterpret_cast<int *>(totals + 2) = (int)task_start[nlists];
     }
-}
-
-__global__ void plan_pairs_kernel(const int32_t *__restrict__ probe_lists,
-                                  const int64_t *__restrict__ list_off,
-                                  const int64_t *__restrict__ probe_off,
-                                  const int64_t *__restrict__ seg_start,
-                                  const int64_t *__restrict__ pair_start, int *__restrict__ fill,
-                                  int nq, int probes, const float *__restrict__ pair_t,
-                                  ScanPair *__restrict__ pairs) {
-    const int64_t i = (int64_t)blockIdx.x * blockDim.x + threadIdx.x;
+    if (acc) {
+        for (int o = 32; o > 0; o >>= 1) {
+            rows += __shfl_xor(rows, o);
+            uniq += __shfl_xor(uniq, o);
+        }
+        if ((threadIdx.x & 63) == 0) {
+            red[0][threadIdx.x >> 6] = rows;
+            red[1][threadIdx.x >> 6] = uniq;
+        }
+        __syncthreads();
+        if (threadIdx.x == 0) {
+            double r = 0.0, u = 0.0;
+            for (int w = 0; w < (int)(blockDim.x >> 6); w++) {
+                r += red[0][w];
+                u += red[1][w];
+            }
+            acc[0] += (double)seg_start[nq];
+            acc[1] += r;
+            acc[5] += u;
+        }
+    }
+}
+
+__device__ __forceinline__ void plan_pairs_body(int64_t i, const int32_t *__restrict__ probe_lists,
+                                                const int64_t *__restrict__ list_off,
+                                                const int64_t *__restrict__ probe_off,
+                                                const int64_t *__restrict__ seg_start,
+                                                const int64_t *__restrict__ pair_start, int *__restrict__ fill,
+                                                int nq, int probes, const float *__restrict__ pair_t,
+                                                ScanPair *__restrict__ pairs) {
     if (i >= (int64_t)nq * probes) return;
     const int q = (int)(i / probes);
     const int l = probe_lists[i];
@@ -94,12 +119,24 @@
     pairs[pos] = pr;
 }
 
-__global__ void plan_tasks_kernel(const int *__restrict__ cnt, const int64_t *__restrict__ list_off,
-                                  const int64_t *__restrict__ pair_start,
-                                  const int64_t *__restrict__ task_start, int nlists, int qt,
-                                  int rows_per_task, ScanTask *__restrict__ tasks) {
+__global__ void plan_pairs_kernel(const int32_t *__restrict__ probe_lists,
+                                  const int64_t *__restrict__ list_off,
+                                  const int64_t *__restrict__ probe_off,
+                                  const int64_t *__restrict__ seg_start,
+                                  const int64_t *__restrict__ pair_start, int *__restrict__ fill,
+                                  int nq, int probes, const float *__restrict__ pair_t,
+                                  ScanPair *__restrict__ pairs) {
+    plan_pairs_body((int64_t)blockIdx.x * blockDim.x + threadIdx.x, probe_lists, list_off, probe_off, seg_start, pair_start,
+                    fill, nq, probes, pair_t, pairs);
+}
+
+__device__ __forceinline__ void plan_tasks_body(int64_t first, int64_t stride, const int *__restrict__ cnt,
+                                                const int64_t *__restrict__ list_off,
+                                                const int64_t *__restrict__ pair_start,
+                                                const int64_t *__restrict__ task_start, int nlists, int qt,
+                                                int rows_per_task, ScanTask *__restrict__ tasks) {
     const int64_t ntasks = task_start[nlists];
-    for (int64_t t = (int64_t)blockIdx.x * blockDim.x + threadIdx.x; t < ntasks; t += (int64_t)gridDim.x * blockDim.x) {
+    for (int64_t t = first; t < ntasks; t += stride) {
         int lo = 0, hi = nlists - 1;
         while (lo < hi) {
             const int mid = (lo + hi + 1) >> 1;
@@ -125,19 +162,44 @@
     }
 }
 
+__global__ void plan_tasks_kernel(const int *__restrict__ cnt, const int64_t *__restrict__ list_off,
+                                  const int64_t *__restrict__ pair_start,
+                                  const int64_t *__restrict__ task_start, int nlists, int qt,
+                                  int rows_per_task, ScanTask *__restrict__ tasks) {
+    plan_tasks_body((int64_t)blockIdx.x * blockDim.x + threadIdx.x, (int64_t)gridDim.x * blockDim.x, cnt, list_off,
+                    pair_start, task_start, nlists, qt, rows_per_task, tasks);
+}
+
+__global__ void plan_pairs_tasks_kernel(const int32_t *__restrict__ probe_lists, const int64_t *__restrict__ list_off,
+                                        const int64_t *__restrict__ probe_off, const int64_t *__restrict__ seg_start,
+                                        const int64_t *__restrict__ pair_start, const int64_t *__restrict__ task_start,
+                                        const int *__restrict__ cnt, int *__restrict__ fill, int nq, int probes, int nlists,
+                                        int qt, int rows_per_task, const float *__restrict__ pair_t, int pair_blocks,
+                                        ScanPair *__restrict__ pairs, ScanTask *__restrict__ tasks) {
+    if ((int)blockIdx.x < pair_blocks)
+        plan_pairs_body((int64_t)blockIdx.x * blockDim.x + threadIdx.x, probe_lists, list_off, probe_off, seg_start,
+                        pair_start, fill, nq, probes, pair_t, pairs);
+    else
+        plan_tasks_body((int64_t)(blockIdx.x - pair_blocks) * blockDim.x + threadIdx.x,
+                        (int64_t)(gridDim.x - pair_blocks) * blockDim.x, cnt, list_off, pair_start, task_start, nlists, qt,
+                        rows_per_task, tasks);
+}
+
 __device__ __forceinline__ bool dist_before(float a, float b) { return float_to_key(a) < float_to_key(b); }
 
 
 __global__ __launch_bounds__(kSelThreads) void topk_kernel(
     const float *__restrict__ vals, const int64_t *__restrict__ seg_start, int64_t fixed_len,
     int k, int kp, int cap, float *__restrict__ out_val, int64_t *__restrict__ out_pos,
-    int32_t *__restrict__ zero_word) {
+    int32_t *__restrict__ zero_word, int32_t *__restrict__ zero_range, int zero_n) {
     extern __shared__ __attribute__((aligned(16))) char smem[];
     unsigned long long *ent = reinterpret_cast<unsigned long long *>(smem);
     SelShared *s = reinterpret_cast<SelShared *>(smem + (size_t)cap * 8);
 
     const int seg = blockIdx.x;
     if (zero_word && seg == 0 && threadIdx.x == 0) *zero_word = 0;
+    if (zero_range)
+        for (int i = seg * kSelThreads + (int)threadIdx.x; i < zero_n; i += (int)gridDim.x * kSelThreads) zero_range[i] = 0;
     const int64_t base = seg_start ? seg_start[seg] : (int64_t)seg * fixed_len;
     const int64_t m = seg_start ? seg_start[seg + 1] - base : fixed_len;
     const float *v = vals + base;
@@ -267,8 +329,25 @@
     return PGV_OK;
 }
 
+int plan_batch_reserve(pgv_ctx *ctx, int nlists, int nq, int probes, PlanBuffers *pb) {
+    const size_t npairs = (size_t)nq * probes;
+    PGV_TRY(ctx->plan_a.ensure(sizeof(int) * 2 * (size_t)nlists));
+    const size_t nb = npairs + (size_t)nq + (size_t)nq + 1 + 2 * ((size_t)nlists + 1) + 3;
+    PGV_TRY(ctx->plan_b.ensure(sizeof(int64_t) * nb));
+    pb->cnt = ctx->plan_a.as<int>();
+    pb->fill = pb->cnt + nlists;
+    pb->probe_off = ctx->plan_b.as<int64_t>();
+    pb->seg_len = pb->probe_off + npairs;
+    pb->seg_start = pb->seg_len + nq;
+    pb->pair_start = pb->seg_start + nq + 1;
+    pb->task_start = pb->pair_start + nlists + 1;
+    pb->totals = pb->task_start + nlists + 1;
+    return PGV_OK;
+}
+
 int launch_plan_batch(pgv_ctx *ctx, const pgv_index *ix, const int32_t *probe_lists, int nq,
-                      int probes, int qt, int rows_per_task, bool read_totals, PlanResult *res, const float *pair_t) {
+                      int probes, int qt, int rows_per_task, bool read_totals, PlanResult *res, const float *pair_t,
+                      bool counted) {
     const int nlists = ix->nlists;
     const size_t npairs = (size_t)nq * probes;
 
@@ -282,45 +361,52 @@
     res->out_bound = (int64_t)nq * ix->len_prefix[probes];
     if (res->ntasks_bound > 0x7fffffff) PGV_FAIL(PGV_ERR_ARG, "plan: too many tasks");
 
-    PGV_TRY(ctx->plan_a.ensure(sizeof(int) * 2 * (size_t)nlists));
-    const size_t nb = npairs + (size_t)nq + (size_t)nq + 1 + 2 * ((size_t)nlists + 1) + 3;
-    PGV_TRY(ctx->plan_b.ensure(sizeof(int64_t) * nb));
+    PlanBuffers pb;
+    PGV_TRY(plan_batch_reserve(ctx, nlists, nq, probes, &pb));
     PGV_TRY(ctx->pairs.ensure(sizeof(ScanPair) * npairs));
     PGV_TRY(ctx->tasks.ensure(sizeof(ScanTask) * (size_t)(res->ntasks_bound > 0 ? res->ntasks_bound : 1) + 16));
-    int *cnt = ctx->plan_a.as<int>();
-    int *fill = cnt + nlists;
-    int64_t *probe_off = ctx->plan_b.as<int64_t>();
-    int64_t *seg_len = probe_off + npairs;
-    int64_t *seg_start = seg_len + nq;
-    int64_t *pair_start = seg_start + nq + 1;
-    int64_t *task_start = pair_start + nlists + 1;
-    int64_t *totals = task_start + nlists + 1;
+    int *cnt = pb.cnt, *fill = pb.fill;
+    int64_t *probe_off = pb.probe_off, *seg_len = pb.seg_len, *seg_start = pb.seg_start, *pair_start = pb.pair_start;
+    int64_t *task_start = pb.task_start, *totals = pb.totals;
     ScanTask *tasks = ctx->tasks.as<ScanTask>();
-
-    PGV_HIP(hipMemsetAsync(cnt, 0, sizeof(int) * 2 * (size_t)nlists, ctx->stream));
-    hipLaunchKernelGGL(plan_count_kernel, dim3((nq + 255) / 256), dim3(256), 0, ctx->stream,
-                       probe_lists, ix->list_offsets, nq, probes, cnt, probe_off, seg_len);
-    hipLaunchKernelGGL(plan_scan_kernel, dim3(1), dim3(1024), 0, ctx->stream, cnt,
-                       ix->list_offsets, seg_len, nq, nlists, qt, rows_per_task, seg_start,
-                       pair_start, task_start, totals);
-    hipLaunchKernelGGL(plan_pairs_kernel, dim3((unsigned)((npairs + 255) / 256)), dim3(256), 0,
-                       ctx->stream, probe_lists, ix->list_offsets, probe_off, seg_start,
-                       pair_start, fill, nq, probes, pair_t, ctx->pairs.as<ScanPair>());
-    {
-        const int64_t want = (res->ntasks_bound + 255) / 256;
-        const int64_t cap = (int64_t)ctx->num_cus * 8;
-        hipLaunchKernelGGL(plan_tasks_kernel, dim3((unsigned)(want < 1 ? 1 : (want > cap ? cap : want))), dim3(256), 0,
-                           ctx->stream, cnt, ix->list_offsets, pair_start, task_start, nlists, qt, rows_per_task, tasks);
-    }
-    PGV_HIP(hipGetLastError());
-
+    const int64_t want = (res->ntasks_bound + 255) / 256;
+    const int64_t cap = (int64_t)ctx->num_cus * 8;
+    const unsigned task_blocks = (unsigned)(want < 1 ? 1 : (want > cap ? cap : want));
+    const unsigned pair_blocks = (unsigned)((npairs + 255) / 256);
     res->ntasks = res->ntasks_bound;
     res->total_out = res->out_bound;
-    if (read_totals) {
-        PGV_TRY(ctx->stats_dev.ensure(8 * sizeof(double)));
-        hipLaunchKernelGGL(plan_stats_kernel, dim3(1), dim3(256), 0, ctx->stream, cnt,
-                           ix->list_offsets, totals, nlists, qt, ctx->stats_dev.as<double>());
+
+    if (counted) {
+        double *acc = nullptr;
+        if (read_totals) {
+            PGV_TRY(ctx->stats_dev.ensure(8 * sizeof(double)));
+            acc = ctx->stats_dev.as<double>();
+        }
+        hipLaunchKernelGGL(plan_scan_kernel, dim3(1), dim3(1024), 0, ctx->stream, cnt, ix->list_offsets, seg_len, nq, nlists,
+                           qt, rows_per_task, seg_start, pair_start, task_start, totals, acc);
+        hipLaunchKernelGGL(plan_pairs_tasks_kernel, dim3(pair_blocks + task_blocks), dim3(256), 0, ctx->stream, probe_lists,
+                           ix->list_offsets, probe_off, seg_start, pair_start, task_start, cnt, fill, nq, probes, nlists, qt,
+                           rows_per_task, pair_t, (int)pair_blocks, ctx->pairs.as<ScanPair>(), tasks);
         PGV_HIP(hipGetLastError());
+    } else {
+        PGV_HIP(hipMemsetAsync(cnt, 0, sizeof(int) * 2 * (size_t)nlists, ctx->stream));
+        hipLaunchKernelGGL(plan_count_kernel, dim3((nq + 255) / 256), dim3(256), 0, ctx->stream,
+                           probe_lists, ix->list_offsets, nq, probes, cnt, probe_off, seg_len);
+        hipLaunchKernelGGL(plan_scan_kernel, dim3(1), dim3(1024), 0, ctx->stream, cnt,
+                           ix->list_offsets, seg_len, nq, nlists, qt, rows_per_task, seg_start,
+                           pair_start, task_start, totals, static_cast<double *>(nullptr));
+        hipLaunchKernelGGL(plan_pairs_kernel, dim3(pair_blocks), dim3(256), 0,
+                           ctx->stream, probe_lists, ix->list_offsets, probe_off, seg_start,
+                           pair_start, fill, nq, probes, pair_t, ctx->pairs.as<ScanPair>());
+        hipLaunchKernelGGL(plan_tasks_kernel, dim3(task_blocks), dim3(256), 0,
+                           ctx->stream, cnt, ix->list_offsets, pair_start, task_start, nlists, qt, rows_per_task, tasks);
+        PGV_HIP(hipGetLastError());
+        if (read_totals) {
+            PGV_TRY(ctx->stats_dev.ensure(8 * sizeof(double)));
+            hipLaunchKernelGGL(plan_stats_kernel, dim3(1), dim3(256), 0, ctx->stream, cnt,
+                               ix->list_offsets, totals, nlists, qt, ctx->stats_dev.as<double>());
+            PGV_HIP(hipGetLastError());
+        }
     }
     res->tasks = tasks;
     res->pairs = ctx->pairs.as<ScanPair>();
@@ -332,7 +418,8 @@
 }
 
 int launch_topk_segments(pgv_ctx *ctx, const float *vals, const int64_t *seg_start, int nseg,
-                         int64_t fixed_len, int k, float *out_val, int64_t *out_pos, int32_t *zero_word) {
+                         int64_t fixed_len, int k, float *out_val, int64_t *out_pos, int32_t *zero_word,
+                         int32_t *zero_range, int zero_n) {
     if (nseg <= 0 || k <= 0) return PGV_OK;
     if (k > 4096) PGV_FAIL(PGV_ERR_ARG, "top-k: k = %d exceeds the supported 4096", k);
     int kp = 1;
@@ -341,7 +428,7 @@
     const int cap = kp > kFastCap ? kp : kFastCap;
     const size_t lds = (size_t)cap * 8 + sizeof(SelShared);
     hipLaunchKernelGGL(topk_kernel, dim3(nseg), dim3(kSelThreads), lds, ctx->stream, vals,
-                       seg_start, fixed_len, k, kp, cap, out_val, out_pos, zero_word);
+                       seg_start, fixed_len, k, kp, cap, out_val, out_pos, zero_word, zero_range, zero_n);
     PGV_HIP(hipGetLastError());
     return PGV_OK;
 }
diff --git a/pgvector_amd/csrc/kernels_shadow.hip b/pgvector_amd/csrc/kernels_shadow.hip
--- a/pgvector_amd/csrc/kernels_shadow.hip
+++ b/pgvector_amd/csrc/kernels_shadow.hip
@@ -84,6 +84,59 @@
     }
 }
 
+constexpr int kCastChunks = 4;
+
+struct CastChunk {
+    float4 a, b;
+};
+
+__device__ __forceinline__ float absmax_keep_nan(float m, float v) {
+    const float a = fabsf(v);
+    return (a > m || a != a) ? a : m;
+}
+
+__device__ __forceinline__ CastChunk cast_chunk_load(const float *__restrict__ x, int c, int ld) {
+    CastChunk r;
+    const float4 zero = make_float4(0.f, 0.f, 0.f, 0.f);
+    r.a = 8 * c < ld ? *reinterpret_cast<const float4 *>(x + 8 * c) : zero;
+    r.b = 8 * c + 4 < ld ? *reinterpret_cast<const float4 *>(x + 8 * c + 4) : zero;
+    return r;
+}
+
+__device__ __forceinline__ float cast_chunk_max(const CastChunk &r, float m) {
+    m = absmax_keep_nan(m, r.a.x);
+    m = absmax_keep_nan(m, r.a.y);
+    m = absmax_keep_nan(m, r.a.z);
+    m = absmax_keep_nan(m, r.a.w);
+    m = absmax_keep_nan(m, r.b.x);
+    m = absmax_keep_nan(m, r.b.y);
+    m = absmax_keep_nan(m, r.b.z);
+    m = absmax_keep_nan(m, r.b.w);
+    return m;
+}
+
+__device__ __forceinline__ void cast_chunk_store(const CastChunk &r, int c, int ld, int sq, double up, __half *__restrict__ h,
+                                                 double (&qq)[4], double (&dd)[4], double (&hh)[4]) {
+    const float xs[8] = {r.a.x, r.a.y, r.a.z, r.a.w, r.b.x, r.b.y, r.b.z, r.b.w};
+    union {
+        __half v[8];
+        uint4 w;
+    } out;
+#pragma unroll
+    for (int e = 0; e < 8; e++) {
+        __half v = __float2half(0.f);
+        if (8 * c + e < ld) {
+            v = __float2half(ldexpf(xs[e], -sq));
+            const double back = (double)__half2float(v) * up, xi = (double)xs[e];
+            qq[e & 3] = fma(xi, xi, qq[e & 3]);
+            dd[e & 3] = fma(xi - back, xi - back, dd[e & 3]);
+            hh[e & 3] = fma(back, back, hh[e & 3]);
+        }
+        out.v[e] = v;
+    }
+    *reinterpret_cast<uint4 *>(h + 8 * c) = out.w;
+}
+
 __global__ __launch_bounds__(256) void shadow_query_kernel(const float *__restrict__ queries, int nq, int ld, int ld16,
                                                            ShadowTerms st, RankShadowTerms rt,
                                                            const float *__restrict__ center_norm_max,
@@ -95,10 +148,21 @@
     if (q >= nq) return;
     const int lane = threadIdx.x & (kWave - 1);
     const float *x = queries + (size_t)q * ld;
+    __half *h = qcast + (size_t)q * ld16;
+    const int nchunks = ld16 / 8;
+    const bool in_regs = nchunks <= kWave * kCastChunks;
+    CastChunk reg[kCastChunks];
     float m = 0.f;
-    for (int i = lane; i < ld; i += kWave) {
-        const float a = fabsf(x[i]);
-        m = (a > m || a != a) ? a : m;
+    if (in_regs) {
+#pragma unroll
+        for (int j = 0; j < kCastChunks; j++) {
+            const int c = lane + j * kWave;
+            reg[j] = cast_chunk_load(x, c < nchunks ? c : nchunks, ld);
+        }
+#pragma unroll
+        for (int j = 0; j < kCastChunks; j++) m = cast_chunk_max(reg[j], m);
+    } else {
+        for (int c = lane; c < nchunks; c += kWave) m = cast_chunk_max(cast_chunk_load(x, c, ld), m);
     }
     for (int o = 32; o > 0; o >>= 1) {
         const float v = __shfl_xor(m, o);
@@ -106,19 +170,19 @@
     }
     const int sq = scale_for(m);
     const double up = ldexp(1.0, sq);
-    double qq = 0.0, dd = 0.0, hh = 0.0;
-    __half *h = qcast + (size_t)q * ld16;
-    for (int i = lane; i < ld16; i += kWave) {
-        __half v = __float2half(0.f);
-        if (i < ld) {
-            v = __float2half(ldexpf(x[i], -sq));
-            const double back = (double)__half2float(v) * up, xi = (double)x[i];
-            qq = fma(xi, xi, qq);
-            dd = fma(xi - back, xi - back, dd);
-            hh = fma(back, back, hh);
-        }
-        h[i] = v;
-    }
+    double qq4[4] = {0.0, 0.0, 0.0, 0.0}, dd4[4] = {0.0, 0.0, 0.0, 0.0}, hh4[4] = {0.0, 0.0, 0.0, 0.0};
+    if (in_regs) {
+#pragma unroll
+        for (int j = 0; j < kCastChunks; j++) {
+            const int c = lane + j * kWave;
+            if (c < nchunks) cast_chunk_store(reg[j], c, ld, sq, up, h, qq4, dd4, hh4);
+        }
+    } else {
+        for (int c = lane; c < nchunks; c += kWave) cast_chunk_store(cast_chunk_load(x, c, ld), c, ld, sq, up, h, qq4, dd4, hh4);
+    }
+    double qq = (qq4[0] + qq4[1]) + (qq4[2] + qq4[3]);
+    double dd = (dd4[0] + dd4[1]) + (dd4[2] + dd4[3]);
+    double hh = (hh4[0] + hh4[1]) + (hh4[2] + hh4[3]);
     for (int o = 32; o > 0; o >>= 1) {
         qq += __shfl_xor(qq, o);
         dd += __shfl_xor(dd, o);
diff --git a/pgvector_amd/csrc/pgv_abi_ivf.hip b/pgvector_amd/csrc/pgv_abi_ivf.hip
--- a/pgvector_amd/csrc/pgv_abi_ivf.hip
+++ b/pgvector_amd/csrc/pgv_abi_ivf.hip
@@ -127,6 +127,8 @@
     float *pair_t = nullptr;
     bool scan_follows = false;
     bool cast_for_scan = false, cast_for_rank = false, pairs_done = false;
+    bool plan_counted = false;
+    int plan_nq = 0, plan_probes = 0;
 };
 
 int shadow_batch_cast(pgv_index *ix, const void *q_dev, int nq, int probes, bool for_rank, bool for_scan, ShadowBatch *sb) {
@@ -807,19 +809,32 @@
             PGV_TRY(dense_scan(ctx, ix->metric, ix->dtype, ix->geom, ix->centers, ix->nlists, q_dev, nq, ix->nlists, mat,
                                true, ix->center_norms, nullptr));
         }
-        PGV_TRY(launch_topk_segments(ctx, mat, nullptr, nq, ix->nlists, cand, sc.cand_val, sc.cand_pos, sc.flags + nq));
+        float *pair_t = (rank_sh && rank_env == 1 && scan_follows) ? sb->pair_t : nullptr;
+        PlanEmit emit;
+        PlanBuffers pbuf;
+        if (pair_t) {
+            PGV_TRY(plan_batch_reserve(ctx, ix->nlists, nq, maxprobes, &pbuf));
+            emit.cnt = pbuf.cnt;
+            emit.probe_off = pbuf.probe_off;
+            emit.seg_len = pbuf.seg_len;
+            emit.list_off = ix->list_offsets;
+        }
+        PGV_TRY(launch_topk_segments(ctx, mat, nullptr, nq, ix->nlists, cand, sc.cand_val, sc.cand_pos, sc.flags + nq,
+                                     emit.cnt, emit.cnt ? 2 * ix->nlists : 0));
         const ExactRows xr{ix->centers, nullptr, nullptr, ix->geom, ix->dtype,
                            reinterpret_cast<const unsigned *>(ix->center_norms + ix->nlists)};
         ScanBound bound = scan_bound_chain(ctx, ix->geom.ld, scan_chain_length(ix->geom, ix->dtype, false));
         if (rank_sh)
             bound = {0.f, 0.f, gamma_n(ix->geom.ld / 64.0 + 10.0, 5.9604645e-8), bound.g_ref};
-        float *pair_t = (rank_sh && rank_env == 1 && scan_follows) ? sb->pair_t : nullptr;
         PGV_TRY(launch_batch_recheck(ctx, xr, q_dev, nq, cand, maxprobes, sc.cand_val, sc.cand_pos, sc.cand_pos, nullptr,
                                      ix->nlists, bound, dist, nullptr, nullptr, sc.flags,
-                                     out_lists_dev, nullptr, nullptr, 0, rank_sh ? sb->ceps : nullptr, pair_t));
+                                     out_lists_dev, nullptr, nullptr, 0, rank_sh ? sb->ceps : nullptr, pair_t, emit));
         PGV_TRY(launch_batch_fix(ctx, xr, q_dev, nq, nullptr, nullptr, 0, nullptr, ix->nlists, sc.flags, mat, maxprobes,
-                                 bound, dist, nullptr, nullptr, out_lists_dev, rank_sh ? sb->ceps : nullptr, pair_t));
+                                 bound, dist, nullptr, nullptr, out_lists_dev, rank_sh ? sb->ceps : nullptr, pair_t, emit));
         sb->pairs_done = pair_t != nullptr;
+        sb->plan_counted = emit.cnt != nullptr;
+        sb->plan_nq = nq;
+        sb->plan_probes = maxprobes;
         return PGV_OK;
     } else {
         PGV_TRY(dense_scan(ctx, ix->metric, ix->dtype, ix->geom, ix->centers, ix->nlists, q_dev, nq, ix->nlists, mat,
@@ -1002,7 +1017,8 @@
     if (shadow && !sb->cast_for_scan) PGV_TRY(shadow_batch_cast(ix, q_dev, nq, probes, false, true, sb));
     const float *pair_t = (shadow && sb->pairs_done) ? sb->pair_t : nullptr;
     PlanResult plan;
-    PGV_TRY(launch_plan_batch(ctx, ix, probe_lists, nq, probes, qt, rows_per_task, ctx->profiling, &plan, pair_t));
+    const bool counted = pair_t && sb->plan_counted && sb->plan_nq == nq && sb->plan_probes == probes;
+    PGV_TRY(launch_plan_batch(ctx, ix, probe_lists, nq, probes, qt, rows_per_task, ctx->profiling, &plan, pair_t, counted));
 
     int kprime = k;
     ApproxScratch sc;
@@ -1137,6 +1153,31 @@
                           out_tid);
 }
 
+int pgv_index_shadow_cast(pgv_index *ix, const void *queries, int nq, void *out_qcast, float *out_qscale, float *out_qeps,
+                          float *out_cscale, float *out_ceps) {
+    if (!ix || !queries || nq < 1) PGV_FAIL(PGV_ERR_ARG, "pgv_index_shadow_cast: index/queries is NULL or nq < 1");
+    if (!ix->shadow || !ix->cshadow) PGV_FAIL(PGV_ERR_STATE, "pgv_index_shadow_cast: the index has no fp16 shadow");
+    pgv_ctx *ctx = ix->ctx;
+    PGV_HIP(hipSetDevice(ctx->device));
+    const void *q_dev;
+    PGV_TRY(stage_rows(ctx, queries, nq, ix->dim, ix->dtype, ix->geom, ctx->q_stage, &q_dev));
+    ShadowBatch sb;
+    PGV_TRY(shadow_batch_cast(ix, q_dev, nq, 1, true, true, &sb));
+    const struct {
+        void *dst;
+        const void *src;
+        size_t bytes;
+    } parts[] = {{out_qcast, sb.qcast, (size_t)nq * ix->shadow_geom.ld * sizeof(uint16_t)},
+                 {out_qscale, sb.qscale, sizeof(float) * (size_t)nq},
+                 {out_qeps, sb.qeps, sizeof(float) * (size_t)nq},
+                 {out_cscale, sb.cscale, sizeof(float) * (size_t)nq},
+                 {out_ceps, sb.ceps, sizeof(float) * (size_t)nq}};
+    for (const auto &p : parts)
+        if (p.dst) PGV_HIP(hipMemcpyAsync(p.dst, p.src, p.bytes, hipMemcpyDefault, ctx->stream));
+    PGV_HIP(hipStreamSynchronize(ctx->stream));
+    return PGV_OK;
+}
+
 namespace {
 
 struct QueryHeadHost {
diff --git a/pgvector_amd/csrc/pgv_internal.h b/pgvector_amd/csrc/pgv_internal.h
--- a/pgvector_amd/csrc/pgv_internal.h
+++ b/pgvector_amd/csrc/pgv_internal.h
@@ -415,11 +415,23 @@
     int64_t *probe_off = nullptr;
     int64_t *pair_start = nullptr;
 };
+struct PlanBuffers {
+    int *cnt = nullptr, *fill = nullptr;
+    int64_t *probe_off = nullptr, *seg_len = nullptr;
+    int64_t *seg_start = nullptr, *pair_start = nullptr, *task_start = nullptr, *totals = nullptr;
+};
+int plan_batch_reserve(pgv_ctx *ctx, int nlists, int nq, int probes, PlanBuffers *pb);
+struct PlanEmit {
+    int *cnt = nullptr;
+    int64_t *probe_off = nullptr, *seg_len = nullptr;
+    const int64_t *list_off = nullptr;
+};
 int launch_plan_batch(pgv_ctx *ctx, const pgv_index *ix, const int32_t *probe_lists, int nq,
                       int probes, int qt, int rows_per_task, bool read_totals, PlanResult *res,
-                      const float *pair_t = nullptr);
+                      const float *pair_t = nullptr, bool counted = false);
 int launch_topk_segments(pgv_ctx *ctx, const float *vals, const int64_t *seg_start, int nseg,
-                         int64_t fixed_len, int k, float *out_val, int64_t *out_pos, int32_t *zero_word = nullptr);
+                         int64_t fixed_len, int k, float *out_val, int64_t *out_pos, int32_t *zero_word = nullptr,
+                         int32_t *zero_range = nullptr, int zero_n = 0);
 int launch_positions_to_slots(pgv_ctx *ctx, const pgv_index *ix, const int32_t *probe_lists,
                               const int64_t *probe_off, int nq, int probes, int k,
                               const int64_t *pos, int64_t *out_slot, uint64_t *out_tid);
@@ -438,12 +450,13 @@
                          int32_t *out_i32 = nullptr, const int32_t *probe_lists = nullptr,
                          const int64_t *probe_off = nullptr, int probes = 0,
                          const float *eps_add = nullptr,
-                         float *pair_t = nullptr);
+                         float *pair_t = nullptr,
+                         const PlanEmit &emit = PlanEmit());
 int launch_batch_fix(pgv_ctx *ctx, const ExactRows &xr, const void *q_dev, int nq, const int32_t *probe_lists,
                      const int64_t *probe_off, int probes, const int64_t *seg_start, int64_t fixed_len,
                      const int32_t *flags, float *seg_vals, int k, const ScanBound &bound, float *out_dist, int64_t *out_slot,
                      uint64_t *out_tid, int32_t *out_i32 = nullptr, const float *eps_add = nullptr,
-                     float *pair_t = nullptr);
+                     float *pair_t = nullptr, const PlanEmit &emit = PlanEmit());
 int launch_iota_slots(pgv_ctx *ctx, const pgv_index *ix, const int32_t *lists_dev, int nlists,
                       const int64_t *probe_off, int64_t *out_slot);
 
```

Result: faster. 1.371 million (median of 6 runs) (+2.9%).
